# kwea123/CasMVSNet_pl

Measured on NVIDIA H100. Metric: depth-maps/sec at 640x512 V=3 D=48/32/8, higher is better.
Workload: dtype f32 (conv products tf32, fp32 accumulate)

## Files before the change

### casmvsnet_pl_b200/_lib.py

```python
import ctypes
import os
from ctypes import c_char_p, c_double, c_float, c_int, c_size_t, c_uint64, c_void_p, POINTER

_HERE = os.path.dirname(os.path.abspath(__file__))
LIB_PATH = os.path.join(_HERE, "csrc", "libcasmvs.so")

NCHW, NHWC = 0, 1
ROUND_TF32 = 256
KEEP_FP32_OUT = 256
FP32, TF32 = 0, 1
CONV, CONV_TRANSPOSE, CONV_PLANAR = 0, 1, 2
PRECISIONS = {"fp32": FP32, "tf32": TF32}

SIGNATURES = {
    "casmvs_version": (c_int, []),
    "casmvs_last_error": (c_char_p, []),
    "casmvs_device_check": (c_int, [c_int]),
    "casmvs_launch_count": (c_uint64, []),
    "casmvs_fallback_count": (c_uint64, []),
    "casmvs_release_weight_images": (c_int, [c_void_p, c_size_t]),
    "casmvs_weight_cache_generation": (c_uint64, []),
    "casmvs_weight_image_count": (c_int, [c_void_p, c_size_t]),
    "casmvs_settle_weight_images": (c_int, []),
    "casmvs_warp_cost_workspace_bytes": (c_size_t, [c_int] * 6),
    "casmvs_warp_cost_fwd": (c_int, [c_void_p, c_int, c_void_p, c_void_p, c_void_p, c_int,
                                     c_int, c_int, c_int, c_int, c_int, c_int, c_int,
                                     c_void_p, c_size_t, c_void_p]),
    "casmvs_homo_warp_fwd": (c_int, [c_void_p, c_int, c_void_p, c_void_p, c_void_p, c_int,
                                     c_int, c_int, c_int, c_int, c_int, c_void_p]),
    "casmvs_packed_conv3d_weight_floats": (c_size_t, [c_int, c_int]),
    "casmvs_pack_conv3d_weights": (c_int, [c_void_p, c_int, c_int, c_int, c_void_p, c_void_p]),
    "casmvs_invalidate_weight_cache": (c_int, []),
    "casmvs_conv3d_fwd": (c_int, [c_void_p, c_void_p, c_void_p, c_void_p, c_float, c_void_p,
                                  c_void_p, c_int, c_int, c_int, c_int, c_int, c_int,
                                  c_int, c_int, c_int, c_void_p]),
    "casmvs_costreg_param_floats": (c_size_t, [c_int]),
    "casmvs_costreg_layer_info": (c_int, [c_int, c_int, POINTER(c_int), POINTER(c_int),
                                          POINTER(c_int), POINTER(c_int), POINTER(c_size_t),
                                          POINTER(c_size_t), POINTER(c_size_t)]),
    "casmvs_costreg_workspace_bytes": (c_size_t, [c_int] * 5),
    "casmvs_costreg_fwd": (c_int, [c_void_p, c_void_p, c_void_p, c_int, c_int, c_int, c_int,
                                   c_int, c_int, c_void_p, c_size_t, c_void_p]),
    "casmvs_regress_fwd": (c_int, [c_void_p, c_void_p, c_int, c_int, c_void_p, c_void_p,
                                   c_void_p, c_void_p, c_int, c_int, c_int, c_int, c_void_p]),
    "casmvs_depth_hypotheses_fwd": (c_int, [c_void_p, c_int, c_float, c_float, c_void_p,
                                            c_void_p, c_int, c_int, c_int, c_int, c_void_p]),
    "casmvs_uniform_hypotheses_fwd": (c_int, [c_float, c_float, c_void_p, c_void_p, c_void_p,
                                              c_int, c_int, c_int, c_int, c_void_p]),
    "casmvs_depth_first_fwd": (c_int, [c_void_p, c_int, c_float, c_float, c_void_p, c_void_p,
                                       c_int, c_int, c_int, c_int, c_void_p]),
    "casmvs_warp_cost_ladder_fwd": (c_int, [c_void_p, c_void_p, c_void_p, c_void_p, c_float, c_void_p,
                                            c_float, c_void_p] + [c_int] * 8 + [c_void_p]),
    "casmvs_regress_ladder_fwd": (c_int, [c_void_p, c_void_p, c_void_p, c_float, c_void_p, c_float,
                                          c_void_p, c_void_p, c_void_p] + [c_int] * 4 + [c_void_p]),
    "casmvs_fpn_level_fwd": (c_int, [c_void_p] * 8 + [c_int] * 5 + [c_void_p]),
    "casmvs_fpn_merge_fwd": (c_int, [c_void_p] * 5 + [c_int] * 5 + [c_void_p]),
    "casmvs_conv2d_rgb8_fwd": (c_int, [c_void_p, c_void_p, c_void_p, c_float, c_void_p] + [c_int] * 4 + [c_void_p]),
    "casmvs_conv2d_5x5s2_fwd": (c_int, [c_void_p, c_void_p, c_void_p, c_float, c_void_p] + [c_int] * 6 + [c_void_p]),
    "casmvs_conv2d_5x5s2_fp32_fwd": (c_int, [c_void_p, c_void_p, c_void_p, c_float, c_void_p] + [c_int] * 5 + [c_void_p]),
    "casmvs_bias_act_nhwc": (c_int, [c_void_p, c_void_p, c_float, c_size_t, c_int, c_int, c_void_p]),
    "casmvs_bias_lrelu_nhwc": (c_int, [c_void_p, c_void_p, c_float, c_size_t, c_int, c_void_p]),
    "casmvs_normalize_u8_fwd": (c_int, [c_void_p, c_void_p, c_int, c_int, c_int, POINTER(c_float),
                                        POINTER(c_float), c_void_p]),
    "casmvs_warp_cost_bwd": (c_int, [c_void_p] * 5 + [c_int] * 7 + [c_void_p]),
    "casmvs_conv3d_wgrad": (c_int, [c_void_p] * 3 + [c_int] * 10 + [c_void_p]),
    "casmvs_regress_bwd": (c_int, [c_void_p, c_void_p, c_int, c_void_p, c_void_p] + [c_int] * 4 + [c_void_p]),
    "casmvs_geo_fuse_fwd": (c_int, [c_void_p, c_void_p, c_void_p, c_void_p, c_void_p,
                                    POINTER(c_float), POINTER(c_float), c_void_p, c_int, c_int,
                                    c_int, c_float, c_int, c_void_p, c_void_p, c_void_p, c_void_p,
                                    c_void_p, c_void_p, c_void_p, c_void_p]),
    "casmvs_pcd_cell_keys": (c_int, [c_void_p, c_int, c_double, c_double, c_double, c_double,
                                     c_int, c_int, c_int, c_int, c_void_p, c_void_p]),
    "casmvs_pcd_thin_workspace_bytes": (c_size_t, [c_int, c_int]),
    "casmvs_pcd_thin_prepare": (c_int, [c_void_p, c_void_p, c_int, c_int, c_int, c_int, c_int,
                                        c_void_p, c_size_t, c_void_p]),
    "casmvs_pcd_thin_round": (c_int, [c_void_p, c_void_p, c_void_p, c_int, c_int, c_double,
                                      c_void_p, c_void_p, c_void_p, c_size_t, c_void_p]),
    "casmvs_pcd_capped_nn": (c_int, [c_void_p, c_int, c_void_p, c_void_p, c_void_p, c_int, c_void_p,
                                     POINTER(c_double), c_double, POINTER(c_int), POINTER(c_double),
                                     POINTER(c_double), c_double, c_void_p, c_void_p]),
    "casmvs_nchw_to_nhwc":(c_int, [c_void_p, c_void_p, c_int, c_int, c_size_t, c_void_p]),
    "casmvs_nhwc_to_nchw": (c_int, [c_void_p, c_void_p, c_int, c_int, c_size_t, c_void_p]),
}

_lib = None


class CasMVSError(RuntimeError):
    pass


def load():
    global _lib
    if _lib is not None:
        return _lib
    if not os.path.isfile(LIB_PATH):
        raise CasMVSError(
            f"{LIB_PATH} not found: build it with `python -c 'import __graft_entry__ as g; "
            "g.build()'` (or `make -C casmvsnet_pl_b200/csrc`). There is no CPU/PyTorch "
            "fallback for the hot path.")
    lib = ctypes.CDLL(LIB_PATH)
    for name, (res, args) in SIGNATURES.items():
        fn = getattr(lib, name)
        fn.restype = res
        fn.argtypes = args
    _lib = lib
    return lib


def check(rc, what=""):
    if rc != 0:
        msg = load().casmvs_last_error()
        raise CasMVSError(f"{what}: {msg.decode() if msg else 'error'} (status {rc})")


def launch_count():
    return int(load().casmvs_launch_count())


def fallback_count():
    return int(load().casmvs_fallback_count())


def weight_cache_generation():
    return int(load().casmvs_weight_cache_generation())
```

### casmvsnet_pl_b200/csrc/api.cu

```cuda
#include <stdarg.h>
#include <string.h>

#include "common.cuh"

namespace casmvs {

std::atomic<uint64_t> g_launches{0};
std::atomic<uint64_t> g_fallbacks{0};
static thread_local char t_err[512] = "";

void set_error(const char* fmt, ...) {
  va_list ap;
  va_start(ap, fmt);
  vsnprintf(t_err, sizeof(t_err), fmt, ap);
  va_end(ap);
}

int conv3d_direct(const float* x, const float* wpk, const float* scale, const float* shift,
                  float slope, const float* skip, float* y, int B, int Cin, int Cout, int D,
                  int h, int w, int kind, int stride, cudaStream_t st, int round_out);
int conv3d_tma(const float* x, const float* wpk, const float* scale, const float* shift,
               float slope, const float* skip, float* y, int B, int Cin, int Cout, int D, int h,
               int w, int kind, int stride, int precision, cudaStream_t st);
int conv3d_tma2(const float* x, const float* wpk, const float* scale, const float* shift,
                float slope, const float* skip, float* y, int B, int Cin, int Cout, int D, int h,
                int w, int kind, int stride, int precision, cudaStream_t st);

struct LayerSpec { int cin, cout, kind, stride; };

static void costreg_layers(int Cin, LayerSpec (&L)[11]) {
  const LayerSpec t[11] = {
      {Cin, 8, CASMVS_CONV, 1},  {8, 16, CASMVS_CONV, 2},  {16, 16, CASMVS_CONV, 1},
      {16, 32, CASMVS_CONV, 2},  {32, 32, CASMVS_CONV, 1}, {32, 64, CASMVS_CONV, 2},
      {64, 64, CASMVS_CONV, 1},  {64, 32, CASMVS_CONV_TRANSPOSE, 2},
      {32, 16, CASMVS_CONV_TRANSPOSE, 2}, {16, 8, CASMVS_CONV_TRANSPOSE, 2},
      {8, 1, CASMVS_CONV, 1}};
  memcpy(L, t, sizeof(t));
}

}

using namespace casmvs;

extern "C" int casmvs_version(void) { return CASMVS_VERSION; }
extern "C" const char* casmvs_last_error(void) { return t_err; }
extern "C" uint64_t casmvs_launch_count(void) { return g_launches.load(); }

extern "C" uint64_t casmvs_fallback_count(void) { return g_fallbacks.load(); }

extern "C" int casmvs_device_check(int device) {
  int n = 0;
  cudaError_t e = cudaGetDeviceCount(&n);
  if (e != cudaSuccess || n == 0) {
    set_error("device_check: no CUDA device (%s)", cudaGetErrorString(e));
    return -3;
  }
  CASMVS_REQUIRE(device >= 0 && device < n, "device_check: device %d out of range (%d)", device, n);
  int major = 0, minor = 0;
  cudaDeviceGetAttribute(&major, cudaDevAttrComputeCapabilityMajor, device);
  cudaDeviceGetAttribute(&minor, cudaDevAttrComputeCapabilityMinor, device);
  if (major != 9 || minor != 0) {
    set_error("device_check: compute capability %d.%d; libcasmvs is built for sm_90a only "
              "(no fallback path)", major, minor);
    return -3;
  }
  return 0;
}

extern "C" int casmvs_conv3d_fwd(const float* x, const float* w_packed, const float* scale,
                                 const float* shift, float slope, const float* skip, float* y,
                                 int B, int Cin, int Cout, int D, int h, int w, int kind,
                                 int stride, int precision, void* stream) {
  CASMVS_REQUIRE(x && w_packed && y, "conv3d: null pointer");
  CASMVS_REQUIRE(B >= 0 && Cin > 0 && Cout > 0 && D > 0 && h > 0 && w > 0, "conv3d: bad dims");
  CASMVS_REQUIRE(Cin % 4 == 0, "conv3d: Cin must be a multiple of 4 (got %d)", Cin);
  CASMVS_REQUIRE(kind == CASMVS_CONV || kind == CASMVS_CONV_TRANSPOSE ||
                     kind == CASMVS_CONV_PLANAR, "conv3d: bad kind");
  CASMVS_REQUIRE(kind == CASMVS_CONV ? (stride == 1 || stride == 2)
                 : kind == CASMVS_CONV_PLANAR ? stride == 1 : stride == 2,
                 "conv3d: unsupported stride %d", stride);
  const int flags = precision & ~0xff;
  precision &= 0xff;
  CASMVS_REQUIRE((precision == CASMVS_FP32 || precision == CASMVS_TF32) &&
                     (flags & ~CASMVS_KEEP_FP32_OUT) == 0, "conv3d: bad precision %d", precision);
  if (B == 0) return 0;
  cudaStream_t st = as_stream(stream);
  if (precision == CASMVS_TF32) {
    const int pf = precision | flags;
    int rc = conv3d_tma(x, w_packed, scale, shift, slope, skip, y, B, Cin, Cout, D, h, w, kind,
                    stride, pf, st);
    if (rc <= 0) return rc;
    if (kind != CASMVS_CONV_PLANAR) {
      rc = conv3d_tma2(x, w_packed, scale, shift, slope, skip, y, B, Cin, Cout, D, h, w, kind,
                       stride, precision, st);
      if (rc <= 0) return rc;
    }
    g_fallbacks.fetch_add(1, std::memory_order_relaxed);
  }
  const int round_out =
      (precision == CASMVS_TF32 && Cout > 1 && !(flags & CASMVS_KEEP_FP32_OUT)) ? 1 : 0;
  return conv3d_direct(x, w_packed, scale, shift, slope, skip, y, B, Cin, Cout, D, h, w, kind,
                       stride, st, round_out);
}

extern "C" size_t casmvs_costreg_param_floats(int Cin) {
  LayerSpec L[11];
  costreg_layers(Cin, L);
  size_t n = 0;
  for (auto& l : L) n += (size_t)27 * l.cin * l.cout + 2 * (size_t)l.cout;
  return n;
}

extern "C" int casmvs_costreg_layer_info(int Cin, int layer, int* cin, int* cout, int* kind,
                                         int* stride, size_t* w_off, size_t* scale_off,
                                         size_t* shift_off) {
  CASMVS_REQUIRE(layer >= 0 && layer < 11, "costreg_layer_info: layer %d out of range", layer);
  LayerSpec L[11];
  costreg_layers(Cin, L);
  size_t off = 0;
  for (int i = 0; i < layer; ++i) off += (size_t)27 * L[i].cin * L[i].cout + 2 * (size_t)L[i].cout;
  if (cin) *cin = L[layer].cin;
  if (cout) *cout = L[layer].cout;
  if (kind) *kind = L[layer].kind;
  if (stride) *stride = L[layer].stride;
  if (w_off) *w_off = off;
  off += (size_t)27 * L[layer].cin * L[layer].cout;
  if (scale_off) *scale_off = off;
  if (shift_off) *shift_off = off + L[layer].cout;
  return 0;
}

extern "C" size_t casmvs_costreg_workspace_bytes(int B, int Cin, int D, int h, int w) {
  (void)Cin;
  const size_t n = (size_t)B * D * h * w;
  return (8 * n + 2 * n + 2 * n + n / 2 + n / 2 + n / 8 + n / 8 + n / 2 + 2 * n + 8 * n + 64) *
         sizeof(float);
}

extern "C" int casmvs_costreg_fwd(const float* x, const float* params, float* logits, int B,
                                  int Cin, int D, int h, int w, int precision, void* workspace,
                                  size_t workspace_bytes, void* stream) {
  CASMVS_REQUIRE(x && params && logits, "costreg: null pointer");
  CASMVS_REQUIRE(D % 8 == 0 && h % 8 == 0 && w % 8 == 0,
                 "costreg: D,h,w must be divisible by 8 (got %d,%d,%d)", D, h, w);
  const size_t need = casmvs_costreg_workspace_bytes(B, Cin, D, h, w);
  CASMVS_REQUIRE(workspace && workspace_bytes >= need, "costreg: workspace too small (%zu < %zu)",
                 workspace_bytes, need);
  if (B == 0) return 0;
  LayerSpec L[11];
  costreg_layers(Cin, L);
  const float *W[11], *SC[11], *SH[11];
  {
    size_t off = 0;
    for (int i = 0; i < 11; ++i) {
      W[i] = params + off; off += (size_t)27 * L[i].cin * L[i].cout;
      SC[i] = params + off; off += L[i].cout;
      SH[i] = params + off; off += L[i].cout;
    }
  }
  const size_t n = (size_t)B * D * h * w;
  float* ws = (float*)workspace;
  float* c0 = ws;            ws += 8 * n;
  float* c1 = ws;            ws += 2 * n;
  float* c2 = ws;            ws += 2 * n;
  float* c3 = ws;            ws += n / 2;
  float* c4 = ws;            ws += n / 2;
  float* c5 = ws;            ws += n / 8;
  float* c6 = ws;            ws += n / 8;
  float* u7 = ws;            ws += n / 2;
  float* u9 = ws;            ws += 2 * n;
  float* u11 = ws;
  const float slope = 0.01f;
  int rc;
#define LAYER(i, in, skip, out, d_, h_, w_, sl)                                                   \
  rc = casmvs_conv3d_fwd(in, W[i], SC[i], SH[i], sl, skip, out, B, L[i].cin, L[i].cout, d_, h_,  \
                         w_, L[i].kind, L[i].stride, precision, stream);                          \
  if (rc) return rc;
  LAYER(0, x, nullptr, c0, D, h, w, slope)
  LAYER(1, c0, nullptr, c1, D, h, w, slope)
  LAYER(2, c1, nullptr, c2, D / 2, h / 2, w / 2, slope)
  LAYER(3, c2, nullptr, c3, D / 2, h / 2, w / 2, slope)
  LAYER(4, c3, nullptr, c4, D / 4, h / 4, w / 4, slope)
  LAYER(5, c4, nullptr, c5, D / 4, h / 4, w / 4, slope)
  LAYER(6, c5, nullptr, c6, D / 8, h / 8, w / 8, slope)
  LAYER(7, c6, c4, u7, D / 8, h / 8, w / 8, slope)
  LAYER(8, u7, c2, u9, D / 4, h / 4, w / 4, slope)
  LAYER(9, u9, c0, u11, D / 2, h / 2, w / 2, slope)
  LAYER(10, u11, nullptr, logits, D, h, w, 1.0f)
#undef LAYER
  return 0;
}
```

### casmvsnet_pl_b200/csrc/common.cuh

```cuda
#pragma once
#include <cuda_runtime.h>
#include <stdint.h>
#include <stdio.h>
#include <atomic>

#include "casmvs.h"

#if defined(__CUDA_ARCH__) && (__CUDA_ARCH__ != 900)
#error "libcasmvs is written for sm_90a (H100) only"
#endif

namespace casmvs {

void set_error(const char* fmt, ...);
extern std::atomic<uint64_t> g_launches;
extern std::atomic<uint64_t> g_fallbacks;

inline cudaStream_t as_stream(void* s) { return reinterpret_cast<cudaStream_t>(s); }

inline int after_launch(const char* what) {
  g_launches.fetch_add(1, std::memory_order_relaxed);
  cudaError_t e = cudaGetLastError();
  if (e != cudaSuccess) {
    set_error("%s: kernel launch failed: %s", what, cudaGetErrorString(e));
    return -2;
  }
  return 0;
}

#define CASMVS_REQUIRE(cond, ...)        \
  do {                                   \
    if (!(cond)) {                       \
      casmvs::set_error(__VA_ARGS__);    \
      return -1;                         \
    }                                    \
  } while (0)

constexpr int kMaxDevices = 64;
inline int cur_device() {
  int dev = 0;
  cudaGetDevice(&dev);
  return dev >= 0 && dev < kMaxDevices ? dev : 0;
}
inline int num_sms() {
  static std::atomic<int> n[kMaxDevices];
  const int dev = cur_device();
  int v = n[dev].load(std::memory_order_relaxed);
  if (v == 0) {
    cudaDeviceGetAttribute(&v, cudaDevAttrMultiProcessorCount, dev);
    if (v <= 0) v = 132;
    n[dev].store(v, std::memory_order_relaxed);
  }
  return v;
}
template <typename K>
inline int opt_in_smem(K kfn, int bytes, std::atomic<bool> (&done)[kMaxDevices], const char* what) {
  const int dev = cur_device();
  if (done[dev].load(std::memory_order_acquire)) return 0;
  cudaError_t e = cudaFuncSetAttribute(kfn, cudaFuncAttributeMaxDynamicSharedMemorySize, bytes);
  if (e != cudaSuccess) {
    set_error("%s: cannot opt in to %d B of shared memory: %s", what, bytes, cudaGetErrorString(e));
    return -2;
  }
  done[dev].store(true, std::memory_order_release);
  return 0;
}

struct FastDiv {
  uint32_t d, m;
};
inline FastDiv make_fastdiv(uint32_t d) {
  return FastDiv{d, d > 1 ? (uint32_t)((1ull << 32) / d) + 1u : 0u};
}
inline bool fastdiv_ok(uint64_t n_max, uint32_t d) { return n_max * d < (1ull << 32); }
__device__ __forceinline__ uint32_t fastdivmod(uint32_t n, const FastDiv f, uint32_t& r) {
  const uint32_t q = f.d > 1 ? __umulhi(n, f.m) : n;
  r = n - q * f.d;
  return q;
}

__device__ __forceinline__ float4 ldg4(const float* p) {
  return __ldg(reinterpret_cast<const float4*>(p));
}
__device__ __forceinline__ void st4(float* p, float4 v) {
  *reinterpret_cast<float4*>(p) = v;
}
__device__ __forceinline__ void st4_stream(float* p, float4 v) {
  asm volatile("st.global.L1::no_allocate.v4.f32 [%0], {%1,%2,%3,%4};" ::"l"(p), "f"(v.x),
               "f"(v.y), "f"(v.z), "f"(v.w)
               : "memory");
}

}
```

### casmvsnet_pl_b200/csrc/conv3d_tma.cu

```cuda
#include <cudaTypedefs.h>
#include <stdlib.h>

#include "common.cuh"
#include "tc_common.cuh"
#include <mutex>

#include "tma_common.cuh"

namespace casmvs {

namespace tma {

using namespace tc;

struct Params {
  const float* bimg;
  const float* scale;
  const float* shift;
  const float* skip;
  float* y;
  float slope;
  int B, D, H, W, Cout;
  int cout_total;
  int tiles_w, tiles_h, nchunks, dchunk;
  int round_out;
  int planar;
};

template <int CIN, int GW, int SLOTS_>
struct Smem {
  static constexpr int SLOTS = SLOTS_;
  static constexpr int CQ = CIN / 4;
  static constexpr int kBrickData = kHaloH * kHaloW * 16;
  static constexpr int kBrickBytes = (kBrickData + 127) / 128 * 128;
  static constexpr int kSlotBytes = CQ * kBrickBytes;
  static constexpr int kWBytes = 9 * CIN * 3 * GW * 4;
  static constexpr int kRingOff = 0;
  static constexpr int kWOff = SLOTS * kSlotBytes;
  static constexpr int kParamOff = kWOff + kWBytes;
  static constexpr int kBarOff = kParamOff + 2 * GW * 4;
  static constexpr int kTotal = kBarOff + 192 + 1024;
};

template <int GW, int OFF>
__device__ __forceinline__ void store_slice(const float* acc, const Params& p, const float* s_param,
                                            int b, int od, int h0, int w0, int row0, int wl,
                                            int lane, int co_base) {
  for_each_pair<OFF, GW>(acc, wl, lane, [&](int r, int c, float a0, float a1) {
    const int m = row0 + r;
    const int oh = h0 + (m >> 3), ow = w0 + (m & 7);
    if (oh >= p.H || ow >= p.W || c >= p.Cout) return;
    const size_t o = ((((size_t)b * p.D + od) * p.H + oh) * p.W + ow) * p.cout_total + co_base + c;
    float v0 = fmaf(a0, s_param[c], s_param[GW + c]);
    float v1 = fmaf(a1, s_param[c + 1], s_param[GW + c + 1]);
    v0 = v0 >= 0.f ? v0 : v0 * p.slope;
    v1 = v1 >= 0.f ? v1 : v1 * p.slope;
    if (c + 1 < p.Cout && (p.cout_total & 1) == 0) {
      if (p.skip) {
        const float2 s2 = __ldg(reinterpret_cast<const float2*>(p.skip + o));
        v0 += s2.x; v1 += s2.y;
      }
      if (p.round_out) { v0 = to_tf32(v0); v1 = to_tf32(v1); }
      *reinterpret_cast<float2*>(p.y + o) = make_float2(v0, v1);
    } else {
      if (p.skip) v0 += __ldg(p.skip + o);
      p.y[o] = p.round_out ? to_tf32(v0) : v0;
      if (c + 1 < p.Cout) {
        if (p.skip) v1 += __ldg(p.skip + o + 1);
        p.y[o + 1] = p.round_out ? to_tf32(v1) : v1;
      }
    }
  });
}

template <int CIN, int GW, int SLOTS_, bool PLANAR>
__global__ void __launch_bounds__(kConvThreads, 1)
conv3d_tma_kernel(const __grid_constant__ CUtensorMap xmap, const Params p) {
  using S = Smem<CIN, GW, SLOTS_>;
  constexpr int SLOTS = S::SLOTS;
  extern __shared__ unsigned char smem_raw[];
  const uint32_t s_raw = smem_u32(smem_raw);
  const uint32_t s_base = (s_raw + 1023u) & ~1023u;
  unsigned char* smem = smem_raw + (s_base - s_raw);
  const uint32_t s_ring = s_base + S::kRingOff, s_w = s_base + S::kWOff,
                 s_bar = s_base + S::kBarOff;
  float* s_param = reinterpret_cast<float*>(smem + S::kParamOff);
  const uint32_t bar_full = s_bar, bar_empty = s_bar + 64, bar_w = s_bar + 128;

  const int warp = warp_uniform(threadIdx.x >> 5), lane = threadIdx.x & 31;
  const int total_items = p.B * p.nchunks * p.tiles_h * p.tiles_w;

  {
    const int t = threadIdx.x;
    if (t < SLOTS) mbar_init(bar_full + 8 * t, 1);
    else if (t < 2 * SLOTS) mbar_init(bar_empty + 8 * (t - SLOTS), kConsumerThreads);
    else if (t == 2 * SLOTS) mbar_init(bar_w, 1);
    if (t <= 2 * SLOTS) fence_barrier_init();
  }
  const int co_base = blockIdx.y * p.Cout;
  for (int i = threadIdx.x; i < GW; i += kConvThreads) {
    s_param[i] = (i < p.Cout) ? (p.scale ? __ldg(p.scale + co_base + i) : 1.f) : 0.f;
    s_param[GW + i] = (i < p.Cout) ? (p.shift ? __ldg(p.shift + co_base + i) : 0.f) : 0.f;
  }
  fence_proxy_async();
  __syncthreads();
  if (threadIdx.x == 0) load_image_bulk(s_w, p.bimg + (size_t)blockIdx.y * (S::kWBytes / 4), S::kWBytes, bar_w);

  tma::pdl_trigger();
  tma::pdl_wait();
  bool w_ready = false;
  uint32_t gs = 0;
  float acc[(PLANAR ? 1 : 3) * GW / 2];
#pragma unroll
  for (int i = 0; i < (PLANAR ? 1 : 3) * GW / 2; ++i) acc[i] = 0.f;
  float done[GW / 2];
  int pend_od = -1, pend_b = 0, pend_h0 = 0, pend_w0 = 0;
  const int wg = warp >> 2, wl = warp & 3;
  const int row0 = 64 * wg;
  for (int item0 = blockIdx.x; item0 < total_items; item0 += gridDim.x) {
    int item = item0;
    const int tw = item % p.tiles_w; item /= p.tiles_w;
    const int th = item % p.tiles_h; item /= p.tiles_h;
    const int ck = item % p.nchunks;
    const int b = item / p.nchunks;
    const int w0 = tw * kTileW, h0 = th * kTileH;
    const int d0 = ck * p.dchunk, d1 = min(p.D, d0 + p.dchunk);
    const int nd = d1 - d0;
    const int halo = PLANAR ? 0 : 1;
    const int nslices = nd + 2 * halo;

    if (warp == kProdWarp) {
      if (lane == 0) {
        for (int it = 0; it < nslices; ++it) {
          const uint32_t g = gs + it;
          const int slot = g % SLOTS;
          if (g >= (uint32_t)SLOTS) mbar_wait(bar_empty + 8 * slot, ((g / SLOTS) - 1) & 1);
          const uint32_t dst = s_ring + slot * S::kSlotBytes;
          mbar_expect_tx(bar_full + 8 * slot, S::CQ * S::kBrickData);
#pragma unroll
          for (int q = 0; q < S::CQ; ++q)
            tma_load_5d(dst + q * S::kBrickBytes, &xmap, bar_full + 8 * slot, q * 4, w0 - 1,
                        h0 - 1, d0 - halo + it, b);
        }
      }
      __syncwarp();
    } else {
      constexpr uint32_t a_lbo = S::kBrickBytes, a_sbo = kHaloW * 16;
      constexpr uint32_t b_lbo = 3 * GW * 16, b_sbo = 128;
      const uint64_t a_desc0 = make_desc(s_ring + 8 * wg * a_sbo, a_lbo, a_sbo);
      const uint64_t b_desc0 = make_desc(s_w, b_lbo, b_sbo);
      for (int it = 0; it < nslices; ++it) {
        const uint32_t g = gs + it;
        mbar_wait(bar_full + 8 * (g % SLOTS), (g / SLOTS) & 1);
        if (!w_ready) { mbar_wait(bar_w, 0); w_ready = true; }
        const uint64_t a_s = a_desc0 + (((g % SLOTS) * S::kSlotBytes) >> 4);
        wgmma_fence();
#pragma unroll
        for (int khw = 0; khw < 9; ++khw) {
          const int kh = khw / 3, kw = khw % 3;
#pragma unroll
          for (int k8 = 0; k8 < CIN / 8; ++k8) {
            const uint32_t a_off = ((kh * kHaloW + kw) * 16 + 2 * k8 * S::kBrickBytes) >> 4;
            const uint32_t b_off = (khw * (CIN * 3 * GW * 4) + k8 * 2 * 3 * GW * 16) >> 4;
            if constexpr (PLANAR)
              wgmma_tf32<GW>(acc, a_s + a_off, b_desc0 + b_off + ((GW * 16) >> 4));
            else
              wgmma_tf32<3 * GW>(acc, a_s + a_off, b_desc0 + b_off);
          }
        }
        wgmma_commit();
        if (pend_od >= 0)
          store_slice<GW, 0>(done, p, s_param, pend_b, pend_od, pend_h0, pend_w0, row0, wl, lane,
                             co_base);
        wgmma_wait_all();
        mbar_arrive(bar_empty + 8 * (g % SLOTS));
#pragma unroll
        for (int i = 0; i < GW / 2; ++i) done[i] = acc[i];
        if constexpr (PLANAR) {
#pragma unroll
          for (int i = 0; i < GW / 2; ++i) acc[i] = 0.f;
        } else {
#pragma unroll
          for (int i = 0; i < GW; ++i) acc[i] = acc[i + GW / 2];
#pragma unroll
          for (int i = 0; i < GW / 2; ++i) acc[GW + i] = 0.f;
        }
        const int j = PLANAR ? it : it - 2;
        pend_od = (j >= 0 && j < nd) ? d0 + j : -1;
        pend_b = b; pend_h0 = h0; pend_w0 = w0;
      }
    }
    gs += nslices;
  }
  if (pend_od >= 0)
    store_slice<GW, 0>(done, p, s_param, pend_b, pend_od, pend_h0, pend_w0, row0, wl, lane, co_base);
}


static PFN_cuTensorMapEncodeTiled_v12000 encode_fn() {
  static PFN_cuTensorMapEncodeTiled_v12000 fn = nullptr;
  static bool tried = false;
  if (!tried) {
    tried = true;
    void* ptr = nullptr;
    cudaDriverEntryPointQueryResult q;
    if (cudaGetDriverEntryPoint("cuTensorMapEncodeTiled", &ptr, cudaEnableDefault, &q) ==
            cudaSuccess && q == cudaDriverEntryPointSuccess)
      fn = reinterpret_cast<PFN_cuTensorMapEncodeTiled_v12000>(ptr);
  }
  return fn;
}

int encode_tiled(CUtensorMap* out, const void* base, int rank, const uint64_t* dims,
                 const uint64_t* strides_bytes, const uint32_t* box, int swizzle_bytes) {
  auto enc = encode_fn();
  if (!enc) { set_error("tma: cuTensorMapEncodeTiled is not available"); return -2; }
  cuuint64_t gdim[5], gstr[4];
  cuuint32_t bx[5], es[5];
  for (int i = 0; i < rank; ++i) { gdim[i] = dims[i]; bx[i] = box[i]; es[i] = 1; }
  for (int i = 0; i + 1 < rank; ++i) gstr[i] = strides_bytes[i];
  const CUtensorMapSwizzle sw = swizzle_bytes == 128 ? CU_TENSOR_MAP_SWIZZLE_128B
                                : swizzle_bytes == 64 ? CU_TENSOR_MAP_SWIZZLE_64B
                                : swizzle_bytes == 32 ? CU_TENSOR_MAP_SWIZZLE_32B
                                                      : CU_TENSOR_MAP_SWIZZLE_NONE;
  const CUresult r = enc(out, CU_TENSOR_MAP_DATA_TYPE_FLOAT32, (cuuint32_t)rank,
                         const_cast<void*>(base), gdim, gstr, bx, es,
                         CU_TENSOR_MAP_INTERLEAVE_NONE, sw, CU_TENSOR_MAP_L2_PROMOTION_L2_128B,
                         CU_TENSOR_MAP_FLOAT_OOB_FILL_NONE);
  if (r != CUDA_SUCCESS) {
    set_error("tma: cuTensorMapEncodeTiled failed (%d), rank %d", (int)r, rank);
    return -2;
  }
  return 0;
}

struct MapEntry { const void* x; int B, D, H, W, C, CB, bw, bh, sw; CUtensorMap map; };
static MapEntry g_maps[128];
static int g_maps_n = 0, g_maps_next = 0;
static std::mutex g_maps_mu;

const CUtensorMap* input_map(const float* x, int B, int D, int H, int W, int C, int CB, int box_w,
                             int box_h, int stride_w) {
  static thread_local CUtensorMap t_ret;
  std::lock_guard<std::mutex> lock(g_maps_mu);
  for (int i = 0; i < g_maps_n; ++i) {
    const MapEntry& e = g_maps[i];
    if (e.x == x && e.B == B && e.D == D && e.H == H && e.W == W && e.C == C && e.CB == CB &&
        e.bw == box_w && e.bh == box_h && e.sw == stride_w) {
      t_ret = e.map;
      return &t_ret;
    }
  }
  auto enc = encode_fn();
  if (!enc) { set_error("conv3d_tma: cuTensorMapEncodeTiled is not available"); return nullptr; }
  MapEntry& e = g_maps[g_maps_next];
  g_maps_next = (g_maps_next + 1) % 128;
  if (g_maps_n < 128) ++g_maps_n;
  const cuuint64_t gdim[5] = {(cuuint64_t)C, (cuuint64_t)W, (cuuint64_t)H, (cuuint64_t)D,
                              (cuuint64_t)B};
  const cuuint64_t gstr[4] = {(cuuint64_t)C * 4, (cuuint64_t)W * C * 4, (cuuint64_t)H * W * C * 4,
                              (cuuint64_t)D * H * W * C * 4};
  const cuuint32_t box[5] = {(cuuint32_t)CB, (cuuint32_t)box_w, (cuuint32_t)box_h, 1, 1};
  const cuuint32_t estr[5] = {1, (cuuint32_t)stride_w, 1, 1, 1};
  const CUtensorMapSwizzle sw = CB * 4 == 128 ? CU_TENSOR_MAP_SWIZZLE_128B
                                : CB * 4 == 64 ? CU_TENSOR_MAP_SWIZZLE_64B
                                : CB * 4 == 32 ? CU_TENSOR_MAP_SWIZZLE_32B
                                               : CU_TENSOR_MAP_SWIZZLE_NONE;
  const CUresult r = enc(&e.map, CU_TENSOR_MAP_DATA_TYPE_FLOAT32, 5, const_cast<float*>(x), gdim,
                         gstr, box, estr, CU_TENSOR_MAP_INTERLEAVE_NONE, sw,
                         CU_TENSOR_MAP_L2_PROMOTION_L2_128B, CU_TENSOR_MAP_FLOAT_OOB_FILL_NONE);
  if (r != CUDA_SUCCESS) {
    e.x = nullptr;
    set_error("conv3d_tma: cuTensorMapEncodeTiled failed (%d) for C=%d W=%d H=%d D=%d B=%d",
              (int)r, C, W, H, D, B);
    return nullptr;
  }
  e.x = x; e.B = B; e.D = D; e.H = H; e.W = W; e.C = C; e.CB = CB; e.bw = box_w; e.bh = box_h; e.sw = stride_w;
  t_ret = e.map;
  return &t_ret;
}


template <int CIN, int GW, int SLOTS, bool PLANAR>
static int launch(const float* x, const float* wpk, Params p, cudaStream_t st) {
  using S = Smem<CIN, GW, SLOTS>;
  static_assert(S::kTotal <= 227 * 1024, "shared memory budget");
  auto kfn = conv3d_tma_kernel<CIN, GW, SLOTS, PLANAR>;
  static std::atomic<bool> attr_set[kMaxDevices];
  if (int rc = opt_in_smem(kfn, S::kTotal, attr_set, "conv3d_tma")) return rc;
  const CUtensorMap* map = input_map(x, p.B, p.D, p.H, p.W, CIN, 4, kHaloW, kHaloH);
  if (!map) return -2;
  static int dchunk_env = -1;
  if (dchunk_env < 0) {
    const char* d = getenv("CASMVS_TMA_DCHUNK");
    dchunk_env = d ? atoi(d) : 0;
  }
  const int per_sm = resident_per_sm(kfn, kConvThreads, S::kTotal);
  const int nco = p.cout_total / p.Cout;
  const int cap = 32;
  const long cols = (long)p.B * p.tiles_w * p.tiles_h;
  int dchunk = pick_dchunk(p.D, cap, cols, (long)num_sms() * per_sm / nco, 1, p.planar ? 0 : 2);
  if (dchunk_env > 0 && dchunk_env <= cap) dchunk = dchunk_env < p.D ? dchunk_env : p.D;
  p.dchunk = dchunk;
  p.nchunks = (p.D + dchunk - 1) / dchunk;
  const ImageRef ir = image_cache_get(wpk, 1000 + CIN * 100 + GW, (size_t)S::kWBytes * nco, st);
  if (!ir.img) return -2;
  if (!ir.hit) {
    if (int rc = build_stride1_image(wpk, ir.img, CIN, GW, p.Cout, p.cout_total, st)) return rc;
    image_cache_built(ir.img, st);
  }
  p.bimg = ir.img;
  const long items = (long)p.B * p.nchunks * p.tiles_h * p.tiles_w;
  int resident = num_sms() * per_sm / nco;
  if (resident < 1) resident = 1;
  const long gx = items < resident ? items : resident;
  launch_pdl(ir.settled, kfn, dim3((unsigned)gx, (unsigned)nco), kConvThreads, S::kTotal, st, *map, p);
  return after_launch("conv3d_tma");
}

}

int conv3d_tma(const float* x, const float* wpk, const float* scale, const float* shift,
               float slope, const float* skip, float* y, int B, int Cin, int Cout, int D, int h,
               int w, int kind, int stride, int precision_flags, cudaStream_t st) {
  const int precision = precision_flags & 0xff;
  static int enabled = -1, round_out = 1;
  if (enabled < 0) {
    const char* e = getenv("CASMVS_TMA");
    enabled = e ? atoi(e) : 1;
    if (const char* s = getenv("CASMVS_TC_ROUND")) round_out = atoi(s);
  }
  if (!enabled || precision != CASMVS_TF32) return 1;
  if ((kind != CASMVS_CONV && kind != CASMVS_CONV_PLANAR) || stride != 1) return 1;
  const bool deep = Cin == 64 && Cout == 64;
  if (!deep && (!(Cin == 8 || Cin == 16 || Cin == 32) || Cout > 32)) return 1;
  if ((reinterpret_cast<uintptr_t>(x) & 15) != 0) return 1;
  tma::Params p;
  p.scale = scale; p.shift = shift; p.skip = skip; p.y = y;
  p.slope = slope; p.B = B; p.D = D; p.H = h; p.W = w;
  p.Cout = deep ? 16 : Cout; p.cout_total = Cout;
  p.tiles_w = (w + tc::kTileW - 1) / tc::kTileW;
  p.tiles_h = (h + tc::kTileH - 1) / tc::kTileH;
  const int npad = p.Cout <= 8 ? 8 : p.Cout <= 16 ? 16 : 32;
  p.planar = kind == CASMVS_CONV_PLANAR ? 1 : 0;
  p.round_out = (round_out && Cout > 1 && !(precision_flags & CASMVS_KEEP_FP32_OUT)) ? 1 : 0;
#define TMA_CASE(CI, NP, SL)                                                    \
  if (Cin == CI && npad == NP)                                                  \
    return p.planar ? tma::launch<CI, NP, SL, true>(x, wpk, p, st)              \
                    : tma::launch<CI, NP, SL, false>(x, wpk, p, st);
  TMA_CASE(8, 8, 4) TMA_CASE(8, 32, 4) TMA_CASE(16, 8, 4) TMA_CASE(16, 16, 4)
  TMA_CASE(16, 32, 4) TMA_CASE(32, 8, 4) TMA_CASE(32, 16, 4) TMA_CASE(32, 32, 4)
  TMA_CASE(64, 16, 2)
#undef TMA_CASE
  return 1;
}

}
```

### casmvsnet_pl_b200/csrc/conv3d_tma2.cu

```cuda
#include <stdlib.h>

#include "common.cuh"
#include "tc_common.cuh"
#include "tma_common.cuh"

namespace casmvs {
namespace tma2 {

using namespace casmvs::tc;
using casmvs::tma::mbar_expect_tx;
using casmvs::tma::tma_load_5d;

enum { MODE_S2 = 0, MODE_T = 1, MODE_P5 = 2 };

struct Params {
  const float* bimg;
  const float* scale;
  const float* shift;
  const float* skip;
  float* y;
  float slope;
  int B, Di, Hi, Wi, Do, Ho, Wo, Cout;
  int tiles_w, tiles_h, nchunks, dchunk;
  int round_out;
};

template <int MODE, int CIN, int COUT>
struct Cfg {
  static constexpr int CQ = CIN / 4;
  static constexpr int BR = MODE == MODE_S2 ? 33 : MODE == MODE_T ? 17 : 35;
  static constexpr int BW = MODE == MODE_P5 ? 10 : 9;
  static constexpr int PAR = MODE == MODE_T ? 1 : 2;
  static constexpr int NPL = PAR * CQ;
  static constexpr int kPlaneData = BR * BW * 16;
  static constexpr int kPlaneBytes = (kPlaneData + 127) / 128 * 128;
  static constexpr int kSlotBytes = NPL * kPlaneBytes;
  static constexpr int GW = MODE == MODE_T ? 8 * COUT : (COUT <= 16 ? 16 : 32);
  static constexpr int BROWS = MODE == MODE_S2 ? 3 * GW : MODE == MODE_T ? 12 * COUT : GW;
  static constexpr int NTAP = MODE == MODE_S2 ? 9 : MODE == MODE_T ? 4 : 25;
  static constexpr int kWBytes = NTAP * CIN * BROWS * 4;
  static constexpr int kFixed = kWBytes + 2 * 32 * 4 + 192 + 1024;
  static constexpr int SLOTS = (kFixed + 4 * kSlotBytes <= 227 * 1024) ? 4
                               : (kFixed + 3 * kSlotBytes <= 227 * 1024) ? 3 : 2;
  static constexpr int kRingOff = 0;
  static constexpr int kWOff = SLOTS * kSlotBytes;
  static constexpr int kParamOff = kWOff + kWBytes;
  static constexpr int kBarOff = kParamOff + 2 * 32 * 4;
  static constexpr int kTotal = kBarOff + 192 + 1024;
};

template <int MODE, int CIN, int COUT>
__global__ void __launch_bounds__(kConvThreads, 1)
conv3d_tma2_kernel(const __grid_constant__ CUtensorMap xmap, const Params p) {
  using C = Cfg<MODE, CIN, COUT>;
  constexpr int BW = C::BW, GW = C::GW, BROWS = C::BROWS;
  constexpr int SLOTS = C::SLOTS;
  extern __shared__ unsigned char smem_raw[];
  const uint32_t s_raw = smem_u32(smem_raw);
  const uint32_t s_base = (s_raw + 1023u) & ~1023u;
  unsigned char* smem = smem_raw + (s_base - s_raw);
  const uint32_t s_ring = s_base + C::kRingOff, s_w = s_base + C::kWOff,
                 s_bar = s_base + C::kBarOff;
  float* s_param = reinterpret_cast<float*>(smem + C::kParamOff);
  const uint32_t bar_full = s_bar, bar_empty = s_bar + 64, bar_w = s_bar + 128;
  const int warp = warp_uniform(threadIdx.x >> 5), lane = threadIdx.x & 31;
  const int total_items = p.B * p.nchunks * p.tiles_h * p.tiles_w;
  const int Dm = MODE == MODE_T ? p.Di : p.Do;

  {
    const int t = threadIdx.x;
    if (t < SLOTS) mbar_init(bar_full + 8 * t, 1);
    else if (t < 2 * SLOTS) mbar_init(bar_empty + 8 * (t - SLOTS), kConsumerThreads);
    else if (t == 2 * SLOTS) mbar_init(bar_w, 1);
    if (t <= 2 * SLOTS) fence_barrier_init();
  }
  const int co_base = blockIdx.y * COUT;
  for (int i = threadIdx.x; i < 32; i += kConvThreads) {
    s_param[i] = (i < COUT) ? (p.scale ? __ldg(p.scale + co_base + i) : 1.f) : 0.f;
    s_param[32 + i] = (i < COUT) ? (p.shift ? __ldg(p.shift + co_base + i) : 0.f) : 0.f;
  }
  fence_proxy_async();
  __syncthreads();
  if (threadIdx.x == 0) tma::load_image_bulk(s_w, p.bimg + (size_t)blockIdx.y * (C::kWBytes / 4), C::kWBytes, bar_w);

  tma::pdl_trigger();
  tma::pdl_wait();
  bool w_ready = false;
  uint32_t gs = 0;
  for (int item0 = blockIdx.x; item0 < total_items; item0 += gridDim.x) {
    int item = item0;
    const int tw = item % p.tiles_w; item /= p.tiles_w;
    const int th = item % p.tiles_h; item /= p.tiles_h;
    const int ck = item % p.nchunks;
    const int b = item / p.nchunks;
    const int w0 = tw * kTileW, h0 = th * kTileH;
    const int g0 = ck * p.dchunk, g1 = min(Dm, g0 + p.dchunk);
    const int ng = g1 - g0;
    const int nslices = MODE == MODE_S2 ? 2 * ng + 1 : MODE == MODE_T ? ng + 1 : ng;
    const int s_first = MODE == MODE_S2 ? 2 * g0 - 1 : g0;

    if (warp == kProdWarp) {
      if (lane == 0) {
        for (int it = 0; it < nslices; ++it) {
          const uint32_t g = gs + it;
          const int slot = g % SLOTS;
          if (g >= (uint32_t)SLOTS) mbar_wait(bar_empty + 8 * slot, ((g / SLOTS) - 1) & 1);
          const uint32_t dst = s_ring + slot * C::kSlotBytes;
          mbar_expect_tx(bar_full + 8 * slot, C::NPL * C::kPlaneData);
#pragma unroll
          for (int pl = 0; pl < C::NPL; ++pl) {
            const int q = pl / C::PAR, par = pl % C::PAR;
            const int wc = MODE == MODE_S2 ? 2 * w0 - 1 + par
                           : MODE == MODE_T ? w0 : 2 * w0 - 2 + par;
            const int hc = MODE == MODE_S2 ? 2 * h0 - 1 : MODE == MODE_T ? h0 : 2 * h0 - 2;
            tma_load_5d(dst + pl * C::kPlaneBytes, &xmap, bar_full + 8 * slot, 4 * q, wc,
                        hc, s_first + it, b);
          }
        }
      }
      __syncwarp();
    } else {
      const int wg = warp >> 2, wl = warp & 3;
      const int row0 = 64 * wg;
      constexpr uint32_t a_lbo = C::PAR * C::kPlaneBytes;
      constexpr uint32_t a_sbo = (MODE == MODE_T ? 1 : 2) * BW * 16;
      constexpr uint32_t b_lbo = BROWS * 16, b_sbo = 128;
      const uint64_t a_desc0 = make_desc(s_ring + 8 * wg * a_sbo, a_lbo, a_sbo);
      const uint64_t b_desc0 = make_desc(s_w, b_lbo, b_sbo);
      constexpr int NACC = MODE == MODE_S2 ? 2 * GW : MODE == MODE_T ? 12 * COUT : GW;
      float acc[NACC / 2];
      float prev0[MODE == MODE_T ? 2 * COUT : 1];
#pragma unroll
      for (int i = 0; i < NACC / 2; ++i) acc[i] = 0.f;

      auto issue = [&](auto n_tag, uint64_t a_s, int row0b) {
        constexpr int N = decltype(n_tag)::value;
        wgmma_fence();
#pragma unroll
        for (int tap = 0; tap < C::NTAP; ++tap) {
          int a_tap, pl0;
          if (MODE == MODE_S2) {
            const int kh = tap / 3, kw = tap % 3;
            a_tap = kh * BW + (kw == 2 ? 1 : 0);
            pl0 = kw == 1 ? 1 : 0;
          } else if (MODE == MODE_P5) {
            const int kh = tap / 5, kw = tap % 5;
            a_tap = kh * BW + (kw >> 1);
            pl0 = kw & 1;
          } else {
            const int sh = tap >> 1, sw = tap & 1;
            a_tap = sh * BW + sw;
            pl0 = 0;
          }
#pragma unroll
          for (int k8 = 0; k8 < CIN / 8; ++k8) {
            const uint32_t a_off = ((2 * k8 * C::PAR + pl0) * C::kPlaneBytes + a_tap * 16) >> 4;
            const uint32_t b_off = (tap * (CIN * BROWS * 4) + k8 * 2 * BROWS * 16 + row0b * 16) >> 4;
            wgmma_tf32<N>(acc, a_s + a_off, b_desc0 + b_off);
          }
        }
        wgmma_commit();
        wgmma_wait_all();
      };

      auto store2 = [&](int od, int oh, int ow, int c, float a0, float a1, bool has_skip) {
        const size_t o = ((((size_t)b * p.Do + od) * p.Ho + oh) * p.Wo + ow) * p.Cout + co_base + c;
        float v0 = fmaf(a0, s_param[c], s_param[32 + c]);
        float v1 = fmaf(a1, s_param[c + 1], s_param[32 + c + 1]);
        v0 = v0 >= 0.f ? v0 : v0 * p.slope;
        v1 = v1 >= 0.f ? v1 : v1 * p.slope;
        if (has_skip) {
          const float2 s2 = __ldg(reinterpret_cast<const float2*>(p.skip + o));
          v0 += s2.x; v1 += s2.y;
        }
        if (p.round_out) { v0 = to_tf32(v0); v1 = to_tf32(v1); }
        *reinterpret_cast<float2*>(p.y + o) = make_float2(v0, v1);
      };
      auto store_plain = [&](const float* src, int od) {
        for_each_pair<0, GW>(src, wl, lane, [&](int r, int c, float a0, float a1) {
          const int m = row0 + r;
          const int mh = h0 + (m >> 3), mw = w0 + (m & 7);
          if (c < COUT && mh < p.Ho && mw < p.Wo) store2(od, mh, mw, c, a0, a1, false);
        });
      };
      auto store_t = [&](const float* pd1, int jd) {
        auto one = [&](int pd, int r, int col, float a0, float a1) {
          const int m = row0 + r;
          const int mh = h0 + (m >> 3), mw = w0 + (m & 7);
          if (mh >= p.Hi || mw >= p.Wi) return;
          const int cls = col / COUT, c = col % COUT;
          const int ph = cls >> 1, pw = cls & 1;
          store2(2 * jd + pd, 2 * mh + ph, 2 * mw + pw, c, a0, a1, p.skip != nullptr);
        };
        for_each_pair<0, 4 * COUT>(prev0, wl, lane,
                                   [&](int r, int col, float a0, float a1) { one(0, r, col, a0, a1); });
        for_each_pair<0, 4 * COUT>(pd1, wl, lane,
                                   [&](int r, int col, float a0, float a1) { one(1, r, col, a0, a1); });
      };

      for (int it = 0; it < nslices; ++it) {
        const uint32_t g = gs + it;
        mbar_wait(bar_full + 8 * (g % SLOTS), (g / SLOTS) & 1);
        if (!w_ready) { mbar_wait(bar_w, 0); w_ready = true; }
        const uint64_t a_s = a_desc0 + (((g % SLOTS) * C::kSlotBytes) >> 4);
        if constexpr (MODE == MODE_S2) {
          if ((it & 1) == 0) issue(std::integral_constant<int, 2 * GW>{}, a_s, GW);
          else issue(std::integral_constant<int, GW>{}, a_s, 0);
        } else if constexpr (MODE == MODE_P5) {
#pragma unroll
          for (int i = 0; i < GW / 2; ++i) acc[i] = 0.f;
          issue(std::integral_constant<int, GW>{}, a_s, 0);
        } else {
          issue(std::integral_constant<int, 12 * COUT>{}, a_s, 0);
        }
        mbar_arrive(bar_empty + 8 * (g % SLOTS));
        if constexpr (MODE == MODE_S2) {
          if ((it & 1) == 0) {
            const int a = it >> 1;
            float done[GW / 2];
#pragma unroll
            for (int i = 0; i < GW / 2; ++i) {
              done[i] = acc[i];
              acc[i] = acc[GW / 2 + i];
              acc[GW / 2 + i] = 0.f;
            }
            if (a >= 1) store_plain(done, g0 + a - 1);
          }
        } else if constexpr (MODE == MODE_P5) {
          float done[GW / 2];
#pragma unroll
          for (int i = 0; i < GW / 2; ++i) done[i] = acc[i];
          store_plain(done, g0 + it);
        } else {
          float pd1[2 * COUT];
#pragma unroll
          for (int i = 0; i < 2 * COUT; ++i) pd1[i] = acc[i];
          if (it >= 1) store_t(pd1, g0 + it - 1);
#pragma unroll
          for (int i = 0; i < 2 * COUT; ++i) {
            prev0[i] = acc[2 * COUT + i];
            acc[i] = acc[4 * COUT + i];
            acc[2 * COUT + i] = 0.f;
            acc[4 * COUT + i] = 0.f;
          }
        }
      }
    }
    gs += nslices;
  }
}

template <int MODE, int CIN, int COUT>
__global__ void build_image_tma2_kernel(const float* __restrict__ wpk, float* __restrict__ img,
                                        int cout_total) {
  using C = Cfg<MODE, CIN, COUT>;
  constexpr int CQ = C::CQ, GW = C::GW, BROWS = C::BROWS;
  constexpr int per = C::NTAP * CIN * BROWS;
  for (int t = blockIdx.x * blockDim.x + threadIdx.x; t < per * (cout_total / COUT);
       t += gridDim.x * blockDim.x) {
    const int ck = t / per, i = t - ck * per;
    const int jq = i & 3;
    const int row = (i >> 2) % BROWS;
    const int r = (i >> 2) / BROWS;
    const int cq = r % CQ, tap = r / CQ;
    const int ci = cq * 4 + jq;
    int kd = -1, kh = -1, kw = -1, co = -1;
    if (MODE == MODE_S2) {
      const int g = row / GW;
      co = row % GW;
      kd = g == 0 ? 1 : g == 1 ? 2 : 0;
      kh = tap / 3; kw = tap % 3;
      if (co >= COUT) kd = -1;
    } else {
      const int sh = tap >> 1, sw = tap & 1;
      const int blk = row / (4 * COUT);
      const int cls = (row / COUT) & 3;
      co = row % COUT;
      const int ph = cls >> 1, pw = cls & 1;
      kd = blk;
      kh = sh == 0 ? (ph == 0 ? 1 : 2) : (ph == 1 ? 0 : -1);
      kw = sw == 0 ? (pw == 0 ? 1 : 2) : (pw == 1 ? 0 : -1);
      if (kh < 0 || kw < 0) kd = -1;
    }
    float v = 0.f;
    if (kd >= 0)
      v = to_tf32(__ldg(wpk + ((size_t)((kd * 3 + kh) * 3 + kw) * CIN + ci) * cout_total +
                        ck * COUT + co));
    img[t] = v;
  }
}

template <int CIN, int COUT>
__global__ void build_image_p5_kernel(const float* __restrict__ wt, float* __restrict__ img) {
  using C = Cfg<MODE_P5, CIN, COUT>;
  constexpr int CQ = C::CQ, GW = C::GW;
  constexpr int total = 25 * CIN * GW;
  for (int t = blockIdx.x * blockDim.x + threadIdx.x; t < total; t += gridDim.x * blockDim.x) {
    const int jq = t & 3;
    const int co = (t >> 2) % GW;
    const int r = (t >> 2) / GW;
    const int cq = r % CQ, tap = r / CQ;
    const int ci = cq * 4 + jq;
    img[t] = co < COUT ? to_tf32(__ldg(wt + ((size_t)co * CIN + ci) * 25 + tap)) : 0.f;
  }
}

template <int MODE, int CIN, int COUT>
static int launch2(const float* x, const float* wpk, Params p, cudaStream_t st) {
  using C = Cfg<MODE, CIN, COUT>;
  static_assert(C::kTotal <= 227 * 1024, "shared memory budget");
  auto kfn = conv3d_tma2_kernel<MODE, CIN, COUT>;
  static std::atomic<bool> attr_set[kMaxDevices];
  if (int rc = opt_in_smem(kfn, C::kTotal, attr_set, "conv3d_tma2")) return rc;
  const CUtensorMap* map =
      MODE == MODE_S2   ? tma::input_map(x, p.B, p.Di, p.Hi, p.Wi, CIN, 4, 17, C::BR, 2)
      : MODE == MODE_P5 ? tma::input_map(x, p.B, p.Di, p.Hi, p.Wi, CIN, 4, 19, C::BR, 2)
                        : tma::input_map(x, p.B, p.Di, p.Hi, p.Wi, CIN, 4, C::BW, C::BR, 1);
  if (!map) return -2;
  const int per_sm = tma::resident_per_sm(kfn, kConvThreads, C::kTotal);
  const int Dm = MODE == MODE_T ? p.Di : p.Do;
  const int Hm = MODE == MODE_T ? p.Hi : p.Ho, Wm = MODE == MODE_T ? p.Wi : p.Wo;
  p.tiles_w = (Wm + kTileW - 1) / kTileW;
  p.tiles_h = (Hm + kTileH - 1) / kTileH;
  const int nco = p.Cout / COUT;
  const int cap = 32;
  const long cols = (long)p.B * p.tiles_w * p.tiles_h;
  const int dchunk = tma::pick_dchunk(Dm, cap, cols, (long)num_sms() * per_sm / nco,
                                      MODE == MODE_S2 ? 2 : 1,
                                      MODE == MODE_S2 ? 1 : MODE == MODE_T ? 1 : 0);
  p.dchunk = dchunk;
  p.nchunks = (Dm + dchunk - 1) / dchunk;
  const long items = cols * p.nchunks;
  const ImageRef ir = image_cache_get(wpk, 2000 + MODE * 10000 + CIN * 100 + COUT,
                                      (size_t)C::kWBytes * nco, st);
  float* img = ir.img;
  if (!img) return -2;
  if (!ir.hit) {
    if constexpr (MODE == MODE_P5)
      build_image_p5_kernel<CIN, COUT><<<32, 256, 0, st>>>(wpk, img);
    else
      build_image_tma2_kernel<MODE, CIN, COUT><<<64, 256, 0, st>>>(wpk, img, p.Cout);
    if (int rc = after_launch("conv3d_tma2/build_image")) return rc;
    image_cache_built(img, st);
  }
  p.bimg = img;
  long resident = (long)num_sms() * per_sm / nco;
  if (resident < 1) resident = 1;
  const long gx = items < resident ? items : resident;
  tma::launch_pdl(ir.settled, kfn, dim3((unsigned)gx, (unsigned)nco), kConvThreads, C::kTotal, st, *map, p);
  return after_launch("conv3d_tma2");
}

}

int conv3d_tma2(const float* x, const float* wpk, const float* scale, const float* shift,
                float slope, const float* skip, float* y, int B, int Cin, int Cout, int D, int h,
                int w, int kind, int stride, int precision, cudaStream_t st) {
  static int enabled = -1;
  if (enabled < 0) {
    const char* e = getenv("CASMVS_TMA2");
    enabled = e ? atoi(e) : 3;
  }
  if (!enabled || precision != CASMVS_TF32) return 1;
  if ((reinterpret_cast<uintptr_t>(x) & 15) != 0) return 1;
  tma2::Params p;
  p.scale = scale; p.shift = shift; p.skip = skip; p.y = y;
  p.slope = slope; p.B = B; p.Di = D; p.Hi = h; p.Wi = w; p.Cout = Cout; p.round_out = 1;
  if (kind == CASMVS_CONV && stride == 2 && (enabled & 1)) {
    if (skip) return 1;
    p.Do = (D - 1) / 2 + 1; p.Ho = (h - 1) / 2 + 1; p.Wo = (w - 1) / 2 + 1;
    if (Cin == 8 && Cout == 16) return tma2::launch2<tma2::MODE_S2, 8, 16>(x, wpk, p, st);
    if (Cin == 16 && Cout == 32) return tma2::launch2<tma2::MODE_S2, 16, 32>(x, wpk, p, st);
    if (Cin == 32 && Cout == 64) return tma2::launch2<tma2::MODE_S2, 32, 16>(x, wpk, p, st);
    return 1;
  }
  if (kind == CASMVS_CONV_TRANSPOSE && (enabled & 2)) {
    p.Do = 2 * D; p.Ho = 2 * h; p.Wo = 2 * w;
    if (Cin == 16 && Cout == 8) return tma2::launch2<tma2::MODE_T, 16, 8>(x, wpk, p, st);
    if (Cin == 32 && Cout == 16) return tma2::launch2<tma2::MODE_T, 32, 16>(x, wpk, p, st);
    if (Cin == 64 && Cout == 32) return tma2::launch2<tma2::MODE_T, 64, 8>(x, wpk, p, st);
    return 1;
  }
  return 1;
}

}

using namespace casmvs;

extern "C" int casmvs_conv2d_5x5s2_fwd(const float* x, const float* w, const float* shift,
                                       float slope, float* y, int N, int Cin, int Cout, int H,
                                       int W, int round_tf32, void* stream) {
  CASMVS_REQUIRE(x && w && y, "conv2d_5x5s2: null pointer");
  CASMVS_REQUIRE(N >= 0 && H >= 2 && W >= 2, "conv2d_5x5s2: bad dims");
  CASMVS_REQUIRE((reinterpret_cast<uintptr_t>(x) & 15) == 0, "conv2d_5x5s2: x must be 16 B aligned");
  if (N == 0) return 0;
  tma2::Params p;
  p.scale = nullptr; p.shift = shift; p.skip = nullptr; p.y = y; p.slope = slope;
  p.B = 1; p.Di = N; p.Hi = H; p.Wi = W; p.Do = N; p.Ho = (H - 1) / 2 + 1; p.Wo = (W - 1) / 2 + 1;
  p.Cout = Cout; p.round_out = round_tf32 ? 1 : 0;
  cudaStream_t st = as_stream(stream);
  if (Cin == 8 && Cout == 16) return tma2::launch2<tma2::MODE_P5, 8, 16>(x, w, p, st);
  if (Cin == 16 && Cout == 32) return tma2::launch2<tma2::MODE_P5, 16, 32>(x, w, p, st);
  set_error("conv2d_5x5s2: only the FeatureNet shapes 8->16 and 16->32 are built (got %d->%d)",
            Cin, Cout);
  return -1;
}
```

### casmvsnet_pl_b200/csrc/k1_common.cuh

```cuda
#pragma once
#include "common.cuh"

namespace casmvs {

constexpr int kCPT = 8;

typedef unsigned long long u64;
__device__ __forceinline__ u64 pk2(float lo, float hi) {
  u64 r; asm("mov.b64 %0, {%1,%2};" : "=l"(r) : "f"(lo), "f"(hi)); return r;
}
__device__ __forceinline__ void unpk2(u64 v, float& lo, float& hi) {
  asm("mov.b64 {%0,%1}, %2;" : "=f"(lo), "=f"(hi) : "l"(v));
}
__device__ __forceinline__ u64 fma2(u64 a, u64 b, u64 c) {
  float a0, a1, b0, b1, c0, c1;
  unpk2(a, a0, a1); unpk2(b, b0, b1); unpk2(c, c0, c1);
  return pk2(__fmaf_rn(a0, b0, c0), __fmaf_rn(a1, b1, c1));
}
__device__ __forceinline__ u64 mul2(u64 a, u64 b) {
  float a0, a1, b0, b1;
  unpk2(a, a0, a1); unpk2(b, b0, b1);
  return pk2(__fmul_rn(a0, b0), __fmul_rn(a1, b1));
}
__device__ __forceinline__ u64 add2(u64 a, u64 b) {
  float a0, a1, b0, b1;
  unpk2(a, a0, a1); unpk2(b, b0, b1);
  return pk2(__fadd_rn(a0, b0), __fadd_rn(a1, b1));
}
struct Tex8 { u64 v[4]; };
__device__ __forceinline__ Tex8 ldg256(const float* p) {
  Tex8 t;
  asm volatile("ld.global.nc.v2.b64 {%0,%1}, [%2];" : "=l"(t.v[0]), "=l"(t.v[1]) : "l"(p));
  asm volatile("ld.global.nc.v2.b64 {%0,%1}, [%2];" : "=l"(t.v[2]), "=l"(t.v[3]) : "l"(p + 4));
  return t;
}
__device__ __forceinline__ void stg256(float* p, const u64 (&v)[4]) {
  asm volatile("st.global.v2.b64 [%0], {%1,%2};" ::"l"(p), "l"(v[0]), "l"(v[1]) : "memory");
  asm volatile("st.global.v2.b64 [%0], {%1,%2};" ::"l"(p + 4), "l"(v[2]), "l"(v[3]) : "memory");
}

__device__ __forceinline__ float round_tf32_f(float x) {
  uint32_t r; asm("cvt.rna.tf32.f32 %0, %1;" : "=r"(r) : "f"(x)); return __uint_as_float(r);
}
__device__ __forceinline__ float rcp_approx(float x) {
  float r; asm("rcp.approx.ftz.f32 %0, %1;" : "=f"(r) : "f"(x)); return r;
}


struct Window {
  Tex8 t00, t01, t10, t11;
};

template <int CT>
__device__ __forceinline__ void sample_view(const float* __restrict__ vbase, float qx, float qy,
                                            float qz, int h, int w, int C, int row_floats,
                                            Window& win, float& w00, float& w01, float& w10,
                                            float& w11) {
  const float rz = rcp_approx(qz);
  const float u = qx * rz, v = qy * rz;
  const float x0f = floorf(u), y0f = floorf(v);
  const int x0 = __float2int_rd(u), y0 = __float2int_rd(v);
  const bool valid = (qz > 1e-7f) && (unsigned)(x0 + 1) <= (unsigned)w &&
                     (unsigned)(y0 + 1) <= (unsigned)h;
  const float fx = u - x0f, fy = v - y0f;
  float wxa = 1.f - fx, wxb = fx, wya = 1.f - fy, wyb = fy;
  if (x0 < 0) { wxa = wxb; wxb = 0.f; }
  if (x0 > w - 2) { wxb = wxa; wxa = 0.f; }
  if (y0 < 0) { wya = wyb; wyb = 0.f; }
  if (y0 > h - 2) { wyb = wya; wya = 0.f; }
  if (!valid) { wxa = 0.f; wxb = 0.f; }
  const int xs = min(max(x0, 0), w - 2), ys = min(max(y0, 0), h - 2);
  w00 = wxa * wya; w01 = wxb * wya; w10 = wxa * wyb; w11 = wxb * wyb;
  const int cc = CT > 0 ? CT : C;
  const unsigned off = (unsigned)(ys * row_floats + xs * cc);
  const float* p = vbase + off;
  win.t00 = ldg256(p);
  win.t01 = ldg256(p + cc);
  win.t10 = ldg256(p + row_floats);
  win.t11 = ldg256(p + row_floats + cc);
}


struct Hyp {
  const float* dv;
  const float* first_map;
  const float* first_b;
  const float* step_b;
  float first, step;
};
struct HypPix {
  const float* p;
  size_t hw;
  float first, step;
  __device__ __forceinline__ HypPix(const Hyp& h, int b, int D, size_t hw_, int pix) : hw(hw_) {
    p = h.dv ? h.dv + (size_t)b * D * hw_ + pix : nullptr;
    first = h.first_map ? __ldg(h.first_map + (size_t)b * hw_ + pix) : h.first_b ? __ldg(h.first_b + b) : h.first;
    step = h.step_b ? __ldg(h.step_b + b) : h.step;
  }
  __device__ __forceinline__ float at(int d) const {
    return p ? __ldg(p + (size_t)d * hw) : __fadd_rn(first, __fmul_rn(step, (float)d));
  }
};

}
```

### casmvsnet_pl_b200/csrc/tma_common.cuh

```cuda
#pragma once
#include <cuda.h>
#include <stdlib.h>

#include "tc_common.cuh"

namespace casmvs {
namespace tma {

__device__ __forceinline__ void mbar_expect_tx(uint32_t bar, uint32_t bytes) {
  asm volatile("mbarrier.arrive.expect_tx.shared::cta.b64 _, [%0], %1;" ::"r"(bar), "r"(bytes)
               : "memory");
}
__device__ __forceinline__ void tma_load_5d(uint32_t dst, const CUtensorMap* map, uint32_t bar,
                                            int c0, int c1, int c2, int c3, int c4) {
  asm volatile(
      "cp.async.bulk.tensor.5d.shared::cluster.global.mbarrier::complete_tx::bytes "
      "[%0], [%1, {%3, %4, %5, %6, %7}], [%2];"
      ::"r"(dst), "l"(reinterpret_cast<uint64_t>(map)), "r"(bar), "r"(c0), "r"(c1), "r"(c2),
      "r"(c3), "r"(c4)
      : "memory");
}

__device__ __forceinline__ void load_image_bulk(uint32_t dst_smem, const float* src, int bytes,
                                                uint32_t bar) {
  mbar_expect_tx(bar, (uint32_t)bytes);
  for (int off = 0; off < bytes; off += 32768) {
    const uint32_t n = (uint32_t)(bytes - off < 32768 ? bytes - off : 32768);
    asm volatile(
        "cp.async.bulk.shared::cluster.global.mbarrier::complete_tx::bytes [%0], [%1], %2, [%3];"
        ::"r"(dst_smem + off), "l"(reinterpret_cast<const char*>(src) + off), "r"(n), "r"(bar)
        : "memory");
  }
}

__device__ __forceinline__ void pdl_wait() { asm volatile("griddepcontrol.wait;" ::: "memory"); }
__device__ __forceinline__ void pdl_trigger() {
  asm volatile("griddepcontrol.launch_dependents;" ::: "memory");
}
template <typename Kernel, typename... Args>
inline cudaError_t launch_pdl(bool allow, Kernel kfn, dim3 grid, int threads, size_t smem,
                              cudaStream_t st, Args... args) {
  static int pdl = -1;
  if (pdl < 0) {
    const char* e = getenv("CASMVS_PDL");
    pdl = e ? atoi(e) : 1;
  }
  cudaLaunchConfig_t cfg = {};
  cfg.gridDim = grid;
  cfg.blockDim = dim3((unsigned)threads);
  cfg.dynamicSmemBytes = smem;
  cfg.stream = st;
  cudaLaunchAttribute attr[1];
  attr[0].id = cudaLaunchAttributeProgrammaticStreamSerialization;
  attr[0].val.programmaticStreamSerializationAllowed = 1;
  cfg.attrs = attr;
  cfg.numAttrs = (pdl && allow) ? 1 : 0;
  return cudaLaunchKernelEx(&cfg, kfn, args...);
}

const CUtensorMap* input_map(const float* x, int B, int D, int H, int W, int C, int CB, int box_w,
                             int box_h, int stride_w = 1);

int encode_tiled(CUtensorMap* out, const void* base, int rank, const uint64_t* dims,
                 const uint64_t* strides_bytes, const uint32_t* box, int swizzle_bytes);

__device__ __forceinline__ void tma_load_4d(uint32_t dst, const CUtensorMap* map, uint32_t bar,
                                            int c0, int c1, int c2, int c3) {
  asm volatile(
      "cp.async.bulk.tensor.4d.shared::cluster.global.mbarrier::complete_tx::bytes "
      "[%0], [%1, {%3, %4, %5, %6}], [%2];"
      ::"r"(dst), "l"(reinterpret_cast<uint64_t>(map)), "r"(bar), "r"(c0), "r"(c1), "r"(c2),
      "r"(c3)
      : "memory");
}

inline int pow2_floor(int v) { int r = 1; while (r * 2 <= v) r *= 2; return r; }

template <typename K>
inline int resident_per_sm(K kfn, int threads, int smem) {
  int n = 0;
  if (cudaOccupancyMaxActiveBlocksPerMultiprocessor(&n, kfn, threads, smem) != cudaSuccess) n = 1;
  return n < 1 ? 1 : n;
}

inline int pick_dchunk(int D, int cap, long cols, long resident, int mul, int add, int fixed = -1) {
  if (fixed < 0) {
    static int env_fixed = -1;
    if (env_fixed < 0) {
      const char* e = getenv("CASMVS_DCHUNK_FIXED");
      env_fixed = e ? atoi(e) : 0;
    }
    fixed = env_fixed;
  }
  if (cap > D) cap = D;
  if (cap < 1) cap = 1;
  if (resident < 1) resident = 1;
  int best = cap;
  long best_cost = -1;
  for (int dc = cap; dc >= 1; --dc) {
    const long items = cols * ((D + dc - 1) / dc);
    const long rounds = (items + resident - 1) / resident;
    const long cost = rounds * (mul * dc + add + fixed);
    if (best_cost < 0 || cost < best_cost) { best_cost = cost; best = dc; }
  }
  return best;
}

}
}
```

### casmvsnet_pl_b200/csrc/warp_cost.cu

```cuda
#include <stdlib.h>

#include "k1_common.cuh"

namespace casmvs {

constexpr int kMaxSrc = 15;
constexpr int kK1Threads = 128;

struct Taps {
  int o00, o01, o10, o11;
  float w00, w01, w10, w11;
  bool any;
};

__device__ __forceinline__ Taps make_taps(float qx, float qy, float qz, int h, int w, int C) {
  Taps t;
  t.any = false;
  t.o00 = t.o01 = t.o10 = t.o11 = 0;
  t.w00 = t.w01 = t.w10 = t.w11 = 0.f;
  if (!(qz > 1e-7f)) return t;
  float rz = __frcp_rn(qz);
  float u = qx * rz, v = qy * rz;
  if (!(u > -1.f && u < (float)w && v > -1.f && v < (float)h)) return t;
  float x0f = floorf(u), y0f = floorf(v);
// ... 274 lines not shown
  const int d_end = min(D, d_begin + dchunk);
  const float* dptr = dv + (size_t)b * D * hw + pixc + (size_t)d_begin * hw;
  float depth_next = d_begin < d_end ? __ldg(dptr) : 1.f;
  float* optr = cost + ((size_t)(b * D + d_begin) * hw + pixc) * C + c0;

  for (int d = d_begin; d < d_end; ++d) {
    const float depth = depth_next;
    dptr += hw;
    if (d + 1 < d_end) depth_next = __ldg(dptr);
    const float inv_d = rcp_approx(depth);
    u64 S[NP], Q[NP];
#pragma unroll
    for (int k = 0; k < NP; ++k) { S[k] = ref.v[k]; Q[k] = mul2(ref.v[k], ref.v[k]); }
#pragma unroll
    for (int v = 0; v < NSRC; ++v) {
      const float qx = fmaf(tx[v], inv_d, ax[v]);
      const float qy = fmaf(ty[v], inv_d, ay[v]);
      const float qz = fmaf(tz[v], inv_d, az[v]);
      const float rz = rcp_approx(qz);
      const float u = qx * rz, vv = qy * rz;
      const float x0f = floorf(u), y0f = floorf(vv);
      const int x0 = __float2int_rd(u), y0 = __float2int_rd(vv);
      const bool valid = (qz > 1e-7f) && (unsigned)(x0 + 1) <= (unsigned)w &&
                         (unsigned)(y0 + 1) <= (unsigned)h;
      const float fx = u - x0f, fy = vv - y0f;
      float wxa = 1.f - fx, wxb = fx, wya = 1.f - fy, wyb = fy;
      if (x0 < 0) { wxa = wxb; wxb = 0.f; }
      if (x0 > w - 2) { wxb = wxa; wxa = 0.f; }
      if (y0 < 0) { wya = wyb; wyb = 0.f; }
      if (y0 > h - 2) { wyb = wya; wya = 0.f; }
      if (!valid) { wxa = 0.f; wxb = 0.f; }
      const int xs = min(max(x0, 0), w - 2), ys = min(max(y0, 0), h - 2);
      if (!SKIP || xs != cx[v] || ys != cy[v]) {
        const float* p = fb + (size_t)(v + 1) * view_stride + (unsigned)(ys * row_floats + xs * C);
        t00[v] = ldg_tex<CPT>(p);
        t01[v] = ldg_tex<CPT>(p + C);
        t10[v] = ldg_tex<CPT>(p + row_floats);
        t11[v] = ldg_tex<CPT>(p + row_floats + C);
        cx[v] = xs; cy[v] = ys;
      }
      const float w00 = wxa * wya, w01 = wxb * wya, w10 = wxa * wyb, w11 = wxb * wyb;
      const u64 p00 = pk2(w00, w00), p01 = pk2(w01, w01), p10 = pk2(w10, w10), p11 = pk2(w11, w11);
#pragma unroll
      for (int k = 0; k < NP; ++k) {
        u64 r = mul2(t00[v].v[k], p00);
        r = fma2(t01[v].v[k], p01, r);
        r = fma2(t10[v].v[k], p10, r);
        r = fma2(t11[v].v[k], p11, r);
        S[k] = add2(S[k], r);
        Q[k] = fma2(r, r, Q[k]);
      }
    }
    u64 o[NP];
#pragma unroll
    for (int k = 0; k < NP; ++k) {
      const u64 m = mul2(S[k], inv_v2), mn = mul2(S[k], ninv_v2);
      o[k] = fma2(mn, m, mul2(Q[k], inv_v2));
    }
    if (round_tf32) {
#pragma unroll
      for (int k = 0; k < NP; ++k) {
        float lo, hi;
        unpk2(o[k], lo, hi);
        o[k] = pk2(round_tf32_f(lo), round_tf32_f(hi));
      }
    }
    if (active) stg_tex<CPT>(optr, o);
    optr += (size_t)hw * C;
  }
}

template <int NSRC, int CT>
static bool launch_var(cudaStream_t st, const float* f, const float* p, const float* dv,
                       float* cost, int B, int D, int h, int w, int dchunk, int rnd) {
  const long threads = (long)h * w * (CT / 8);
  dim3 grd((unsigned)((threads + kK1Threads - 1) / kK1Threads), (unsigned)B,
           (unsigned)((D + dchunk - 1) / dchunk));
  warp_var_kernel<NSRC, CT, 8, false, 6><<<grd, kK1Threads, 0, st>>>(f, p, dv, cost, D, h, w, dchunk, rnd);
  return true;
}

template <bool OUT_NHWC>
__global__ void __launch_bounds__(kK1Threads)
homo_warp_kernel(const float* __restrict__ src,
                 const float* __restrict__ proj,
                 const float* __restrict__ dv, float* __restrict__ out, int C, int D, int h,
                 int w) {
  const int b = blockIdx.y;
  const float* P = proj + (size_t)b * 12;
  const int tpp = C / kCPT;
  const int gtid = blockIdx.x * blockDim.x + threadIdx.x;
  const int pix = gtid / tpp;
  const int c0 = (gtid - pix * tpp) * kCPT;
  const int hw = h * w;
  if (pix >= hw) return;
  const int y = pix / w, x = pix - y * w;
  const float xf = (float)x, yf = (float)y;
  const float ax = fmaf(P[0], xf, fmaf(P[1], yf, P[2]));
  const float ay = fmaf(P[4], xf, fmaf(P[5], yf, P[6]));
  const float az = fmaf(P[8], xf, fmaf(P[9], yf, P[10]));
  const float* sb = src + (size_t)b * hw * C + c0;
  for (int d = 0; d < D; ++d) {
    const float inv_d = __frcp_rn(__ldg(dv + ((size_t)b * D + d) * hw + pix));
    Taps t = make_taps(fmaf(P[3], inv_d, ax), fmaf(P[7], inv_d, ay), fmaf(P[11], inv_d, az),
                       h, w, C);
    float r[kCPT];
#pragma unroll
    for (int k = 0; k < kCPT; ++k) r[k] = 0.f;
    if (t.any) blend8(sb, t, r);
    if (OUT_NHWC) {
      float* op = out + ((size_t)(b * D + d) * hw + pix) * C + c0;
      st4(op, make_float4(r[0], r[1], r[2], r[3]));
      st4(op + 4, make_float4(r[4], r[5], r[6], r[7]));
    } else {
#pragma unroll
      for (int k = 0; k < kCPT; ++k) out[((size_t)(b * C + c0 + k) * D + d) * hw + pix] = r[k];
    }
  }
}

__global__ void transpose_rs_kernel(const float* __restrict__ in, float* __restrict__ out,
                                    size_t R, size_t S, unsigned tiles_s) {
  __shared__ float tile[32][33];
  const size_t n = blockIdx.y;
  const float* ip = in + n * R * S;
  float* op = out + n * R * S;
  const size_t s0 = (size_t)(blockIdx.x % tiles_s) * 32;
  const size_t r0 = (size_t)(blockIdx.x / tiles_s) * 32;
  for (int j = threadIdx.y; j < 32; j += blockDim.y) {
    size_t r = r0 + j, s = s0 + threadIdx.x;
    tile[j][threadIdx.x] = (r < R && s < S) ? ip[r * S + s] : 0.f;
  }
  __syncthreads();
  for (int j = threadIdx.y; j < 32; j += blockDim.y) {
    size_t s = s0 + j, r = r0 + threadIdx.x;
    if (r < R && s < S) op[s * R + r] = tile[threadIdx.x][j];
  }
}

static int launch_transpose(const float* in, float* out, int N, size_t R, size_t S,
                            cudaStream_t st, const char* what) {
  if (N == 0 || R == 0 || S == 0) return 0;
  dim3 blk(32, 8);
  size_t tiles_s = (S + 31) / 32, tiles_r = (R + 31) / 32;
  CASMVS_REQUIRE(tiles_s * tiles_r < (1ull << 31) && N <= 65535, "%s: dims too large", what);
  dim3 grd((unsigned)(tiles_s * tiles_r), (unsigned)N);
  transpose_rs_kernel<<<grd, blk, 0, st>>>(in, out, R, S, (unsigned)tiles_s);
  return after_launch(what);
}

int g_k1_dchunk = 0;

int warp_var_smem(const float* feats, const float* proj, const Hyp& dv, float* cost, int B,
                  int V, int C, int D, int h, int w, int num_groups, int rnd, cudaStream_t st);

template <int NSRC, int CT>
static void launch_k1(bool gwc, bool nhwc, dim3 grd, cudaStream_t st, const float* f,
                      const float* p, const float* dv, float* cost, int V, int C, int D, int h,
                      int w, int G, int dchunk, int rnd) {
  if (gwc) {
    if (nhwc) warp_cost_kernel<NSRC, CT, true, true><<<grd, kK1Threads, 0, st>>>(f, p, dv, cost, V, C, D, h, w, G, dchunk, rnd);
    else warp_cost_kernel<NSRC, CT, true, false><<<grd, kK1Threads, 0, st>>>(f, p, dv, cost, V, C, D, h, w, G, dchunk, rnd);
  } else {
    if (nhwc) warp_cost_kernel<NSRC, CT, false, true><<<grd, kK1Threads, 0, st>>>(f, p, dv, cost, V, C, D, h, w, G, dchunk, rnd);
    else warp_cost_kernel<NSRC, CT, false, false><<<grd, kK1Threads, 0, st>>>(f, p, dv, cost, V, C, D, h, w, G, dchunk, rnd);
  }
}

template <int NSRC>
static void launch_k1_c(bool gwc, bool nhwc, dim3 grd, cudaStream_t st, const float* f,
                        const float* p, const float* dv, float* cost, int V, int C, int D, int h,
                        int w, int G, int dchunk, int rnd) {
  switch (C) {
    case 8: launch_k1<NSRC, 8>(gwc, nhwc, grd, st, f, p, dv, cost, V, C, D, h, w, G, dchunk, rnd); break;
    case 16: launch_k1<NSRC, 16>(gwc, nhwc, grd, st, f, p, dv, cost, V, C, D, h, w, G, dchunk, rnd); break;
    case 32: launch_k1<NSRC, 32>(gwc, nhwc, grd, st, f, p, dv, cost, V, C, D, h, w, G, dchunk, rnd); break;
    default: launch_k1<NSRC, 0>(gwc, nhwc, grd, st, f, p, dv, cost, V, C, D, h, w, G, dchunk, rnd); break;
  }
}

}

using namespace casmvs;

extern "C" size_t casmvs_warp_cost_workspace_bytes(int feat_layout, int B, int V, int C, int h,
                                                   int w) {
  if (feat_layout == CASMVS_NHWC) return 0;
  return (size_t)B * V * C * h * w * sizeof(float);
}

extern "C" int casmvs_warp_cost_fwd(const float* feats, int feat_layout, const float* proj,
                                    const float* depth_values, float* cost, int cost_layout,
                                    int B, int V, int C, int D, int h, int w, int num_groups,
                                    void* workspace, size_t workspace_bytes, void* stream) {
  CASMVS_REQUIRE(feats && proj && depth_values && cost, "warp_cost: null pointer");
  CASMVS_REQUIRE(B >= 0 && V >= 2 && C > 0 && D > 0 && h >= 2 && w >= 2, "warp_cost: bad dims (h,w >= 2)");
  CASMVS_REQUIRE(V - 1 <= kMaxSrc, "warp_cost: at most %d source views", kMaxSrc);
  CASMVS_REQUIRE(C % kCPT == 0, "warp_cost: C must be a multiple of %d (got %d)", kCPT, C);
  CASMVS_REQUIRE(C / kCPT <= 32 && (32 % (C / kCPT)) == 0, "warp_cost: C/8 must divide 32");
  CASMVS_REQUIRE(num_groups >= 1 && C % num_groups == 0, "warp_cost: C %% num_groups != 0");
  const bool gwc = num_groups > 1;
  if (gwc) {
    int cpg = C / num_groups;
    CASMVS_REQUIRE((cpg & (cpg - 1)) == 0, "warp_cost: C/num_groups must be a power of two");
  }
  CASMVS_REQUIRE((size_t)h * w * C < (1u << 31), "warp_cost: view too large for 32-bit offsets");
  CASMVS_REQUIRE(B <= 65535, "warp_cost: B too large");
  if (B == 0) return 0;
  cudaStream_t st = as_stream(stream);
  const float* f = feats;
  if (feat_layout == CASMVS_NCHW) {
    size_t need = casmvs_warp_cost_workspace_bytes(feat_layout, B, V, C, h, w);
    CASMVS_REQUIRE(workspace && workspace_bytes >= need,
                   "warp_cost: workspace too small (%zu < %zu)", workspace_bytes, need);
    int rc = launch_transpose(feats, (float*)workspace, B * V, (size_t)C, (size_t)h * w, st,
                              "warp_cost/nchw_to_nhwc");
    if (rc) return rc;
    f = (const float*)workspace;
  } else {
    CASMVS_REQUIRE(feat_layout == CASMVS_NHWC, "warp_cost: bad feat_layout");
  }
  const int rnd = (cost_layout & CASMVS_ROUND_TF32) ? 1 : 0;
  cost_layout &= ~CASMVS_ROUND_TF32;
  CASMVS_REQUIRE(cost_layout == CASMVS_NCHW || cost_layout == CASMVS_NHWC,
                 "warp_cost: bad cost_layout");
  const bool nhwc = cost_layout == CASMVS_NHWC;
  const long threads = (long)h * w * (C / kCPT);
  const unsigned xblocks = (unsigned)((threads + kK1Threads - 1) / kK1Threads);
  static bool env_read = false;
  if (!env_read) {
    env_read = true;
    if (const char* e = getenv("CASMVS_K1_DCHUNK")) g_k1_dchunk = atoi(e);
  }
  int dchunk = D;
  if (g_k1_dchunk > 0) dchunk = g_k1_dchunk;
  else {
    const long want_ctas = (long)num_sms() * 16;
    while (dchunk > 8 && (long)xblocks * B * ((D + dchunk - 1) / dchunk) < want_ctas)
      dchunk = (dchunk + 1) / 2;
  }
  if (nhwc) {
    const Hyp hyp{depth_values, nullptr, nullptr, nullptr, 0.f, 0.f};
    const int rc = warp_var_smem(f, proj, hyp, cost, B, V, C, D, h, w, num_groups, rnd, st);
    if (rc <= 0) return rc;
  }
  if (!gwc && nhwc && (V == 3 || V == 2) && (C == 8 || C == 16 || C == 32)) {
    bool ok = false;
    if (V == 3) {
      if (C == 8) ok = launch_var<2, 8>(st, f, proj, depth_values, cost, B, D, h, w, dchunk, rnd);
      else if (C == 16) ok = launch_var<2, 16>(st, f, proj, depth_values, cost, B, D, h, w, dchunk, rnd);
      else ok = launch_var<2, 32>(st, f, proj, depth_values, cost, B, D, h, w, dchunk, rnd);
    } else {
      if (C == 8) ok = launch_var<1, 8>(st, f, proj, depth_values, cost, B, D, h, w, dchunk, rnd);
      else if (C == 16) ok = launch_var<1, 16>(st, f, proj, depth_values, cost, B, D, h, w, dchunk, rnd);
      else ok = launch_var<1, 32>(st, f, proj, depth_values, cost, B, D, h, w, dchunk, rnd);
    }
    if (ok) return after_launch("warp_cost");
  }
  dim3 grd(xblocks, (unsigned)B, (unsigned)((D + dchunk - 1) / dchunk));
  switch (V - 1) {
    case 1: launch_k1_c<1>(gwc, nhwc, grd, st, f, proj, depth_values, cost, V, C, D, h, w, num_groups, dchunk, rnd); break;
    case 2: launch_k1_c<2>(gwc, nhwc, grd, st, f, proj, depth_values, cost, V, C, D, h, w, num_groups, dchunk, rnd); break;
    case 4: launch_k1_c<4>(gwc, nhwc, grd, st, f, proj, depth_values, cost, V, C, D, h, w, num_groups, dchunk, rnd); break;
    case 6: launch_k1_c<6>(gwc, nhwc, grd, st, f, proj, depth_values, cost, V, C, D, h, w, num_groups, dchunk, rnd); break;
    default: launch_k1<0, 0>(gwc, nhwc, grd, st, f, proj, depth_values, cost, V, C, D, h, w, num_groups, dchunk, rnd); break;
  }
  return after_launch("warp_cost");
}

extern "C" int casmvs_homo_warp_fwd(const float* src_feat, int feat_layout, const float* proj,
                                    const float* depth_values, float* warped, int out_layout,
                                    int B, int C, int D, int h, int w, void* stream) {
  CASMVS_REQUIRE(src_feat && proj && depth_values && warped, "homo_warp: null pointer");
  CASMVS_REQUIRE(feat_layout == CASMVS_NHWC,
                 "homo_warp: features must be channels-last (use casmvs_nchw_to_nhwc)");
  CASMVS_REQUIRE(C % kCPT == 0 && B >= 0 && B <= 65535 && D > 0 && h > 0 && w > 0,
                 "homo_warp: bad dims");
  CASMVS_REQUIRE((size_t)h * w * C < (1u << 31), "homo_warp: view too large");
  if (B == 0) return 0;
  const long threads = (long)h * w * (C / kCPT);
  dim3 grd((unsigned)((threads + kK1Threads - 1) / kK1Threads), (unsigned)B);
  cudaStream_t st = as_stream(stream);
  if (out_layout == CASMVS_NHWC)
    homo_warp_kernel<true><<<grd, kK1Threads, 0, st>>>(src_feat, proj, depth_values, warped, C, D, h, w);
  else
    homo_warp_kernel<false><<<grd, kK1Threads, 0, st>>>(src_feat, proj, depth_values, warped, C, D, h, w);
  return after_launch("homo_warp");
}

extern "C" int casmvs_nchw_to_nhwc(const float* in, float* out, int N, int C, size_t S,
                                   void* stream) {
  CASMVS_REQUIRE(in && out, "nchw_to_nhwc: null pointer");
  return launch_transpose(in, out, N, (size_t)C, S, as_stream(stream), "nchw_to_nhwc");
}

extern "C" int casmvs_nhwc_to_nchw(const float* in, float* out, int N, int C, size_t S,
                                   void* stream) {
  CASMVS_REQUIRE(in && out, "nhwc_to_nchw: null pointer");
  return launch_transpose(in, out, N, S, (size_t)C, as_stream(stream), "nhwc_to_nchw");
}

extern "C" int casmvs_warp_cost_ladder_fwd(const float* feats, const float* proj,
                                           const float* first_map, const float* first_b,
                                           float first, const float* step_b, float step, float* cost,
                                           int round_tf32, int B, int V, int C, int D, int h, int w,
                                           int num_groups, void* stream) {
  CASMVS_REQUIRE(feats && proj && cost, "warp_cost_ladder: null pointer");
  CASMVS_REQUIRE(B >= 0 && B <= 65535 && V >= 2 && C > 0 && D > 0 && h >= 2 && w >= 2,
                 "warp_cost_ladder: bad dims (h,w >= 2)");
  CASMVS_REQUIRE((size_t)h * w * C < (1u << 31), "warp_cost_ladder: view too large");
  if (B == 0) return 0;
  const Hyp hyp{nullptr, first_map, first_b, step_b, first, step};
  const int rc = warp_var_smem(feats, proj, hyp, cost, B, V, C, D, h, w, num_groups,
                               round_tf32 ? 1 : 0, as_stream(stream));
  if (rc == 1) {
    set_error("warp_cost_ladder: shape not covered by the staged kernel (V-1 in {1,2}, C in "
              "{8,16,32}, groups 1 or 8, channels-last features): materialise the hypotheses and "
              "call casmvs_warp_cost_fwd (got V=%d C=%d G=%d)", V, C, num_groups);
    return -1;
  }
  return rc;
}
```

### casmvsnet_pl_b200/csrc/warp_cost_smem.cu

```cuda
#include <limits.h>
#include <stdlib.h>

#include <mutex>

#include "k1_common.cuh"
#include "tma_common.cuh"

namespace casmvs {
namespace k1s {

using tc::fence_barrier_init;
using tc::mbar_init;
using tc::mbar_wait;
using tc::smem_u32;

constexpr int kMaxSrcSmem = 6;
constexpr float kMagic = 12582912.f;
constexpr int kMagicBits = 0x4B400000;

__device__ __forceinline__ float fadd_rd(float a, float b) { return __fadd_rd(a, b); }

template <int TEXB>
__device__ __forceinline__ uint32_t swz(uint32_t off) {
  constexpr uint32_t m = (TEXB == 128 ? 7u : TEXB == 64 ? 3u : 1u) << 4;
  return off ^ ((off >> 3) & m);
}
__device__ __forceinline__ void lds_tex(uint32_t addr, Tex8& t) {
  asm volatile("ld.shared.v2.b64 {%0,%1}, [%2];" : "=l"(t.v[0]), "=l"(t.v[1]) : "r"(addr));
  asm volatile("ld.shared.v2.b64 {%0,%1}, [%2];" : "=l"(t.v[2]), "=l"(t.v[3]) : "r"(addr ^ 16u));
}

struct Small {
  float proj[kMaxSrcSmem * 12];
  int mm[kMaxSrcSmem * 4];
  int box[kMaxSrcSmem * 2];
  unsigned long long bar;
};

template <int CP> struct TexP { u64 v[CP / 2]; };
template <int CP>
__device__ __forceinline__ void lds_texp(uint32_t addr, TexP<CP>& t) {
#pragma unroll
  for (int k = 0; k < CP / 4; ++k)
    asm volatile("ld.shared.v2.b64 {%0,%1}, [%2];" : "=l"(t.v[2 * k]), "=l"(t.v[2 * k + 1])
                 : "r"(addr ^ (16u * k)));
}
template <int CP>
__device__ __forceinline__ TexP<CP> ldg_texp(const float* p) {
  TexP<CP> t;
#pragma unroll
  for (int k = 0; k < CP / 8; ++k) {
    const Tex8 a = ldg256(p + 8 * k);
#pragma unroll
    for (int j = 0; j < 4; ++j) t.v[4 * k + j] = a.v[j];
  }
  return t;
}

template <int NSRC, int C, int TW, int TH, int MINB, bool GWC = false, int CP = 8>
__global__ void __launch_bounds__(TW* TH*(C / CP), MINB)
warp_var_smem_kernel(const __grid_constant__ CUtensorMap fmap, const float* __restrict__ feats,
                     const float* __restrict__ proj, const Hyp hyp,
                     float* __restrict__ cost, int D, int h, int w, int dchunk, int BW, int BH,
                     int box_stride, int tiles_x, int round_tf32) {
  constexpr int V = NSRC + 1, TPP = C / CP, TEXB = C * 4, NT = TW * TH * TPP, NP = CP / 2;
  static_assert(!GWC || CP == 8, "group-wise correlation is built for 8 channels per thread");
  constexpr int CPG = C / 8, NG = kCPT / CPG, COUT = GWC ? 8 : C;
  extern __shared__ uint8_t smem_raw[];
  const uint32_t base = (smem_u32(smem_raw) + 1023u) & ~1023u;
  Small* sm = reinterpret_cast<Small*>(smem_raw + (base - smem_u32(smem_raw)) + NSRC * box_stride);
  const uint32_t bar = smem_u32(&sm->bar);

  const int tid = threadIdx.x;
  const int b = blockIdx.y;
  const int tile_y = blockIdx.x / tiles_x, tile_x = blockIdx.x - tile_y * tiles_x;
  const int lp = tid / TPP, sub = tid - lp * TPP;
  const int py = lp / TW, px = lp - py * TW;
  const int xr = tile_x * TW + px, yr = tile_y * TH + py;
  const bool active = xr < w && yr < h;
  const int x = min(xr, w - 1), y = min(yr, h - 1);
  const int c0 = sub * CP;
  const int hw = h * w, pix = y * w + x;

  for (int i = tid; i < NSRC * 12; i += NT) sm->proj[i] = proj[(size_t)b * NSRC * 12 + i];
  if (tid == 0) {
    mbar_init(bar, 1);
    fence_barrier_init();
  }
  __syncthreads();

  const float xf = (float)x, yf = (float)y;
  float ax[NSRC], ay[NSRC], az[NSRC], tx[NSRC], ty[NSRC], tz[NSRC];
#pragma unroll
  for (int v = 0; v < NSRC; ++v) {
    const float* P = sm->proj + v * 12;
    ax[v] = fmaf(P[0], xf, fmaf(P[1], yf, P[2]));
    ay[v] = fmaf(P[4], xf, fmaf(P[5], yf, P[6]));
    az[v] = fmaf(P[8], xf, fmaf(P[9], yf, P[10]));
    tx[v] = P[3]; ty[v] = P[7]; tz[v] = P[11];
  }
  const size_t view_stride = (size_t)hw * C;
  const float* fb = feats + (size_t)b * V * view_stride + c0;
  const TexP<CP> ref = ldg_texp<CP>(fb + (size_t)pix * C);
  const float inv_v = 1.f / (float)V;
  const u64 inv_v2 = pk2(inv_v, inv_v), ninv_v2 = pk2(-inv_v, -inv_v);

  const int d_begin = blockIdx.z * dchunk;
  const int d_end = min(D, d_begin + dchunk);
  const HypPix hp(hyp, b, D, (size_t)hw, pix);
  float* optr = cost + ((size_t)(b * D + d_begin) * hw + pix) * COUT + (GWC ? sub * NG : c0);
  const int row_b = BW * TEXB;

  uint32_t phase = 0;

  for (int d0 = d_begin; d0 < d_end;) {
    int n = d_end - d0;
    int bx[NSRC], by[NSRC];
    for (;;) {
      __syncthreads();
      if (tid < NSRC * 4) sm->mm[tid] = (tid & 2) ? INT_MIN : INT_MAX;
      __syncthreads();
      const float ia = rcp_approx(hp.at(d0));
      const float ib = rcp_approx(hp.at(d0 + n - 1));
#pragma unroll
      for (int v = 0; v < NSRC; ++v) {
        int mnx = INT_MAX, mny = INT_MAX, mxx = INT_MIN, mxy = INT_MIN;
#pragma unroll
        for (int e = 0; e < 2; ++e) {
          const float id = e ? ib : ia;
          const float qz = fmaf(tz[v], id, az[v]);
          const float rz = rcp_approx(qz);
          const float u = fmaf(tx[v], id, ax[v]) * rz, vv = fmaf(ty[v], id, ay[v]) * rz;
          if (active && qz > 1e-7f && u > -2.f && u < (float)(w + 1) && vv > -2.f &&
              vv < (float)(h + 1)) {
            const int xi = __float2int_rd(u), yi = __float2int_rd(vv);
            mnx = min(mnx, xi); mxx = max(mxx, xi);
            mny = min(mny, yi); mxy = max(mxy, yi);
          }
        }
        mnx = __reduce_min_sync(0xffffffffu, mnx); mny = __reduce_min_sync(0xffffffffu, mny);
        mxx = __reduce_max_sync(0xffffffffu, mxx); mxy = __reduce_max_sync(0xffffffffu, mxy);
        if ((tid & 31) == 0) {
          atomicMin(&sm->mm[v * 4 + 0], mnx); atomicMin(&sm->mm[v * 4 + 1], mny);
          atomicMax(&sm->mm[v * 4 + 2], mxx); atomicMax(&sm->mm[v * 4 + 3], mxy);
        }
      }
      __syncthreads();
      bool fits = true;
#pragma unroll
      for (int v = 0; v < NSRC; ++v) {
        const int mnx = sm->mm[v * 4 + 0], mny = sm->mm[v * 4 + 1];
        const int mxx = sm->mm[v * 4 + 2], mxy = sm->mm[v * 4 + 3];
        if (mnx > mxx) { bx[v] = 0; by[v] = 0; continue; }
        const int sx = mxx + 2 - mnx, sy = mxy + 2 - mny;
        if (sx > BW || sy > BH) fits = false;
        bx[v] = mnx - max(0, (BW - sx) >> 1);
        by[v] = mny - max(0, (BH - sy) >> 1);
      }
      if (fits || n == 1) break;
      n = (n + 1) >> 1;
    }
    if (tid == 0) {
      tma::mbar_expect_tx(bar, (uint32_t)(NSRC * BW * BH * TEXB));
#pragma unroll
      for (int v = 0; v < NSRC; ++v)
        tma::tma_load_4d(base + v * box_stride, &fmap, bar, 0, bx[v], by[v], b * V + v + 1);
    }
    int kx[NSRC], ky[NSRC];
#pragma unroll
    for (int v = 0; v < NSRC; ++v) {
      kx[v] = kMagicBits + bx[v]; ky[v] = kMagicBits + by[v];
    }
    float depth_next = hp.at(d0);
    mbar_wait(bar, phase);
    phase ^= 1;

    for (int d = d0; d < d0 + n; ++d) {
      const float inv_d = rcp_approx(depth_next);
      if (d + 1 < d0 + n) depth_next = hp.at(d + 1);
      u64 S[NP], Q[NP];
#pragma unroll
      for (int k = 0; k < NP; ++k) {
        S[k] = GWC ? 0ull : ref.v[k];
        Q[k] = mul2(ref.v[k], ref.v[k]);
      }
#pragma unroll
      for (int v = 0; v < NSRC; ++v) {
        const float qx = fmaf(tx[v], inv_d, ax[v]);
        const float qy = fmaf(ty[v], inv_d, ay[v]);
        const float qz = fmaf(tz[v], inv_d, az[v]);
        const float rz = rcp_approx(qz);
        const float u = qx * rz, vv = qy * rz;
        const float fu = fadd_rd(u, kMagic), fv = fadd_rd(vv, kMagic);
        const int xi = __float_as_int(fu) - kx[v], yi = __float_as_int(fv) - ky[v];
        const bool inbox = (unsigned)xi < (unsigned)(BW - 1) && (unsigned)yi < (unsigned)(BH - 1) &&
                           qz > 1e-7f;
        u64 r[NP];
        if (__builtin_expect(inbox, 1)) {
          const float fx = u - (fu - kMagic), fy = vv - (fv - kMagic);
          const float wxa = 1.f - fx, wya = 1.f - fy;
          const int l00 = v * box_stride + yi * row_b + xi * TEXB + c0 * 4;
          TexP<CP> t00, t01, t10, t11;
          lds_texp<CP>(base + swz<TEXB>(l00), t00);
          lds_texp<CP>(base + swz<TEXB>(l00 + TEXB), t01);
          lds_texp<CP>(base + swz<TEXB>(l00 + row_b), t10);
          lds_texp<CP>(base + swz<TEXB>(l00 + row_b + TEXB), t11);
          const float w00 = wxa * wya, w01 = fx * wya, w10 = wxa * fy, w11 = fx * fy;
          const u64 p00 = pk2(w00, w00), p01 = pk2(w01, w01), p10 = pk2(w10, w10),
                    p11 = pk2(w11, w11);
#pragma unroll
          for (int k = 0; k < NP; ++k) {
            u64 a = mul2(t00.v[k], p00);
            a = fma2(t01.v[k], p01, a);
            a = fma2(t10.v[k], p10, a);
            r[k] = fma2(t11.v[k], p11, a);
          }
        } else if (qz <= 1e-7f || u <= -1.f || u >= (float)w || vv <= -1.f || vv >= (float)h) {
          continue;
        } else {
#pragma unroll
          for (int hh = 0; hh < CP / 8; ++hh) {
            Window win;
            float w00, w01, w10, w11;
            sample_view<C>(fb + (size_t)(v + 1) * view_stride + 8 * hh, qx, qy, qz, h, w, C, w * C,
                           win, w00, w01, w10, w11);
            const u64 p00 = pk2(w00, w00), p01 = pk2(w01, w01), p10 = pk2(w10, w10),
                      p11 = pk2(w11, w11);
#pragma unroll
            for (int k = 0; k < 4; ++k) {
              u64 a = mul2(win.t00.v[k], p00);
              a = fma2(win.t01.v[k], p01, a);
              a = fma2(win.t10.v[k], p10, a);
              r[4 * hh + k] = fma2(win.t11.v[k], p11, a);
            }
          }
        }
#pragma unroll
        for (int k = 0; k < NP; ++k) {
          S[k] = add2(S[k], r[k]);
          if (!GWC) Q[k] = fma2(r[k], r[k], Q[k]);
        }
      }
      if constexpr (GWC) {
        float pr[kCPT], o[NG];
#pragma unroll
        for (int k = 0; k < NP; ++k) unpk2(mul2(S[k], ref.v[k]), pr[2 * k], pr[2 * k + 1]);
#pragma unroll
        for (int k = 0; k < NG; ++k) {
          float acc = CPG == 1 ? pr[k] : CPG == 2 ? pr[2 * k] + pr[2 * k + 1]
                      : (pr[4 * k] + pr[4 * k + 1]) + (pr[4 * k + 2] + pr[4 * k + 3]);
          float val = __fdiv_rn(acc * (1.f / (float)CPG), (float)NSRC);
          o[k] = round_tf32 ? round_tf32_f(val) : val;
        }
        if (active) {
          if constexpr (NG == 8) {
            u64 ov[4] = {pk2(o[0], o[1]), pk2(o[2], o[3]), pk2(o[4], o[5]), pk2(o[6], o[7])};
            stg256(optr, ov);
          } else if constexpr (NG == 4) {
            st4(optr, make_float4(o[0], o[1], o[2], o[3]));
          } else {
            *reinterpret_cast<float2*>(optr) = make_float2(o[0], o[1]);
          }
        }
        optr += (size_t)hw * COUT;
        continue;
      }
      u64 o[NP];
#pragma unroll
      for (int k = 0; k < NP; ++k) {
        const u64 m = mul2(S[k], inv_v2), mn = mul2(S[k], ninv_v2);
        o[k] = fma2(mn, m, mul2(Q[k], inv_v2));
      }
      if (round_tf32) {
#pragma unroll
        for (int k = 0; k < NP; ++k) {
          float lo, hi;
          unpk2(o[k], lo, hi);
          o[k] = pk2(round_tf32_f(lo), round_tf32_f(hi));
        }
      }
      if (active) {
#pragma unroll
        for (int hh = 0; hh < CP / 8; ++hh) {
          const u64 oo[4] = {o[4 * hh], o[4 * hh + 1], o[4 * hh + 2], o[4 * hh + 3]};
          stg256(optr + 8 * hh, oo);
        }
      }
      optr += (size_t)hw * C;
    }
    d0 += n;
  }
}

template <int C, int TW, int TH, int PG, int MINB>
__global__ void __launch_bounds__(TW* TH*(C / kCPT), MINB)
warp_var_smem_pg_kernel(const __grid_constant__ CUtensorMap fmap, const float* __restrict__ feats,
                        const float* __restrict__ proj, const Hyp hyp, float* __restrict__ cost,
                        int D, int h, int w, int dchunk, int BW, int BH, int box_stride, int tiles_x,
                        int round_tf32) {
  constexpr int NSRC = 2, V = 3, TPP = C / kCPT, TEXB = C * 4, NT = TW * TH * TPP;
  extern __shared__ uint8_t smem_raw[];
  const uint32_t base = (smem_u32(smem_raw) + 1023u) & ~1023u;
  Small* sm = reinterpret_cast<Small*>(smem_raw + (base - smem_u32(smem_raw)) + NSRC * box_stride);
  const uint32_t bar = smem_u32(&sm->bar);
  const int tid = threadIdx.x;
  const int b = blockIdx.y;
  const int tile_y = blockIdx.x / tiles_x, tile_x = blockIdx.x - tile_y * tiles_x;
  const int lp = tid / TPP, sub = tid - lp * TPP;
  const int py = lp / TW, px = lp - py * TW;
  const int xr = tile_x * TW + px, yr = tile_y * TH + py;
  const bool active = xr < w && yr < h;
  const int x = min(xr, w - 1), y = min(yr, h - 1);
  const int c0 = sub * kCPT;
  const int hw = h * w, pix = y * w + x;

  for (int i = tid; i < NSRC * 12; i += NT) sm->proj[i] = proj[(size_t)b * NSRC * 12 + i];
  if (tid == 0) {
    mbar_init(bar, 1);
    fence_barrier_init();
  }
  __syncthreads();
  const float xf = (float)x, yf = (float)y;
  float ax[NSRC], ay[NSRC], az[NSRC], tx[NSRC], ty[NSRC], tz[NSRC];
#pragma unroll
  for (int v = 0; v < NSRC; ++v) {
    const float* P = sm->proj + v * 12;
    ax[v] = fmaf(P[0], xf, fmaf(P[1], yf, P[2]));
    ay[v] = fmaf(P[4], xf, fmaf(P[5], yf, P[6]));
    az[v] = fmaf(P[8], xf, fmaf(P[9], yf, P[10]));
    tx[v] = P[3]; ty[v] = P[7]; tz[v] = P[11];
  }
  const size_t view_stride = (size_t)hw * C;
  const float* fb = feats + (size_t)b * V * view_stride + c0;
  const Tex8 ref = ldg256(fb + (size_t)pix * C);
  const float inv_v = 1.f / (float)V;
  const u64 inv_v2 = pk2(inv_v, inv_v), ninv_v2 = pk2(-inv_v, -inv_v);
  const int d_begin = blockIdx.z * dchunk;
  const int d_end = min(D, d_begin + dchunk);
  const HypPix hp(hyp, b, D, (size_t)hw, pix);
  float* optr = cost + ((size_t)(b * D + d_begin) * hw + pix) * C + c0;
  const int row_b = BW * TEXB;
  const bool rowal = (row_b & 1023) == 0;
  u64 refsq[4];
#pragma unroll
  for (int k = 0; k < 4; ++k) refsq[k] = mul2(ref.v[k], ref.v[k]);
  uint32_t phase = 0;

  for (int d0 = d_begin; d0 < d_end;) {
    int n = d_end - d0;
    int bx[NSRC], by[NSRC];
    for (;;) {
      __syncthreads();
      if (tid < NSRC * 4) sm->mm[tid] = (tid & 2) ? INT_MIN : INT_MAX;
      __syncthreads();
      const float ia = rcp_approx(hp.at(d0));
      const float ib = rcp_approx(hp.at(d0 + n - 1));
#pragma unroll
      for (int v = 0; v < NSRC; ++v) {
        int mnx = INT_MAX, mny = INT_MAX, mxx = INT_MIN, mxy = INT_MIN;
#pragma unroll
        for (int e = 0; e < 2; ++e) {
          const float id = e ? ib : ia;
          const float qz = fmaf(tz[v], id, az[v]);
          const float rz = rcp_approx(qz);
          const float u = fmaf(tx[v], id, ax[v]) * rz, vv = fmaf(ty[v], id, ay[v]) * rz;
          if (active && qz > 1e-7f && u > -2.f && u < (float)(w + 1) && vv > -2.f &&
              vv < (float)(h + 1)) {
            const int xi = __float2int_rd(u), yi = __float2int_rd(vv);
            mnx = min(mnx, xi); mxx = max(mxx, xi);
            mny = min(mny, yi); mxy = max(mxy, yi);
          }
        }
        mnx = __reduce_min_sync(0xffffffffu, mnx); mny = __reduce_min_sync(0xffffffffu, mny);
        mxx = __reduce_max_sync(0xffffffffu, mxx); mxy = __reduce_max_sync(0xffffffffu, mxy);
        if ((tid & 31) == 0) {
          atomicMin(&sm->mm[v * 4 + 0], mnx); atomicMin(&sm->mm[v * 4 + 1], mny);
          atomicMax(&sm->mm[v * 4 + 2], mxx); atomicMax(&sm->mm[v * 4 + 3], mxy);
        }
      }
      __syncthreads();
      bool fits = true;
#pragma unroll
      for (int v = 0; v < NSRC; ++v) {
        const int mnx = sm->mm[v * 4 + 0], mny = sm->mm[v * 4 + 1];
        const int mxx = sm->mm[v * 4 + 2], mxy = sm->mm[v * 4 + 3];
        if (mnx > mxx) { bx[v] = 0; by[v] = 0; continue; }
        const int sx = mxx + 2 - mnx, sy = mxy + 2 - mny;
        if (sx > BW || sy > BH) fits = false;
        bx[v] = mnx - max(0, (BW - sx) >> 1);
        by[v] = mny - max(0, (BH - sy) >> 1);
      }
      if (fits || n == 1) break;
      n = (n + 1) >> 1;
    }
    if (tid == 0) {
      tma::mbar_expect_tx(bar, (uint32_t)(NSRC * BW * BH * TEXB));
#pragma unroll
      for (int v = 0; v < NSRC; ++v)
        tma::tma_load_4d(base + v * box_stride, &fmap, bar, 0, bx[v], by[v], b * V + v + 1);
    }
    int kx[NSRC], ky[NSRC];
#pragma unroll
    for (int v = 0; v < NSRC; ++v) { kx[v] = kMagicBits + bx[v]; ky[v] = kMagicBits + by[v]; }
    float dnext[PG];
#pragma unroll
    for (int p = 0; p < PG; ++p) dnext[p] = hp.at(min(d0 + p, d0 + n - 1));
    mbar_wait(bar, phase);
    phase ^= 1;

    for (int d = d0; d < d0 + n; d += PG) {
      float inv_d[PG];
#pragma unroll
      for (int p = 0; p < PG; ++p) {
        inv_d[p] = rcp_approx(dnext[p]);
        dnext[p] = hp.at(min(d + PG + p, d0 + n - 1));
      }
      u64 r1[PG][4];
#pragma unroll
      for (int v = 0; v < NSRC; ++v) {
        Tex8 t00, t01, t10, t11;
        int cur = -1;
#pragma unroll
        for (int p = 0; p < PG; ++p) {
          const float qx = fmaf(tx[v], inv_d[p], ax[v]);
          const float qy = fmaf(ty[v], inv_d[p], ay[v]);
          const float qz = fmaf(tz[v], inv_d[p], az[v]);
          const float rz = rcp_approx(qz);
          const float u = qx * rz, vv = qy * rz;
          const float fu = fadd_rd(u, kMagic), fv = fadd_rd(vv, kMagic);
          const int xi = __float_as_int(fu) - kx[v], yi = __float_as_int(fv) - ky[v];
          const bool inbox = (unsigned)xi < (unsigned)(BW - 1) && (unsigned)yi < (unsigned)(BH - 1) &&
                             qz > 1e-7f;
          u64 r[4] = {0ull, 0ull, 0ull, 0ull};
          if (__builtin_expect(inbox, 1)) {
            const float fx = u - (fu - kMagic), fy = vv - (fv - kMagic);
            const float wxa = 1.f - fx, wya = 1.f - fy;
            const int l00 = v * box_stride + yi * row_b + xi * TEXB + c0 * 4;
            if (l00 != cur) {
              const uint32_t a0 = base + swz<TEXB>(l00), a1 = base + swz<TEXB>(l00 + TEXB);
              lds_tex(a0, t00);
              lds_tex(a1, t01);
              lds_tex(rowal ? a0 + row_b : base + swz<TEXB>(l00 + row_b), t10);
              lds_tex(rowal ? a1 + row_b : base + swz<TEXB>(l00 + row_b + TEXB), t11);
              cur = l00;
            }
            const float w00 = wxa * wya, w01 = fx * wya, w10 = wxa * fy, w11 = fx * fy;
            const u64 p00 = pk2(w00, w00), p01 = pk2(w01, w01), p10 = pk2(w10, w10),
                      p11 = pk2(w11, w11);
#pragma unroll
            for (int k = 0; k < 4; ++k) {
              u64 a = mul2(t00.v[k], p00);
              a = fma2(t01.v[k], p01, a);
              a = fma2(t10.v[k], p10, a);
              r[k] = fma2(t11.v[k], p11, a);
            }
          } else if (!(qz <= 1e-7f || u <= -1.f || u >= (float)w || vv <= -1.f || vv >= (float)h)) {
            Window win;
            float w00, w01, w10, w11;
            sample_view<C>(fb + (size_t)(v + 1) * view_stride, qx, qy, qz, h, w, C, w * C, win, w00,
                           w01, w10, w11);
            const u64 p00 = pk2(w00, w00), p01 = pk2(w01, w01), p10 = pk2(w10, w10),
                      p11 = pk2(w11, w11);
#pragma unroll
            for (int k = 0; k < 4; ++k) {
              u64 a = mul2(win.t00.v[k], p00);
              a = fma2(win.t01.v[k], p01, a);
              a = fma2(win.t10.v[k], p10, a);
              r[k] = fma2(win.t11.v[k], p11, a);
            }
          }
          if (v == 0) {
#pragma unroll
            for (int k = 0; k < 4; ++k) r1[p][k] = r[k];
          } else if (d + p < d0 + n) {
            u64 o[4];
#pragma unroll
            for (int k = 0; k < 4; ++k) {
              const u64 S = add2(add2(ref.v[k], r1[p][k]), r[k]);
              const u64 Q = fma2(r[k], r[k], fma2(r1[p][k], r1[p][k], refsq[k]));
              const u64 m = mul2(S, inv_v2), mn = mul2(S, ninv_v2);
              o[k] = fma2(mn, m, mul2(Q, inv_v2));
            }
            if (round_tf32) {
#pragma unroll
              for (int k = 0; k < 4; ++k) {
                float lo, hi;
                unpk2(o[k], lo, hi);
                o[k] = pk2(round_tf32_f(lo), round_tf32_f(hi));
              }
            }
            if (active) stg256(optr + (size_t)p * hw * C, o);
          }
        }
      }
      optr += (size_t)PG * hw * C;
    }
    optr -= (size_t)(((n + PG - 1) / PG) * PG - n) * hw * C;
    d0 += n;
  }
}

struct MapEntry { const void* p; int BV, h, w, C, BW, BH; CUtensorMap map; };
static MapEntry g_maps[32];
static int g_maps_n = 0, g_maps_next = 0;
static std::mutex g_maps_mu;

static bool feature_map(CUtensorMap* out, const float* feats, int BV, int h, int w, int C, int BW,
                        int BH) {
  std::lock_guard<std::mutex> lock(g_maps_mu);
  for (int i = 0; i < g_maps_n; ++i) {
    const MapEntry& e = g_maps[i];
    if (e.p == feats && e.BV == BV && e.h == h && e.w == w && e.C == C && e.BW == BW && e.BH == BH) {
      *out = e.map;
      return true;
    }
  }
  const uint64_t dims[4] = {(uint64_t)C, (uint64_t)w, (uint64_t)h, (uint64_t)BV};
  const uint64_t str[3] = {(uint64_t)C * 4, (uint64_t)w * C * 4, (uint64_t)h * w * C * 4};
  const uint32_t box[4] = {(uint32_t)C, (uint32_t)BW, (uint32_t)BH, 1};
  MapEntry e{feats, BV, h, w, C, BW, BH, {}};
  if (tma::encode_tiled(&e.map, feats, 4, dims, str, box, C * 4)) return false;
  g_maps[g_maps_next] = e;
  g_maps_next = (g_maps_next + 1) % 32;
  if (g_maps_n < 32) ++g_maps_n;
  *out = e.map;
  return true;
}

static int env_int(const char* name, int dflt) {
  const char* e = getenv(name);
  return e ? atoi(e) : dflt;
}

template <int NSRC, int C, int TW, int TH, int MINB, bool GWC = false, int CP = 8>
static int launch(const float* feats, const float* proj, const Hyp& dv, float* cost, int B, int D,
                  int h, int w, int rnd, cudaStream_t st) {
  constexpr int NT = TW * TH * (C / CP);
  static const int mx = env_int("CASMVS_K1_MARGIN_X", NSRC <= 2 ? 16 : 8);
  static const int my = env_int("CASMVS_K1_MARGIN_Y", NSRC <= 2 ? 4 : 3);
  static const int dc_env = env_int("CASMVS_K1S_DCHUNK", 0);
  const int BW = TW + mx, BH = TH + my;
  const int box_stride = (BW * BH * C * 4 + 1023) & ~1023;
  const size_t smem = (size_t)NSRC * box_stride + sizeof(Small) + 1024;
  auto kfn = warp_var_smem_kernel<NSRC, C, TW, TH, MINB, GWC, CP>;
  static std::atomic<bool> attr_set[kMaxDevices];
  if (int rc = opt_in_smem(kfn, 200 * 1024, attr_set, "warp_cost")) return rc;
  if (smem > 200 * 1024) return 1;
  CUtensorMap map;
  if (!feature_map(&map, feats, B * (NSRC + 1), h, w, C, BW, BH)) return -2;
  const int tiles_x = (w + TW - 1) / TW, tiles_y = (h + TH - 1) / TH;
  int dchunk = dc_env > 0 ? dc_env : (D <= 16 ? D : 16);
  while (dc_env <= 0 && dchunk > 4 &&
         (long)tiles_x * tiles_y * B * ((D + dchunk - 1) / dchunk) < (long)num_sms() * 8)
    dchunk = (dchunk + 1) / 2;
  dim3 grd((unsigned)(tiles_x * tiles_y), (unsigned)B, (unsigned)((D + dchunk - 1) / dchunk));
  kfn<<<grd, NT, smem, st>>>(map, feats, proj, dv, cost, D, h, w, dchunk, BW, BH, box_stride,
                             tiles_x, rnd);
  return after_launch("warp_cost(smem)");
}

template <int C, int TW, int TH, int PG, int MINB>
static int launch_pg(const float* feats, const float* proj, const Hyp& dv, float* cost, int B, int D,
                     int h, int w, int rnd, cudaStream_t st) {
  constexpr int NSRC = 2, NT = TW * TH * (C / kCPT);
  static const int mx = env_int("CASMVS_K1_MARGIN_X", 16);
  static const int my = env_int("CASMVS_K1_MARGIN_Y", 4);
  static const int dc_env = env_int("CASMVS_K1S_DCHUNK", 0);
  const int wq = 1024 / (C * 4);
  const int BW = (TW + mx + wq - 1) / wq * wq, BH = TH + my;
  const int box_stride = (BW * BH * C * 4 + 1023) & ~1023;
  const size_t smem = (size_t)NSRC * box_stride + sizeof(Small) + 1024;
  auto kfn = warp_var_smem_pg_kernel<C, TW, TH, PG, MINB>;
  static std::atomic<bool> attr_set[kMaxDevices];
  if (int rc = opt_in_smem(kfn, 200 * 1024, attr_set, "warp_cost")) return rc;
  if (smem > 200 * 1024) return 1;
  CUtensorMap map;
  if (!feature_map(&map, feats, B * (NSRC + 1), h, w, C, BW, BH)) return -2;
  const int tiles_x = (w + TW - 1) / TW, tiles_y = (h + TH - 1) / TH;
  int dchunk = dc_env > 0 ? dc_env : (D <= 16 ? D : 16);
  while (dc_env <= 0 && dchunk > 4 &&
         (long)tiles_x * tiles_y * B * ((D + dchunk - 1) / dchunk) < (long)num_sms() * 8)
    dchunk = (dchunk + 1) / 2;
  dim3 grd((unsigned)(tiles_x * tiles_y), (unsigned)B, (unsigned)((D + dchunk - 1) / dchunk));
  kfn<<<grd, NT, smem, st>>>(map, feats, proj, dv, cost, D, h, w, dchunk, BW, BH, box_stride,
                             tiles_x, rnd);
  return after_launch("warp_cost(smem,pg)");
}

}

int warp_var_smem(const float* feats, const float* proj, const Hyp& dv, float* cost, int B,
                  int V, int C, int D, int h, int w, int num_groups, int rnd, cudaStream_t st) {
  static const int enabled = k1s::env_int("CASMVS_K1_SMEM", 1);
  if (!enabled) return 1;
  if ((reinterpret_cast<uintptr_t>(feats) & 15) != 0 || B > 65535) return 1;
  using namespace k1s;
  static const int many = env_int("CASMVS_K1S_MANYVIEWS", 0);
  if (V - 1 > 2 && !many) return 1;
  if (num_groups != 1) {
    if (num_groups != 8) return 1;
#define K1G(NS, CC, TW_, TH_, MB) \
  if (V - 1 == NS && C == CC) return launch<NS, CC, TW_, TH_, MB, true>(feats, proj, dv, cost, B, D, h, w, rnd, st);
    K1G(1, 8, 32, 4, 5) K1G(1, 16, 32, 2, 5) K1G(1, 32, 16, 2, 5)
    K1G(2, 8, 32, 4, 5) K1G(2, 16, 32, 2, 5) K1G(2, 32, 16, 2, 5)
    K1G(4, 8, 32, 4, 4) K1G(4, 16, 32, 4, 2) K1G(4, 32, 16, 4, 2)
#undef K1G
    return 1;
  }
  static const int variant = env_int("CASMVS_K1S_VARIANT", 16);
#define K1S(VAR, NS, CC, TW_, TH_, MB) \
  if (variant == VAR && V - 1 == NS && C == CC) return launch<NS, CC, TW_, TH_, MB>(feats, proj, dv, cost, B, D, h, w, rnd, st);
#define K1P(VAR, CC, TW_, TH_, PG_, MB) \
  if (variant == VAR && V - 1 == 2 && C == CC) return launch_pg<CC, TW_, TH_, PG_, MB>(feats, proj, dv, cost, B, D, h, w, rnd, st);
  K1P(16, 8, 32, 4, 2, 4) K1P(16, 16, 32, 2, 2, 4) K1P(16, 32, 16, 2, 2, 4)
  K1P(11, 8, 32, 4, 4, 4) K1P(11, 16, 32, 2, 4, 4) K1P(11, 32, 16, 2, 4, 4)
  K1S(4, 2, 8, 32, 4, 5) K1S(4, 2, 16, 32, 2, 5) K1S(4, 2, 32, 16, 2, 5)
#undef K1P
  if (V - 1 == 2) return 1;
  K1S(variant, 1, 8, 32, 4, 5) K1S(variant, 1, 16, 32, 2, 5) K1S(variant, 1, 32, 16, 2, 5)
  K1S(variant, 4, 8, 32, 4, 4) K1S(variant, 4, 16, 32, 4, 2) K1S(variant, 4, 32, 16, 4, 2)
  K1S(variant, 6, 8, 32, 4, 4) K1S(variant, 6, 16, 32, 4, 2) K1S(variant, 6, 32, 16, 4, 2)
#undef K1S
  return 1;
}

}
```

### casmvsnet_pl_b200/models/mvsnet.py

```python
import torch
import torch.nn as nn
import torch.nn.functional as F

from .. import ops
from ..norm_act import activation_slope, folded_scale_shift
from .modules import *
from .modules import ConvBnReLU, ConvBnReLU3D, InPlaceABN


class FeatureNet(nn.Module):

    def __init__(self, norm_act=InPlaceABN):
        super().__init__()
        self.conv0 = nn.Sequential(ConvBnReLU(3, 8, 3, 1, 1, norm_act=norm_act),
                                   ConvBnReLU(8, 8, 3, 1, 1, norm_act=norm_act))
        self.conv1 = nn.Sequential(ConvBnReLU(8, 16, 5, 2, 2, norm_act=norm_act),
                                   ConvBnReLU(16, 16, 3, 1, 1, norm_act=norm_act),
                                   ConvBnReLU(16, 16, 3, 1, 1, norm_act=norm_act))
        self.conv2 = nn.Sequential(ConvBnReLU(16, 32, 5, 2, 2, norm_act=norm_act),
                                   ConvBnReLU(32, 32, 3, 1, 1, norm_act=norm_act),
                                   ConvBnReLU(32, 32, 3, 1, 1, norm_act=norm_act))
        self.toplayer = nn.Conv2d(32, 32, 1)
        self.lat1 = nn.Conv2d(16, 32, 1)
        self.lat0 = nn.Conv2d(8, 32, 1)
# ... 109 lines not shown
    def _forward_folded(self, x):
        cache = self._folded()
        if not x.is_cuda:
            x = x.contiguous(memory_format=torch.channels_last)

            def run(t, lo, hi):
                for w, b, stride, pad, slope in cache[lo:hi]:
                    t = F.leaky_relu_(F.conv2d(t, w, b, stride, pad), slope)
                return t
            c0 = run(x, 0, 2)
            c1 = run(c0, 2, 5)
            c2 = run(c1, 5, 8)
            return self._head(c0, c1, c2)
        packed = self._packed_fp32()

        def planar(t, i):
            w, b, _, _, slope = cache[i]
            return ops.conv2d_planar(t, packed[i], w.shape[1], w.shape[0], b, slope, ops.FP32)

        def strided(t, i):
            _, b, _, _, slope = cache[i]
            return ops.conv2d_5x5s2_fp32(t, packed[i], b, slope)

        w0, b0, _, _, slope0 = cache[0]
        c0 = planar(ops.conv2d_rgb8(x, w0, b0, slope0), 1)
        c1 = planar(planar(strided(c0, 2), 3), 4)
        c2 = planar(planar(strided(c1, 5), 6), 7)
        return self._head(c0, c1, c2)

    def _packed_fp32(self):
        key = self._fold_key
        if getattr(self, "_pack32_key", None) != key:
            cache = self._fold_cache
            packed = {i: ops.pack_conv3d_weight(cache[i][0].contiguous(), ops.CONV_PLANAR)
                      for i in (1, 3, 4, 6, 7)}
            for i in (2, 5):
                packed[i] = cache[i][0].detach().contiguous(memory_format=torch.contiguous_format).clone()
            self._pack32_cache, self._pack32_key = packed, key
        return self._pack32_cache

    def _forward_modules(self, x):
        x = x.contiguous(memory_format=torch.channels_last)
        c0 = self.conv0(x)
        c1 = self.conv1(c0)
        c2 = self.conv2(c1)
        return self._head(c0, c1, c2)

    def _head(self, c0, c1, c2):
        if c0.is_cuda and not (self.training or torch.is_grad_enabled()):
            f2 = ops.fpn_merge(None, c2, self.toplayer.weight, self.toplayer.bias)
        else:
            f2 = self.toplayer(c2)
        if c0.is_cuda and not (self.training or torch.is_grad_enabled()):
            f1, l1 = ops.fpn_level(f2, c1, self.lat1.weight, self.lat1.bias,
                                   self.smooth1.weight, self.smooth1.bias, want_feat=True)
            _, l0 = ops.fpn_level(f1, c0, self.lat0.weight, self.lat0.bias,
                                  self.smooth0.weight, self.smooth0.bias, want_feat=False)
            return {"level_0": l0, "level_1": l1,
                    "level_2": f2.contiguous(memory_format=torch.channels_last)}
        f1 = self._up2(f2) + self.lat1(c1)
        f0 = self._up2(f1) + self.lat0(c0)
        f1 = self.smooth1(f1)
        f0 = self.smooth0(f0)
        return {"level_0": f0.contiguous(memory_format=torch.channels_last),
                "level_1": f1.contiguous(memory_format=torch.channels_last),
                "level_2": f2.contiguous(memory_format=torch.channels_last)}


class CostRegNet(nn.Module):

    _ORDER = ("conv0", "conv1", "conv2", "conv3", "conv4", "conv5", "conv6",
              "conv7", "conv9", "conv11", "prob")

    def __init__(self, in_channels, norm_act=InPlaceABN):
        super().__init__()
        self.in_channels = in_channels
        self.conv0 = ConvBnReLU3D(in_channels, 8, norm_act=norm_act)
        self.conv1 = ConvBnReLU3D(8, 16, stride=2, norm_act=norm_act)
        self.conv2 = ConvBnReLU3D(16, 16, norm_act=norm_act)
        self.conv3 = ConvBnReLU3D(16, 32, stride=2, norm_act=norm_act)
        self.conv4 = ConvBnReLU3D(32, 32, norm_act=norm_act)
        self.conv5 = ConvBnReLU3D(32, 64, stride=2, norm_act=norm_act)
        self.conv6 = ConvBnReLU3D(64, 64, norm_act=norm_act)

        def up(cin, cout):
            return nn.Sequential(nn.ConvTranspose3d(cin, cout, 3, padding=1, output_padding=1,
                                                    stride=2, bias=False), norm_act(cout))
        self.conv7 = up(64, 32)
        self.conv9 = up(32, 16)
        self.conv11 = up(16, 8)
        self.prob = nn.Conv3d(8, 1, 3, stride=1, padding=1)
        self.precision = "fp32"
        self._blob = None
        self._blob_key = None

    def _layer_tensors(self, name):
        m = getattr(self, name)
        if name == "prob":
            return m.weight, None, m.bias
        if isinstance(m, ConvBnReLU3D):
            return m.conv.weight, m.bn, None
        return m[0].weight, m[1], None

    def _norm_modules(self):
        for name in self._ORDER[:-1]:
            yield self._layer_tensors(name)[1]

    def packed_params(self):
        key = tuple((t.data_ptr(), t._version) for t in
                    list(self.parameters()) + list(self.buffers()))
        if key == self._blob_key:
            return self._blob
        dev = self.prob.weight.device
        if self._blob is not None:
            ops.release_weight_images(self._blob)
        n = ops._lib.load().casmvs_costreg_param_floats(self.in_channels)
        blob = torch.empty(n, device=dev, dtype=torch.float32)
        ops.release_weight_images(blob)
        for i, name in enumerate(self._ORDER):
            info = ops.costreg_layer_info(self.in_channels, i)
            w, bn, bias = self._layer_tensors(name)
            wp = ops.pack_conv3d_weight(w, info["kind"])
            blob[info["w_off"]:info["w_off"] + wp.numel()] = wp
            co = info["cout"]
            if bn is not None:
                a, b = folded_scale_shift(bn)
            else:
                a = torch.ones(co, device=dev)
                b = bias.detach().float()
            blob[info["scale_off"]:info["scale_off"] + co] = a
            blob[info["shift_off"]:info["shift_off"] + co] = b
        self._blob, self._blob_key = blob, key
        return blob

    def _forward_autograd(self, x):
        from .. import autograd as AG
        prec = ops.PRECISIONS[self.precision]

        def cbr(m, t, stride=1):
            return m.bn(AG.conv3d(t, m.conv.weight, ops.CONV, stride, prec))

        def up(m, t):
            return m[1](AG.conv3d(t, m[0].weight, ops.CONV_TRANSPOSE, 2, prec))

        conv0 = cbr(self.conv0, x)
        conv2 = cbr(self.conv2, cbr(self.conv1, conv0, 2))
        conv4 = cbr(self.conv4, cbr(self.conv3, conv2, 2))
        x = cbr(self.conv6, cbr(self.conv5, conv4, 2))
        x = conv4 + up(self.conv7, x)
        x = conv2 + up(self.conv9, x)
        x = conv0 + up(self.conv11, x)
        return AG.conv3d(x, self.prob.weight, ops.CONV, 1, prec) + self.prob.bias.view(1, -1, 1, 1, 1)

    def forward(self, x):
        if torch.is_grad_enabled() and (x.requires_grad or
                                        any(p.requires_grad for p in self.parameters())):
            return self._forward_autograd(x)
        for bn in self._norm_modules():
            if bn.training:
                raise ops._lib.CasMVSError("CostRegNet inference path needs .eval() (training "
                                           "runs through the autograd path: enable grad)")
            if abs(activation_slope(bn) - 0.01) > 1e-12:
                raise ops._lib.CasMVSError("casmvs_costreg_fwd assumes LeakyReLU(0.01) norm_act")
        logits = ops.costreg(x, self.packed_params(), self.in_channels,
                             ops.PRECISIONS[self.precision])
        return logits.unsqueeze(1)


class CascadeMVSNet(nn.Module):
    def __init__(self, n_depths=[8, 32, 48], interval_ratios=[1, 2, 4], num_groups=1,
                 norm_act=InPlaceABN, precision="fp32"):
        super().__init__()
        self.levels = 3
        self.n_depths = n_depths
        self.interval_ratios = interval_ratios
        self.G = num_groups
        self.feature = FeatureNet(norm_act)
        import os
        self.overlap_pyramid = os.environ.get("CASMVS_OVERLAP", "1") != "0"
        self.return_index = False
        self._last_index = None
        self.fuse_hypotheses = os.environ.get("CASMVS_LADDER", "1") != "0"
        for l in range(self.levels):
            cin = self.G if self.G > 1 else 8 * 2 ** l
            setattr(self, f"cost_reg_{l}", CostRegNet(cin, norm_act))
        self.set_precision(precision)

    def set_precision(self, precision):
        if precision not in ops.PRECISIONS:
            raise ValueError(f"precision must be one of {list(ops.PRECISIONS)}")
        self.precision = precision
        for m in self.modules():
            if isinstance(m, (CostRegNet, ConvBnReLU3D)):
                m.precision = precision
        self.feature.allow_tf32 = precision == "tf32"
        return self

    def predict_depth(self, feats, proj_mats, depth_values, cost_reg):
        if torch.is_grad_enabled() and (feats.requires_grad or
                                        any(p.requires_grad for p in cost_reg.parameters())):
            from .. import autograd as AG
            cost = AG.warp_cost(feats, proj_mats, depth_values, self.G)
            logits = cost_reg(cost).squeeze(1)
            return AG.regress(logits, depth_values)
        cost = ops.warp_cost(feats, proj_mats, depth_values, self.G, ops.NHWC,
                             round_tf32=(getattr(cost_reg, "precision", "fp32") == "tf32"))
        logits = cost_reg(cost).squeeze(1)
        del cost
        depth, confidence, index, _ = ops.regress(logits, depth_values,
                                                  want_index=self.return_index)
        self._last_index = index
        return depth, confidence

    def _forward_autograd(self, imgs, proj_mats, init_depth_min, depth_interval):
        B, V, _, H, W = imgs.shape
        torch.backends.cudnn.allow_tf32 = self.precision == "tf32"
        feats = self.feature(imgs.reshape(B * V, 3, H, W))
        proj_by_level = proj_mats.permute(2, 0, 1, 3, 4).contiguous()
        results = {}
        depth_l = None
        for l in reversed(range(self.levels)):
            feats_l = feats[f"level_{l}"]
            feats_l = feats_l.view(B, V, *feats_l.shape[1:])
            depth_interval_l = depth_interval * self.interval_ratios[l]
            D = self.n_depths[l]
            h, w = feats_l.shape[-2:]
            with torch.no_grad():
                if l == self.levels - 1:
                    depth_values = ops.uniform_hypotheses(init_depth_min, depth_interval_l, D, B,
                                                          h, w, imgs.device)
                else:
                    depth_values = ops.depth_hypotheses(depth_l.detach(), D, depth_interval_l,
                                                        upsample=True)
            depth_l, confidence_l = self.predict_depth(feats_l, proj_by_level[l], depth_values,
                                                       getattr(self, f"cost_reg_{l}"))
            results[f"depth_{l}"] = depth_l
            results[f"confidence_{l}"] = confidence_l
        return results

    def packed_buffers(self):
        bufs = []
        for l in range(self.levels):
            b = getattr(self, f"cost_reg_{l}")._blob
            if b is not None:
                bufs.append(b)
        f = self.feature
        bufs += list(getattr(f, "_pack_cache", {}).values()) + list(getattr(f, "_smooth_pack", ()))
        return [b for b in bufs if torch.is_tensor(b) and b.is_cuda]

    def run_stage(self, l, feats_l, proj_mats_l, depth_prev, init_depth_min, depth_interval):
        B, V, C, h, w = feats_l.shape
        D = self.n_depths[l]
        depth_interval_l = depth_interval * self.interval_ratios[l]
        cost_reg = getattr(self, f"cost_reg_{l}")
        if self.fuse_hypotheses and ops.ladder_supported(V, C, self.G) and \
                ops.is_channels_last_feats(feats_l):
            first = init_depth_min if depth_prev is None else ops.depth_first(depth_prev, D, depth_interval_l)
            lad = ops.Ladder(first, depth_interval_l, D, B, h, w, feats_l.device)
            cost = ops.warp_cost_ladder(feats_l, proj_mats_l, lad, self.G,
                                        round_tf32=(cost_reg.precision == "tf32"))
            logits = cost_reg(cost).squeeze(1)
            del cost
            depth, confidence, self._last_index = ops.regress_ladder(logits, lad,
                                                                     want_index=self.return_index)
            return depth, confidence
        if depth_prev is None:
            depth_values = ops.uniform_hypotheses(init_depth_min, depth_interval_l, D, B, h, w,
                                                  feats_l.device)
        else:
            depth_values = ops.depth_hypotheses(depth_prev, D, depth_interval_l, upsample=True)
        return self.predict_depth(feats_l, proj_mats_l, depth_values, cost_reg)

    def forward(self, imgs, proj_mats, init_depth_min, depth_interval):
        B, V, _, H, W = imgs.shape
        if not imgs.is_cuda:
            raise ops._lib.CasMVSError(
                "CascadeMVSNet (H100 engine) needs CUDA inputs; there is no CPU fallback")
        differentiable = torch.is_grad_enabled() and (
            imgs.requires_grad or any(p.requires_grad for p in self.parameters()))
        if torch.is_tensor(init_depth_min):
            init_depth_min = init_depth_min.to(imgs.device, torch.float32)
        if torch.is_tensor(depth_interval):
            depth_interval = depth_interval.to(imgs.device, torch.float32)
        if differentiable:
            return self._forward_autograd(imgs, proj_mats, init_depth_min, depth_interval)
        results = {}
        with torch.no_grad():
            feats = self.feature(imgs.reshape(B * V, 3, H, W), overlap=self.overlap_pyramid)
            ready = feats.get("_ready", {})
            proj_by_level = proj_mats.permute(2, 0, 1, 3, 4).contiguous()
            depth_l = None
            for l in reversed(range(self.levels)):
                if l in ready:
                    torch.cuda.current_stream(imgs.device).wait_event(ready[l])
                feats_l = feats[f"level_{l}"]
                feats_l = feats_l.view(B, V, *feats_l.shape[1:])
                proj_mats_l = proj_by_level[l]
                depth_l, confidence_l = self.run_stage(l, feats_l, proj_mats_l, depth_l,
                                                       init_depth_min, depth_interval)
                results[f"depth_{l}"] = depth_l
                results[f"confidence_{l}"] = confidence_l
                if self.return_index:
                    results[f"depth_index_{l}"] = self._last_index
        return results
```

### casmvsnet_pl_b200/ops.py

```python
from __future__ import annotations

import ctypes
import functools
import math

import torch

from . import _lib
from ._lib import (CONV, CONV_PLANAR, CONV_TRANSPOSE, FP32, KEEP_FP32_OUT, NCHW, NHWC, PRECISIONS, TF32,
                   check)

_checked_devices = set()


def _stream():
    return ctypes.c_void_p(torch.cuda.current_stream().cuda_stream)


def _on_tensor_device(fn):
    @functools.wraps(fn)
    def wrapper(*args, **kw):
        dev = kw.get("device")
        if dev is None:
            dev = next((a.device for a in args if torch.is_tensor(a) and a.is_cuda), None)
        else:
            dev = torch.device(dev)
        if dev is None or dev.type != "cuda" or dev.index is None or \
                dev.index == torch.cuda.current_device():
            return fn(*args, **kw)
        with torch.cuda.device(dev):
            return fn(*args, **kw)
    return wrapper


def _ptr(t):
    return ctypes.c_void_p(t.data_ptr()) if t is not None else None


def _require_cuda(*tensors):
    for t in tensors:
        if t is None:
            continue
        if not t.is_cuda:
            raise _lib.CasMVSError(
                "casmvsnet_pl_b200 ops need CUDA tensors on a H100 (no CPU fallback); "
                f"got a tensor on {t.device}")
        if t.dtype != torch.float32:
            raise _lib.CasMVSError(f"fp32 only (reference opt.py:69-70), got {t.dtype}")
    first = next((t for t in tensors if t is not None), None)
    if first is None:
        return
    for t in tensors:
        if t is not None and t.device != first.device:
            raise _lib.CasMVSError(f"tensors on different devices: {first.device} and {t.device}")
    dev = first.device.index
    if dev is None:
        dev = torch.cuda.current_device()
    if dev not in _checked_devices:
        check(_lib.load().casmvs_device_check(dev), "device_check")
        _checked_devices.add(dev)


def _no_grad_only(*tensors):
    if torch.is_grad_enabled() and any(t is not None and t.requires_grad for t in tensors):
        raise _lib.CasMVSError(
            "the H100 engine is forward-only this round (SURVEY.md §8f-1): call it under "
            "torch.no_grad() or with tensors that do not require grad")


def is_channels_last_feats(feats):
    C, h, w = feats.shape[-3:]
    st = feats.stride()
    if not (st[-3] == 1 and st[-1] == C and st[-2] == w * C):
        return False
    expect = h * w * C
    for size, s in zip(reversed(feats.shape[:-3]), reversed(st[:-3])):
        if size != 1 and s != expect:
            return False
        expect *= size
    return True


def as_volume_view(buf_ndhwc):
    return buf_ndhwc.permute(0, 4, 1, 2, 3)


def volume_storage(x):
    v = x.permute(0, 2, 3, 4, 1)
    return v if v.is_contiguous() else v.contiguous()


@_on_tensor_device
def warp_cost(feats, proj_mats, depth_values, num_groups=1, out_layout=NHWC, round_tf32=False):
    _require_cuda(feats, proj_mats, depth_values)
    _no_grad_only(feats)
    B, V, C, h, w = feats.shape
    D = depth_values.shape[1]
    lib = _lib.load()
    if is_channels_last_feats(feats):
        flayout, fbuf = NHWC, feats
    else:
        flayout, fbuf = NCHW, feats.contiguous()
    proj = proj_mats.contiguous()
    dv = depth_values.contiguous()
    assert proj.shape == (B, V - 1, 3, 4) and dv.shape == (B, D, h, w)
    cout = C if num_groups == 1 else num_groups
    ws_bytes = lib.casmvs_warp_cost_workspace_bytes(flayout, B, V, C, h, w)
    ws = torch.empty(ws_bytes // 4, device=feats.device, dtype=torch.float32) if ws_bytes else None
    if out_layout == NHWC:
        out = torch.empty(B, D, h, w, cout, device=feats.device, dtype=torch.float32)
    else:
        out = torch.empty(B, cout, D, h, w, device=feats.device, dtype=torch.float32)
    check(lib.casmvs_warp_cost_fwd(_ptr(fbuf), flayout, _ptr(proj), _ptr(dv), _ptr(out),
                                   out_layout | (_lib.ROUND_TF32 if round_tf32 else 0),
                                   B, V, C, D, h, w, num_groups, _ptr(ws),
                                   ws_bytes, _stream()), "warp_cost")
    return as_volume_view(out) if out_layout == NHWC else out


@_on_tensor_device
def homo_warp(src_feat, proj_mat, depth_values):
    _require_cuda(src_feat, proj_mat, depth_values)
    _no_grad_only(src_feat)
    B, C, h, w = src_feat.shape
    D = depth_values.shape[1]
    lib = _lib.load()
    if is_channels_last_feats(src_feat):
        fbuf = src_feat
    else:
        fbuf = torch.empty(B, h, w, C, device=src_feat.device, dtype=torch.float32)
        check(lib.casmvs_nchw_to_nhwc(_ptr(src_feat.contiguous()), _ptr(fbuf), B, C, h * w,
                                      _stream()), "nchw_to_nhwc")
    out = torch.empty(B, C, D, h, w, device=src_feat.device, dtype=torch.float32)
    check(lib.casmvs_homo_warp_fwd(_ptr(fbuf), NHWC, _ptr(proj_mat.contiguous()),
                                   _ptr(depth_values.contiguous()), _ptr(out), NCHW,
                                   B, C, D, h, w, _stream()), "homo_warp")
    return out


def invalidate_weight_cache():
    check(_lib.load().casmvs_invalidate_weight_cache(), "invalidate_weight_cache")


def release_weight_images(packed):
    check(_lib.load().casmvs_release_weight_images(_ptr(packed), packed.numel() * packed.element_size()),
          "release_weight_images")


@_on_tensor_device
def pack_conv3d_weight(weight, kind):
    _require_cuda(weight)
    if kind == CONV_PLANAR:
        assert weight.dim() == 4 and tuple(weight.shape[2:]) == (3, 3)
    if kind in (CONV, CONV_PLANAR):
        cout, cin = weight.shape[:2]
    else:
        cin, cout = weight.shape[:2]
    out = torch.empty(27 * cin * cout, device=weight.device, dtype=torch.float32)
    release_weight_images(out)
    check(_lib.load().casmvs_pack_conv3d_weights(_ptr(weight.detach().contiguous()), kind, cin,
                                                 cout, _ptr(out), _stream()), "pack_conv3d")
    return out


@_on_tensor_device
def conv3d(x, w_packed, cin, cout, scale=None, shift=None, slope=1.0, skip=None,
           kind=CONV, stride=1, precision=FP32):
    _require_cuda(x, w_packed, scale, shift, skip)
    _no_grad_only(x)
    xs = volume_storage(x)
    B, D, h, w, _ = xs.shape
    if kind == CONV_PLANAR:
        assert stride == 1
        Do, ho, wo = D, h, w
    elif kind == CONV:
        Do, ho, wo = (D - 1) // stride + 1, (h - 1) // stride + 1, (w - 1) // stride + 1
    else:
        Do, ho, wo = 2 * D, 2 * h, 2 * w
    y = torch.empty(B, Do, ho, wo, cout, device=x.device, dtype=torch.float32)
    sk = volume_storage(skip) if skip is not None else None
    check(_lib.load().casmvs_conv3d_fwd(_ptr(xs), _ptr(w_packed), _ptr(scale), _ptr(shift),
                                        float(slope), _ptr(sk), _ptr(y), B, cin, cout, D, h, w,
                                        kind, stride, precision, _stream()), "conv3d")
    return as_volume_view(y)


def costreg_layer_info(cin, layer):
    lib = _lib.load()
    ci, co, kind, stride = (ctypes.c_int() for _ in range(4))
    wo, so, ho = (ctypes.c_size_t() for _ in range(3))
    check(lib.casmvs_costreg_layer_info(cin, layer, ci, co, kind, stride, wo, so, ho),
          "costreg_layer_info")
    return dict(cin=ci.value, cout=co.value, kind=kind.value, stride=stride.value,
                w_off=wo.value, scale_off=so.value, shift_off=ho.value)


@_on_tensor_device
def costreg(x, params, cin, precision=FP32):
    _require_cuda(x, params)
    _no_grad_only(x)
    xs = volume_storage(x)
    B, D, h, w, c = xs.shape
    assert c == cin
    lib = _lib.load()
    ws_bytes = lib.casmvs_costreg_workspace_bytes(B, cin, D, h, w)
    ws = torch.empty(ws_bytes // 4, device=x.device, dtype=torch.float32)
    logits = torch.empty(B, D, h, w, device=x.device, dtype=torch.float32)
    check(lib.casmvs_costreg_fwd(_ptr(xs), _ptr(params), _ptr(logits), B, cin, D, h, w,
                                 precision, _ptr(ws), ws_bytes, _stream()), "costreg")
    return logits


@_on_tensor_device
def regress(logits, depth_values, input_is_prob=False, want_index=False, want_prob=False):
    _require_cuda(logits, depth_values)
    _no_grad_only(logits)
    lg = logits.contiguous()
    B, D, h, w = lg.shape
    dv_vec = depth_values.dim() == 1
    dv = depth_values.contiguous()
    depth = torch.empty(B, h, w, device=lg.device, dtype=torch.float32)
    conf = torch.empty_like(depth)
    index = torch.empty(B, h, w, device=lg.device, dtype=torch.int64) if want_index else None
    prob = torch.empty_like(lg) if want_prob else None
    check(_lib.load().casmvs_regress_fwd(_ptr(lg), _ptr(dv), int(dv_vec), int(input_is_prob),
                                         _ptr(depth), _ptr(conf), _ptr(index), _ptr(prob),
                                         B, D, h, w, _stream()), "regress")
    return depth, conf, index, prob


def _interval_args(depth_interval, B, device):
    if isinstance(depth_interval, (float, int)):
        return float(depth_interval), None
    t = depth_interval.reshape(-1).to(device=device, dtype=torch.float32).contiguous()
    if t.numel() == 1 and B > 1:
        t = t.expand(B).contiguous()
    assert t.numel() == B
    return 0.0, t


@_on_tensor_device
def depth_hypotheses(current_depth, n_depths, depth_interval, upsample=False):
    _require_cuda(current_depth)
    cur = current_depth.contiguous()
    if upsample:
        B, hi, wi = cur.shape
        h, w = 2 * hi, 2 * wi
    else:
        B, _, h, w = cur.shape
    step, step_dev = _interval_args(depth_interval, B, cur.device)
    half = float(n_depths / 2 * step)
    out = torch.empty(B, n_depths, h, w, device=cur.device, dtype=torch.float32)
    check(_lib.load().casmvs_depth_hypotheses_fwd(_ptr(cur), int(upsample), half, step,
                                                  _ptr(step_dev), _ptr(out), B, n_depths, h, w,
                                                  _stream()), "depth_hypotheses")
    return out


def uniform_hypotheses(init_depth_min, depth_interval, n_depths, B, h, w, device):
    with torch.cuda.device(device):
        return _uniform_hypotheses(init_depth_min, depth_interval, n_depths, B, h, w, device)


def _uniform_hypotheses(init_depth_min, depth_interval, n_depths, B, h, w, device):
    dmin, dmin_dev = _interval_args(init_depth_min, B, device)
    step, step_dev = _interval_args(depth_interval, B, device)
    out = torch.empty(B, n_depths, h, w, device=device, dtype=torch.float32)
    check(_lib.load().casmvs_uniform_hypotheses_fwd(dmin, step, _ptr(dmin_dev), _ptr(step_dev),
                                                    _ptr(out), B, n_depths, h, w, _stream()),
          "uniform_hypotheses")
    return out


class Ladder:

    def __init__(self, first, step, D, B, h, w, device):
        self.first, self.step, self.D, self.B, self.h, self.w, self.device = first, step, D, B, h, w, device

    def _args(self):
        fm = fb = sb = None
        f = s = 0.0
        if torch.is_tensor(self.first):
            if self.first.dim() == 3:
                fm = self.first.contiguous()
            else:
                fb = self.first.reshape(-1).contiguous()
        else:
            f = float(self.first)
        if torch.is_tensor(self.step):
            sb = self.step.reshape(-1).contiguous()
        else:
            s = float(self.step)
        return fm, fb, f, sb, s

    def materialize(self):
        d = torch.arange(self.D, device=self.device, dtype=torch.float32).view(1, -1, 1, 1)
        first = self.first if torch.is_tensor(self.first) else torch.tensor(float(self.first), device=self.device)
        step = self.step if torch.is_tensor(self.step) else torch.tensor(float(self.step), device=self.device)
        first = first.view(self.B, 1, self.h, self.w) if first.dim() == 3 else first.reshape(-1, 1, 1, 1)
        return (first + step.reshape(-1, 1, 1, 1) * d).expand(self.B, self.D, self.h, self.w).contiguous()


def ladder_supported(V, C, num_groups):
    import os
    if os.environ.get("CASMVS_K1_SMEM", "1") == "0":
        return False
    return (V - 1) in (1, 2) and C in (8, 16, 32) and num_groups in (1, 8)


@_on_tensor_device
def warp_cost_ladder(feats, proj_mats, ladder, num_groups=1, round_tf32=False):
    _require_cuda(feats, proj_mats)
    _no_grad_only(feats)
    B, V, C, h, w = feats.shape
    assert is_channels_last_feats(feats) and (ladder.B, ladder.h, ladder.w) == (B, h, w)
    cout = C if num_groups == 1 else num_groups
    out = torch.empty(B, ladder.D, h, w, cout, device=feats.device, dtype=torch.float32)
    fm, fb, f, sb, s = ladder._args()
    check(_lib.load().casmvs_warp_cost_ladder_fwd(_ptr(feats), _ptr(proj_mats.contiguous()), _ptr(fm),
                                                  _ptr(fb), f, _ptr(sb), s, _ptr(out),
                                                  1 if round_tf32 else 0, B, V, C, ladder.D, h, w,
                                                  num_groups, _stream()), "warp_cost_ladder")
    return as_volume_view(out)


@_on_tensor_device
def regress_ladder(logits, ladder, want_index=False):
    _require_cuda(logits)
    _no_grad_only(logits)
    lg = logits.contiguous()
    B, D, h, w = lg.shape
    depth = torch.empty(B, h, w, device=lg.device, dtype=torch.float32)
    conf = torch.empty_like(depth)
    index = torch.empty(B, h, w, device=lg.device, dtype=torch.int64) if want_index else None
    fm, fb, f, sb, s = ladder._args()
    check(_lib.load().casmvs_regress_ladder_fwd(_ptr(lg), _ptr(fm), _ptr(fb), f, _ptr(sb), s,
                                                _ptr(depth), _ptr(conf), _ptr(index), B, D, h, w,
                                                _stream()), "regress_ladder")
    return depth, conf, index


@_on_tensor_device
def depth_first(current_depth, n_depths, depth_interval):
    _require_cuda(current_depth)
    cur = current_depth.contiguous()
    B, hi, wi = cur.shape
    h, w = 2 * hi, 2 * wi
    step, step_dev = _interval_args(depth_interval, B, cur.device)
    half = float(n_depths / 2 * step)
    out = torch.empty(B, h, w, device=cur.device, dtype=torch.float32)
    check(_lib.load().casmvs_depth_first_fwd(_ptr(cur), 1, half, step, _ptr(step_dev), _ptr(out), B,
                                             n_depths, h, w, _stream()), "depth_first")
    return out


@_on_tensor_device
def fpn_level(prev, c, lat_w, lat_b, smooth_w, smooth_b, want_feat):
    _require_cuda(prev, c, lat_w, lat_b, smooth_w, smooth_b)
    pv = prev.contiguous(memory_format=torch.channels_last)
    cv = c.contiguous(memory_format=torch.channels_last)
    N, clat, h, w = cv.shape
    cout = smooth_w.shape[0]
    assert pv.shape == (N, 32, h // 2, w // 2) and smooth_w.shape[1:] == (32, 3, 3)
    out = torch.empty((N, cout, h, w), device=c.device, dtype=torch.float32,
                      memory_format=torch.channels_last)
    feat = torch.empty((N, 32, h, w), device=c.device, dtype=torch.float32,
                       memory_format=torch.channels_last) if want_feat else None
    check(_lib.load().casmvs_fpn_level_fwd(
        _ptr(pv), _ptr(cv), _ptr(lat_w.detach().contiguous()), _ptr(lat_b.detach().contiguous()),
        _ptr(smooth_w.detach().contiguous()), _ptr(smooth_b.detach().contiguous()), _ptr(feat),
        _ptr(out), N, h, w, clat, cout, _stream()), "fpn_level")
    return feat, out


@_on_tensor_device
def conv2d_planar(x, w_packed, cin, cout, shift=None, slope=1.0, precision=TF32,
                  keep_fp32=False, scale=None):
    _require_cuda(x, w_packed, scale, shift)
    _no_grad_only(x)
    xs = x.contiguous(memory_format=torch.channels_last)
    N, C, H, W = xs.shape
    assert C == cin
    y = torch.empty((N, cout, H, W), device=x.device, dtype=torch.float32,
                    memory_format=torch.channels_last)
    check(_lib.load().casmvs_conv3d_fwd(_ptr(xs), _ptr(w_packed), _ptr(scale), _ptr(shift),
                                        float(slope), None, _ptr(y), 1, cin, cout, N, H, W,
                                        CONV_PLANAR, 1,
                                        precision | (KEEP_FP32_OUT if keep_fp32 else 0),
                                        _stream()), "conv2d_planar")
    return y


@_on_tensor_device
def fpn_merge(prev, c, lat_w, lat_b, round_tf32=False):
    _require_cuda(prev, c, lat_w, lat_b)
    cv = c.contiguous(memory_format=torch.channels_last)
    N, clat, h, w = cv.shape
    pv = None
    if prev is not None:
        pv = prev.contiguous(memory_format=torch.channels_last)
        assert pv.shape == (N, 32, h // 2, w // 2)
    assert lat_w.shape[0] == 32 and lat_w.shape[1] == clat
    feat = torch.empty((N, 32, h, w), device=c.device, dtype=torch.float32,
                       memory_format=torch.channels_last)
    check(_lib.load().casmvs_fpn_merge_fwd(_ptr(pv), _ptr(cv), _ptr(lat_w.detach().contiguous()),
                                           _ptr(lat_b.detach().contiguous()), _ptr(feat), N, h, w,
                                           clat, 1 if round_tf32 else 0, _stream()), "fpn_merge")
    return feat


@_on_tensor_device
def conv2d_rgb8(x, w, bias, slope, round_tf32=False):
    _require_cuda(x, w, bias)
    xs = x.contiguous()
    N, C, H, W = xs.shape
    assert C == 3 and tuple(w.shape) == (8, 3, 3, 3)
    y = torch.empty((N, 8, H, W), device=x.device, dtype=torch.float32,
                    memory_format=torch.channels_last)
    check(_lib.load().casmvs_conv2d_rgb8_fwd(_ptr(xs), _ptr(w.contiguous()), _ptr(bias),
                                             float(slope), _ptr(y), N, H, W,
                                             1 if round_tf32 else 0, _stream()), "conv2d_rgb8")
    return y


@_on_tensor_device
def pack_conv2d_5x5s2_weight(weight):
    _require_cuda(weight)
    assert weight.dim() == 4 and tuple(weight.shape[2:]) == (5, 5)
    out = torch.empty(weight.shape, device=weight.device, dtype=torch.float32)
    release_weight_images(out)
    out.copy_(weight.detach())
    return out


@_on_tensor_device
def conv2d_5x5s2(x, w, shift, slope, round_tf32=False):
    _require_cuda(x, w, shift)
    _no_grad_only(x)
    xs = x.contiguous(memory_format=torch.channels_last)
    N, cin, H, W = xs.shape
    cout = w.shape[0]
    assert tuple(w.shape) == (cout, cin, 5, 5) and w.is_contiguous()
    Ho, Wo = (H - 1) // 2 + 1, (W - 1) // 2 + 1
    y = torch.empty((N, cout, Ho, Wo), device=x.device, dtype=torch.float32,
                    memory_format=torch.channels_last)
    check(_lib.load().casmvs_conv2d_5x5s2_fwd(_ptr(xs), _ptr(w), _ptr(shift), float(slope),
                                              _ptr(y), N, cin, cout, H, W,
                                              1 if round_tf32 else 0, _stream()), "conv2d_5x5s2")
    return y


@_on_tensor_device
def conv2d_5x5s2_fp32(x, w, shift, slope):
    _require_cuda(x, w, shift)
    _no_grad_only(x)
    xs = x.contiguous(memory_format=torch.channels_last)
    N, cin, H, W = xs.shape
    cout = w.shape[0]
    assert tuple(w.shape) == (cout, cin, 5, 5) and w.is_contiguous()
    y = torch.empty((N, cout, (H - 1) // 2 + 1, (W - 1) // 2 + 1), device=x.device,
                    dtype=torch.float32, memory_format=torch.channels_last)
    check(_lib.load().casmvs_conv2d_5x5s2_fp32_fwd(_ptr(xs), _ptr(w), _ptr(shift), float(slope),
                                                   _ptr(y), N, cin, cout, H, W, _stream()),
          "conv2d_5x5s2_fp32")
    return y


@_on_tensor_device
def bias_lrelu_(x, bias, slope, round_tf32=False):
    _require_cuda(x, bias)
    assert x.is_contiguous(memory_format=torch.channels_last) and x.shape[1] % 4 == 0
    check(_lib.load().casmvs_bias_act_nhwc(_ptr(x), _ptr(bias), float(slope), x.numel(),
                                           x.shape[1], 1 if round_tf32 else 0, _stream()),
          "bias_lrelu")
    return x

# ... 87 lines not shown
```

### include/casmvs.h

```cpp
#ifndef CASMVS_H_
#define CASMVS_H_

#include <stddef.h>
#include <stdint.h>

#ifdef __cplusplus
extern "C" {
#endif

#define CASMVS_VERSION 100

enum casmvs_layout { CASMVS_NCHW = 0, CASMVS_NHWC = 1 };
#define CASMVS_ROUND_TF32 256

enum casmvs_precision {
  CASMVS_FP32 = 0,
  CASMVS_TF32 = 1
};

#define CASMVS_KEEP_FP32_OUT 256

enum casmvs_conv_kind {
  CASMVS_CONV = 0,
  CASMVS_CONV_TRANSPOSE = 1,
  CASMVS_CONV_PLANAR = 2
};

int casmvs_version(void);
const char* casmvs_last_error(void);
int casmvs_device_check(int device);
uint64_t casmvs_launch_count(void);
uint64_t casmvs_fallback_count(void);

size_t casmvs_warp_cost_workspace_bytes(int feat_layout, int B, int V, int C, int h, int w);
int casmvs_warp_cost_fwd(const float* feats, int feat_layout, const float* proj,
                         const float* depth_values, float* cost, int cost_layout,
                         int B, int V, int C, int D, int h, int w, int num_groups,
                         void* workspace, size_t workspace_bytes, void* stream);

int casmvs_homo_warp_fwd(const float* src_feat, int feat_layout, const float* proj,
                         const float* depth_values, float* warped, int out_layout,
                         int B, int C, int D, int h, int w, void* stream);

size_t casmvs_packed_conv3d_weight_floats(int Cin, int Cout);
int casmvs_pack_conv3d_weights(const float* w_torch, int kind, int Cin, int Cout,
                               float* w_packed, void* stream);
int casmvs_release_weight_images(const void* w_packed, size_t bytes);
int casmvs_invalidate_weight_cache(void);
uint64_t casmvs_weight_cache_generation(void);
int casmvs_weight_image_count(const void* w_packed, size_t bytes);
int casmvs_settle_weight_images(void);
int casmvs_conv3d_fwd(const float* x, const float* w_packed, const float* scale,
                      const float* shift, float slope, const float* skip, float* y,
                      int B, int Cin, int Cout, int D, int h, int w,
                      int kind, int stride, int precision, void* stream);

size_t casmvs_costreg_param_floats(int Cin);
int casmvs_costreg_layer_info(int Cin, int layer, int* cin, int* cout, int* kind, int* stride,
                              size_t* w_off, size_t* scale_off, size_t* shift_off);
size_t casmvs_costreg_workspace_bytes(int B, int Cin, int D, int h, int w);
int casmvs_costreg_fwd(const float* x, const float* params, float* logits,
                       int B, int Cin, int D, int h, int w, int precision,
                       void* workspace, size_t workspace_bytes, void* stream);

int casmvs_regress_fwd(const float* logits, const float* depth_values, int dv_is_vector,
                       int input_is_prob, float* depth, float* confidence,
                       int64_t* index, float* prob, int B, int D, int h, int w,
                       void* stream);

int casmvs_depth_hypotheses_fwd(const float* cur, int upsample, float half_range,
                                float step, const float* step_dev, float* out,
                                int B, int D, int h, int w, void* stream);
int casmvs_uniform_hypotheses_fwd(float depth_min, float step, const float* depth_min_dev,
                                  const float* step_dev, float* out,
                                  int B, int D, int h, int w, void* stream);

int casmvs_depth_first_fwd(const float* cur, int upsample, float half_range, float step,
                           const float* step_dev, float* out, int B, int D, int h, int w,
                           void* stream);
int casmvs_warp_cost_ladder_fwd(const float* feats, const float* proj, const float* first_map,
                                const float* first_b, float first, const float* step_b, float step,
                                float* cost, int round_tf32, int B, int V, int C, int D, int h, int w,
                                int num_groups, void* stream);
int casmvs_regress_ladder_fwd(const float* logits, const float* first_map, const float* first_b,
                              float first, const float* step_b, float step, float* depth,
                              float* confidence, int64_t* index, int B, int D, int h, int w,
                              void* stream);

int casmvs_fpn_level_fwd(const float* prev, const float* c, const float* lat_w,
                         const float* lat_b, const float* smooth_w, const float* smooth_b,
                         float* feat_out, float* out, int N, int h, int w, int CLAT, int COUT,
                         void* stream);

int casmvs_fpn_merge_fwd(const float* prev, const float* c, const float* lat_w,
                         const float* lat_b, float* feat, int N, int h, int w, int CLAT,
                         int round_tf32, void* stream);

int casmvs_conv2d_rgb8_fwd(const float* x, const float* w, const float* bias, float slope,
                           float* y, int N, int H, int W, int round_tf32, void* stream);

int casmvs_conv2d_5x5s2_fwd(const float* x, const float* w, const float* shift, float slope,
                            float* y, int N, int Cin, int Cout, int H, int W, int round_tf32,
                            void* stream);

int casmvs_conv2d_5x5s2_fp32_fwd(const float* x, const float* w, const float* shift, float slope,
                                 float* y, int N, int Cin, int Cout, int H, int W, void* stream);

int casmvs_bias_lrelu_nhwc(float* x, const float* bias, float slope, size_t numel, int C,
                           void* stream);
int casmvs_bias_act_nhwc(float* x, const float* bias, float slope, size_t numel, int C,
                         int round_tf32, void* stream);

int casmvs_warp_cost_bwd(const float* feats, const float* proj, const float* depth_values,
                         const float* grad_cost, float* grad_feats, int B, int V, int C, int D,
                         int h, int w, int num_groups, void* stream);
int casmvs_conv3d_wgrad(const float* x, const float* grad_y, float* grad_w, int B, int Ca, int Cb,
                        int Di, int hi, int wi, int Do, int ho, int wo, int stride, void* stream);
int casmvs_regress_bwd(const float* logits, const float* depth_values, int dv_is_vector,
                       const float* grad_depth, float* grad_logits, int B, int D, int h, int w,
                       void* stream);

int casmvs_normalize_u8_fwd(const uint8_t* images, float* out, int N, int H, int W,
                            const float* mean3, const float* std3, void* stream);

int casmvs_geo_fuse_fwd(const float* depth_ref, const float* image_ref, const float* proba_ref,
                        const float* const* depth_src, const float* const* image_src,
                        const float* proj_ref2src, const float* proj_src2ref,
                        const float* ref2world, int S, int H, int W, float conf_thresh,
                        int min_consistent, float* depth_refined, float* image_refined,
                        int* geo_count, unsigned char* mask_final, float* points,
                        float* reproj_dbg, unsigned char* mask_dbg, void* stream);

int casmvs_pcd_cell_keys(const float* points, int n, double ox, double oy, double oz, double cell,
                         int gx, int gy, int gz, int sub, int64_t* keys, void* stream);
size_t casmvs_pcd_thin_workspace_bytes(int n, int ncells);
int casmvs_pcd_thin_prepare(const int64_t* cell_keys, const int* cell_start, int n, int ncells,
                            int gx, int gy, int gz, void* workspace, size_t workspace_bytes,
                            void* stream);
int casmvs_pcd_thin_round(const float* points, const int* rank, const int* cell_start, int n,
                          int ncells, double dst, unsigned char* state, int* undecided,
                          const void* workspace, size_t workspace_bytes, void* stream);
int casmvs_pcd_capped_nn(const float* queries, int nq, const float* targets,
                         const int64_t* cell_keys, const int* cell_start, int ncells,
                         const int* super_begin, const double* origin3, double h,
                         const int* super_dims3, const double* box_lo3, const double* box_hi3,
                         double cap, double* dist, void* stream);

int casmvs_nchw_to_nhwc(const float* in, float* out, int N, int C, size_t S, void* stream);
int casmvs_nhwc_to_nchw(const float* in, float* out, int N, int C, size_t S, void* stream);

#ifdef __cplusplus
}
#endif
#endif
```

Baseline: 526.9.

## Use channel-blocked (C/4,D,H,W,4) layout through cost volume and cost-regularization convs

Adds a blocked activation layout in which channels are grouped in fours outermost, (B,C/4,D,h,w,4). The warp-cost kernel writes the cost volume in this layout, and every tensor-core conv3d layer of CostRegNet reads and writes it through new TMA tensor-map descriptors and blocked store offsets. The aim is to make TMA brick loads contiguous and cheaper for the small channel slices the wgmma kernels fetch. It adds layout plumbing across warp, conv and TMA map caching, and returns an error if any layer lacks a tensor-core kernel for the blocked layout.

```diff
diff --git a/casmvsnet_pl_b200/_lib.py b/casmvsnet_pl_b200/_lib.py
--- a/casmvsnet_pl_b200/_lib.py
+++ b/casmvsnet_pl_b200/_lib.py
@@ -8,6 +8,7 @@
 NCHW, NHWC = 0, 1
 ROUND_TF32 = 256
 KEEP_FP32_OUT = 256
+BLOCKED = 512
 FP32, TF32 = 0, 1
 CONV, CONV_TRANSPOSE, CONV_PLANAR = 0, 1, 2
 PRECISIONS = {"fp32": FP32, "tf32": TF32}
@@ -39,6 +40,7 @@
                                           POINTER(c_int), POINTER(c_int), POINTER(c_size_t),
                                           POINTER(c_size_t), POINTER(c_size_t)]),
     "casmvs_costreg_workspace_bytes": (c_size_t, [c_int] * 5),
+    "casmvs_costreg_blocked_supported": (c_int, [c_int, c_int]),
     "casmvs_costreg_fwd": (c_int, [c_void_p, c_void_p, c_void_p, c_int, c_int, c_int, c_int,
                                    c_int, c_int, c_void_p, c_size_t, c_void_p]),
     "casmvs_regress_fwd": (c_int, [c_void_p, c_void_p, c_int, c_int, c_void_p, c_void_p,
diff --git a/casmvsnet_pl_b200/csrc/api.cu b/casmvsnet_pl_b200/csrc/api.cu
--- a/casmvsnet_pl_b200/csrc/api.cu
+++ b/casmvsnet_pl_b200/csrc/api.cu
@@ -21,10 +21,12 @@
                   int h, int w, int kind, int stride, cudaStream_t st, int round_out);
 int conv3d_tma(const float* x, const float* wpk, const float* scale, const float* shift,
                float slope, const float* skip, float* y, int B, int Cin, int Cout, int D, int h,
-               int w, int kind, int stride, int precision, cudaStream_t st);
+               int w, int kind, int stride, int precision, int layout, cudaStream_t st);
 int conv3d_tma2(const float* x, const float* wpk, const float* scale, const float* shift,
                 float slope, const float* skip, float* y, int B, int Cin, int Cout, int D, int h,
-                int w, int kind, int stride, int precision, cudaStream_t st);
+                int w, int kind, int stride, int precision, int layout, cudaStream_t st);
+bool conv3d_tma_enabled();
+int conv3d_tma2_modes();
 
 struct LayerSpec { int cin, cout, kind, stride; };
 
@@ -67,10 +69,10 @@
   return 0;
 }
 
-extern "C" int casmvs_conv3d_fwd(const float* x, const float* w_packed, const float* scale,
-                                 const float* shift, float slope, const float* skip, float* y,
-                                 int B, int Cin, int Cout, int D, int h, int w, int kind,
-                                 int stride, int precision, void* stream) {
+static int conv_layer(const float* x, const float* w_packed, const float* scale,
+                      const float* shift, float slope, const float* skip, float* y, int B,
+                      int Cin, int Cout, int D, int h, int w, int kind, int stride, int precision,
+                      int layout, void* stream) {
   CASMVS_REQUIRE(x && w_packed && y, "conv3d: null pointer");
   CASMVS_REQUIRE(B >= 0 && Cin > 0 && Cout > 0 && D > 0 && h > 0 && w > 0, "conv3d: bad dims");
   CASMVS_REQUIRE(Cin % 4 == 0, "conv3d: Cin must be a multiple of 4 (got %d)", Cin);
@@ -88,19 +90,29 @@
   if (precision == CASMVS_TF32) {
     const int pf = precision | flags;
     int rc = conv3d_tma(x, w_packed, scale, shift, slope, skip, y, B, Cin, Cout, D, h, w, kind,
-                    stride, pf, st);
+                        stride, pf, layout, st);
     if (rc <= 0) return rc;
     if (kind != CASMVS_CONV_PLANAR) {
       rc = conv3d_tma2(x, w_packed, scale, shift, slope, skip, y, B, Cin, Cout, D, h, w, kind,
-                       stride, precision, st);
+                       stride, precision, layout, st);
       if (rc <= 0) return rc;
     }
+    CASMVS_REQUIRE(layout == 0, "conv3d: no tensor-core kernel for the blocked layer %d -> %d "
+                   "(kind %d, stride %d)", Cin, Cout, kind, stride);
     g_fallbacks.fetch_add(1, std::memory_order_relaxed);
   }
   const int round_out =
       (precision == CASMVS_TF32 && Cout > 1 && !(flags & CASMVS_KEEP_FP32_OUT)) ? 1 : 0;
   return conv3d_direct(x, w_packed, scale, shift, slope, skip, y, B, Cin, Cout, D, h, w, kind,
                        stride, st, round_out);
+}
+
+extern "C" int casmvs_conv3d_fwd(const float* x, const float* w_packed, const float* scale,
+                                 const float* shift, float slope, const float* skip, float* y,
+                                 int B, int Cin, int Cout, int D, int h, int w, int kind,
+                                 int stride, int precision, void* stream) {
+  return conv_layer(x, w_packed, scale, shift, slope, skip, y, B, Cin, Cout, D, h, w, kind, stride,
+                    precision, 0, stream);
 }
 
 extern "C" size_t casmvs_costreg_param_floats(int Cin) {
@@ -137,10 +149,23 @@
          sizeof(float);
 }
 
+extern "C" int casmvs_costreg_blocked_supported(int Cin, int precision) {
+  return precision == CASMVS_TF32 && conv3d_tma_enabled() && (conv3d_tma2_modes() & 3) == 3 &&
+         (Cin == 8 || Cin == 16 || Cin == 32);
+}
+
 extern "C" int casmvs_costreg_fwd(const float* x, const float* params, float* logits, int B,
                                   int Cin, int D, int h, int w, int precision, void* workspace,
                                   size_t workspace_bytes, void* stream) {
   CASMVS_REQUIRE(x && params && logits, "costreg: null pointer");
+  const bool blocked_in = (precision & CASMVS_BLOCKED) != 0;
+  precision &= ~CASMVS_BLOCKED;
+  const bool blocked = casmvs_costreg_blocked_supported(Cin, precision) &&
+                       ((reinterpret_cast<uintptr_t>(x) | reinterpret_cast<uintptr_t>(workspace)) &
+                        15) == 0;
+  CASMVS_REQUIRE(!blocked_in || blocked,
+                 "costreg: a blocked input needs the TF32 precision, Cin in {8,16,32}, the "
+                 "tensor-core kernels enabled and 16-byte aligned x and workspace (got Cin=%d)", Cin);
   CASMVS_REQUIRE(D % 8 == 0 && h % 8 == 0 && w % 8 == 0,
                  "costreg: D,h,w must be divisible by 8 (got %d,%d,%d)", D, h, w);
   const size_t need = casmvs_costreg_workspace_bytes(B, Cin, D, h, w);
@@ -171,22 +196,24 @@
   float* u9 = ws;            ws += 2 * n;
   float* u11 = ws;
   const float slope = 0.01f;
+  const int blk = blocked ? kLayoutXBlocked | kLayoutYBlocked : 0;
   int rc;
-#define LAYER(i, in, skip, out, d_, h_, w_, sl)                                                   \
-  rc = casmvs_conv3d_fwd(in, W[i], SC[i], SH[i], sl, skip, out, B, L[i].cin, L[i].cout, d_, h_,  \
-                         w_, L[i].kind, L[i].stride, precision, stream);                          \
+#define LAYER(i, in, skip, out, d_, h_, w_, sl, lay)                                              \
+  rc = conv_layer(in, W[i], SC[i], SH[i], sl, skip, out, B, L[i].cin, L[i].cout, d_, h_, w_,     \
+                  L[i].kind, L[i].stride, precision, lay, stream);                                \
   if (rc) return rc;
-  LAYER(0, x, nullptr, c0, D, h, w, slope)
-  LAYER(1, c0, nullptr, c1, D, h, w, slope)
-  LAYER(2, c1, nullptr, c2, D / 2, h / 2, w / 2, slope)
-  LAYER(3, c2, nullptr, c3, D / 2, h / 2, w / 2, slope)
-  LAYER(4, c3, nullptr, c4, D / 4, h / 4, w / 4, slope)
-  LAYER(5, c4, nullptr, c5, D / 4, h / 4, w / 4, slope)
-  LAYER(6, c5, nullptr, c6, D / 8, h / 8, w / 8, slope)
-  LAYER(7, c6, c4, u7, D / 8, h / 8, w / 8, slope)
-  LAYER(8, u7, c2, u9, D / 4, h / 4, w / 4, slope)
-  LAYER(9, u9, c0, u11, D / 2, h / 2, w / 2, slope)
-  LAYER(10, u11, nullptr, logits, D, h, w, 1.0f)
+  LAYER(0, x, nullptr, c0, D, h, w, slope,
+        (blk & kLayoutYBlocked) | (blocked_in ? kLayoutXBlocked : 0))
+  LAYER(1, c0, nullptr, c1, D, h, w, slope, blk)
+  LAYER(2, c1, nullptr, c2, D / 2, h / 2, w / 2, slope, blk)
+  LAYER(3, c2, nullptr, c3, D / 2, h / 2, w / 2, slope, blk)
+  LAYER(4, c3, nullptr, c4, D / 4, h / 4, w / 4, slope, blk)
+  LAYER(5, c4, nullptr, c5, D / 4, h / 4, w / 4, slope, blk)
+  LAYER(6, c5, nullptr, c6, D / 8, h / 8, w / 8, slope, blk)
+  LAYER(7, c6, c4, u7, D / 8, h / 8, w / 8, slope, blk)
+  LAYER(8, u7, c2, u9, D / 4, h / 4, w / 4, slope, blk)
+  LAYER(9, u9, c0, u11, D / 2, h / 2, w / 2, slope, blk)
+  LAYER(10, u11, nullptr, logits, D, h, w, 1.0f, blk & kLayoutXBlocked)
 #undef LAYER
   return 0;
 }
diff --git a/casmvsnet_pl_b200/csrc/common.cuh b/casmvsnet_pl_b200/csrc/common.cuh
--- a/casmvsnet_pl_b200/csrc/common.cuh
+++ b/casmvsnet_pl_b200/csrc/common.cuh
@@ -17,6 +17,8 @@
 extern std::atomic<uint64_t> g_fallbacks;
 
 inline cudaStream_t as_stream(void* s) { return reinterpret_cast<cudaStream_t>(s); }
+
+constexpr int kLayoutXBlocked = 1, kLayoutYBlocked = 2;
 
 inline int after_launch(const char* what) {
   g_launches.fetch_add(1, std::memory_order_relaxed);
diff --git a/casmvsnet_pl_b200/csrc/conv3d_tma.cu b/casmvsnet_pl_b200/csrc/conv3d_tma.cu
--- a/casmvsnet_pl_b200/csrc/conv3d_tma.cu
+++ b/casmvsnet_pl_b200/csrc/conv3d_tma.cu
@@ -25,6 +25,8 @@
   int tiles_w, tiles_h, nchunks, dchunk;
   int round_out;
   int planar;
+  int x_blocked;
+  int y_blocked;
 };
 
 template <int CIN, int GW, int SLOTS_>
@@ -42,7 +44,7 @@
   static constexpr int kTotal = kBarOff + 192 + 1024;
 };
 
-template <int GW, int OFF>
+template <int GW, int OFF, bool PLANAR>
 __device__ __forceinline__ void store_slice(const float* acc, const Params& p, const float* s_param,
                                             int b, int od, int h0, int w0, int row0, int wl,
                                             int lane, int co_base) {
@@ -50,7 +52,8 @@
     const int m = row0 + r;
     const int oh = h0 + (m >> 3), ow = w0 + (m & 7);
     if (oh >= p.H || ow >= p.W || c >= p.Cout) return;
-    const size_t o = ((((size_t)b * p.D + od) * p.H + oh) * p.W + ow) * p.cout_total + co_base + c;
+    const size_t o =
+        vol_offset(!PLANAR && p.y_blocked, b, od, oh, ow, co_base + c, p.D, p.H, p.W, p.cout_total);
     float v0 = fmaf(a0, s_param[c], s_param[GW + c]);
     float v1 = fmaf(a1, s_param[c + 1], s_param[GW + c + 1]);
     v0 = v0 >= 0.f ? v0 : v0 * p.slope;
@@ -138,9 +141,12 @@
           const uint32_t dst = s_ring + slot * S::kSlotBytes;
           mbar_expect_tx(bar_full + 8 * slot, S::CQ * S::kBrickData);
 #pragma unroll
-          for (int q = 0; q < S::CQ; ++q)
-            tma_load_5d(dst + q * S::kBrickBytes, &xmap, bar_full + 8 * slot, q * 4, w0 - 1,
-                        h0 - 1, d0 - halo + it, b);
+          for (int q = 0; q < S::CQ; ++q) {
+            const Coords5 k = brick_coords(!PLANAR && p.x_blocked, 1, S::CQ, q, w0 - 1, h0 - 1,
+                                           d0 - halo + it, b);
+            tma_load_5d(dst + q * S::kBrickBytes, &xmap, bar_full + 8 * slot, k.c[0], k.c[1],
+                        k.c[2], k.c[3], k.c[4]);
+          }
         }
       }
       __syncwarp();
@@ -170,8 +176,8 @@
         }
         wgmma_commit();
         if (pend_od >= 0)
-          store_slice<GW, 0>(done, p, s_param, pend_b, pend_od, pend_h0, pend_w0, row0, wl, lane,
-                             co_base);
+          store_slice<GW, 0, PLANAR>(done, p, s_param, pend_b, pend_od, pend_h0, pend_w0, row0, wl,
+                                     lane, co_base);
         wgmma_wait_all();
         mbar_arrive(bar_empty + 8 * (g % SLOTS));
 #pragma unroll
@@ -193,7 +199,8 @@
     gs += nslices;
   }
   if (pend_od >= 0)
-    store_slice<GW, 0>(done, p, s_param, pend_b, pend_od, pend_h0, pend_w0, row0, wl, lane, co_base);
+    store_slice<GW, 0, PLANAR>(done, p, s_param, pend_b, pend_od, pend_h0, pend_w0, row0, wl, lane,
+                               co_base);
 }
 
 
@@ -234,19 +241,20 @@
   return 0;
 }
 
-struct MapEntry { const void* x; int B, D, H, W, C, CB, bw, bh, sw; CUtensorMap map; };
+struct MapEntry { const void* x; int B, D, H, W, C, CB, bw, bh, sw, blk; CUtensorMap map; };
 static MapEntry g_maps[128];
 static int g_maps_n = 0, g_maps_next = 0;
 static std::mutex g_maps_mu;
 
 const CUtensorMap* input_map(const float* x, int B, int D, int H, int W, int C, int CB, int box_w,
-                             int box_h, int stride_w) {
+                             int box_h, int stride_w, bool blocked) {
   static thread_local CUtensorMap t_ret;
+  const int blk = blocked ? 1 : 0;
   std::lock_guard<std::mutex> lock(g_maps_mu);
   for (int i = 0; i < g_maps_n; ++i) {
     const MapEntry& e = g_maps[i];
     if (e.x == x && e.B == B && e.D == D && e.H == H && e.W == W && e.C == C && e.CB == CB &&
-        e.bw == box_w && e.bh == box_h && e.sw == stride_w) {
+        e.bw == box_w && e.bh == box_h && e.sw == stride_w && e.blk == blk) {
       t_ret = e.map;
       return &t_ret;
     }
@@ -256,12 +264,27 @@
   MapEntry& e = g_maps[g_maps_next];
   g_maps_next = (g_maps_next + 1) % 128;
   if (g_maps_n < 128) ++g_maps_n;
-  const cuuint64_t gdim[5] = {(cuuint64_t)C, (cuuint64_t)W, (cuuint64_t)H, (cuuint64_t)D,
+  const cuuint64_t vox = (cuuint64_t)D * H * W;
+  cuuint64_t gdim[5] = {(cuuint64_t)C, (cuuint64_t)W, (cuuint64_t)H, (cuuint64_t)D, (cuuint64_t)B};
+  cuuint64_t gstr[4] = {(cuuint64_t)C * 4, (cuuint64_t)W * C * 4, (cuuint64_t)H * W * C * 4,
+                        vox * C * 4};
+  cuuint32_t box[5] = {(cuuint32_t)CB, (cuuint32_t)box_w, (cuuint32_t)box_h, 1, 1};
+  cuuint32_t estr[5] = {1, (cuuint32_t)stride_w, 1, 1, 1};
+  if (blocked && stride_w == 1) {
+    const cuuint64_t d2[5] = {4 * (cuuint64_t)W, (cuuint64_t)H, (cuuint64_t)D, (cuuint64_t)C / 4,
                               (cuuint64_t)B};
-  const cuuint64_t gstr[4] = {(cuuint64_t)C * 4, (cuuint64_t)W * C * 4, (cuuint64_t)H * W * C * 4,
-                              (cuuint64_t)D * H * W * C * 4};
-  const cuuint32_t box[5] = {(cuuint32_t)CB, (cuuint32_t)box_w, (cuuint32_t)box_h, 1, 1};
-  const cuuint32_t estr[5] = {1, (cuuint32_t)stride_w, 1, 1, 1};
+    const cuuint64_t s2[4] = {(cuuint64_t)W * 16, (cuuint64_t)H * W * 16, vox * 16, vox * C * 4};
+    const cuuint32_t b2[5] = {4 * (cuuint32_t)box_w, (cuuint32_t)box_h, 1, 1, 1};
+    for (int i = 0; i < 5; ++i) { gdim[i] = d2[i]; box[i] = b2[i]; estr[i] = 1; }
+    for (int i = 0; i < 4; ++i) gstr[i] = s2[i];
+  } else if (blocked) {
+    const cuuint64_t d2[5] = {4, (cuuint64_t)W, (cuuint64_t)H, (cuuint64_t)D,
+                              (cuuint64_t)C / 4 * B};
+    const cuuint64_t s2[4] = {16, (cuuint64_t)W * 16, (cuuint64_t)H * W * 16, vox * 16};
+    for (int i = 0; i < 5; ++i) gdim[i] = d2[i];
+    for (int i = 0; i < 4; ++i) gstr[i] = s2[i];
+    box[0] = 4;
+  }
   const CUtensorMapSwizzle sw = CB * 4 == 128 ? CU_TENSOR_MAP_SWIZZLE_128B
                                 : CB * 4 == 64 ? CU_TENSOR_MAP_SWIZZLE_64B
                                 : CB * 4 == 32 ? CU_TENSOR_MAP_SWIZZLE_32B
@@ -275,7 +298,8 @@
               (int)r, C, W, H, D, B);
     return nullptr;
   }
-  e.x = x; e.B = B; e.D = D; e.H = H; e.W = W; e.C = C; e.CB = CB; e.bw = box_w; e.bh = box_h; e.sw = stride_w;
+  e.x = x; e.B = B; e.D = D; e.H = H; e.W = W; e.C = C; e.CB = CB; e.bw = box_w; e.bh = box_h;
+  e.sw = stride_w; e.blk = blk;
   t_ret = e.map;
   return &t_ret;
 }
@@ -288,7 +312,7 @@
   auto kfn = conv3d_tma_kernel<CIN, GW, SLOTS, PLANAR>;
   static std::atomic<bool> attr_set[kMaxDevices];
   if (int rc = opt_in_smem(kfn, S::kTotal, attr_set, "conv3d_tma")) return rc;
-  const CUtensorMap* map = input_map(x, p.B, p.D, p.H, p.W, CIN, 4, kHaloW, kHaloH);
+  const CUtensorMap* map = input_map(x, p.B, p.D, p.H, p.W, CIN, 4, kHaloW, kHaloH, 1, p.x_blocked);
   if (!map) return -2;
   static int dchunk_env = -1;
   if (dchunk_env < 0) {
@@ -320,18 +344,25 @@
 
 }
 
+bool conv3d_tma_enabled() {
+  static const int enabled = [] {
+    const char* e = getenv("CASMVS_TMA");
+    return e ? atoi(e) : 1;
+  }();
+  return enabled != 0;
+}
+
 int conv3d_tma(const float* x, const float* wpk, const float* scale, const float* shift,
                float slope, const float* skip, float* y, int B, int Cin, int Cout, int D, int h,
-               int w, int kind, int stride, int precision_flags, cudaStream_t st) {
+               int w, int kind, int stride, int precision_flags, int layout, cudaStream_t st) {
   const int precision = precision_flags & 0xff;
-  static int enabled = -1, round_out = 1;
-  if (enabled < 0) {
-    const char* e = getenv("CASMVS_TMA");
-    enabled = e ? atoi(e) : 1;
-    if (const char* s = getenv("CASMVS_TC_ROUND")) round_out = atoi(s);
-  }
-  if (!enabled || precision != CASMVS_TF32) return 1;
+  static const int round_out = [] {
+    const char* s = getenv("CASMVS_TC_ROUND");
+    return s ? atoi(s) : 1;
+  }();
+  if (!conv3d_tma_enabled() || precision != CASMVS_TF32) return 1;
   if ((kind != CASMVS_CONV && kind != CASMVS_CONV_PLANAR) || stride != 1) return 1;
+  if (kind == CASMVS_CONV_PLANAR && layout != 0) return 1;
   const bool deep = Cin == 64 && Cout == 64;
   if (!deep && (!(Cin == 8 || Cin == 16 || Cin == 32) || Cout > 32)) return 1;
   if ((reinterpret_cast<uintptr_t>(x) & 15) != 0) return 1;
@@ -343,6 +374,8 @@
   p.tiles_h = (h + tc::kTileH - 1) / tc::kTileH;
   const int npad = p.Cout <= 8 ? 8 : p.Cout <= 16 ? 16 : 32;
   p.planar = kind == CASMVS_CONV_PLANAR ? 1 : 0;
+  p.x_blocked = (layout & kLayoutXBlocked) ? 1 : 0;
+  p.y_blocked = (layout & kLayoutYBlocked) ? 1 : 0;
   p.round_out = (round_out && Cout > 1 && !(precision_flags & CASMVS_KEEP_FP32_OUT)) ? 1 : 0;
 #define TMA_CASE(CI, NP, SL)                                                    \
   if (Cin == CI && npad == NP)                                                  \
diff --git a/casmvsnet_pl_b200/csrc/conv3d_tma2.cu b/casmvsnet_pl_b200/csrc/conv3d_tma2.cu
--- a/casmvsnet_pl_b200/csrc/conv3d_tma2.cu
+++ b/casmvsnet_pl_b200/csrc/conv3d_tma2.cu
@@ -23,6 +23,8 @@
   int B, Di, Hi, Wi, Do, Ho, Wo, Cout;
   int tiles_w, tiles_h, nchunks, dchunk;
   int round_out;
+  int x_blocked;
+  int y_blocked;
 };
 
 template <int MODE, int CIN, int COUT>
@@ -113,8 +115,11 @@
             const int wc = MODE == MODE_S2 ? 2 * w0 - 1 + par
                            : MODE == MODE_T ? w0 : 2 * w0 - 2 + par;
             const int hc = MODE == MODE_S2 ? 2 * h0 - 1 : MODE == MODE_T ? h0 : 2 * h0 - 2;
-            tma_load_5d(dst + pl * C::kPlaneBytes, &xmap, bar_full + 8 * slot, 4 * q, wc,
-                        hc, s_first + it, b);
+            const tma::Coords5 k = tma::brick_coords(MODE != MODE_P5 && p.x_blocked,
+                                                     MODE == MODE_T ? 1 : 2, C::CQ,
+                                                     q, wc, hc, s_first + it, b);
+            tma_load_5d(dst + pl * C::kPlaneBytes, &xmap, bar_full + 8 * slot, k.c[0], k.c[1],
+                        k.c[2], k.c[3], k.c[4]);
           }
         }
       }
@@ -164,7 +169,9 @@
       };
 
       auto store2 = [&](int od, int oh, int ow, int c, float a0, float a1, bool has_skip) {
-        const size_t o = ((((size_t)b * p.Do + od) * p.Ho + oh) * p.Wo + ow) * p.Cout + co_base + c;
+        const size_t o =
+            tma::vol_offset(MODE != MODE_P5 && p.y_blocked, b, od, oh, ow, co_base + c, p.Do, p.Ho,
+                            p.Wo, p.Cout);
         float v0 = fmaf(a0, s_param[c], s_param[32 + c]);
         float v1 = fmaf(a1, s_param[c + 1], s_param[32 + c + 1]);
         v0 = v0 >= 0.f ? v0 : v0 * p.slope;
@@ -183,7 +190,52 @@
           if (c < COUT && mh < p.Ho && mw < p.Wo) store2(od, mh, mw, c, a0, a1, false);
         });
       };
+      auto store_t_blocked = [&](const float* src, int od) {
+        const bool odd = lane & 1;
+        const size_t qstr = (size_t)p.Do * p.Ho * p.Wo * 4;
+        const size_t yoff = ((size_t)b * (p.Cout / 4) + co_base / 4) * qstr +
+                            (size_t)od * p.Ho * p.Wo * 4;
+#pragma unroll
+        for (int ph = 0; ph < 2; ++ph) {
+#pragma unroll
+          for (int jj = 0; jj < COUT / 8; ++jj) {
+#pragma unroll
+            for (int h = 0; h < 2; ++h) {
+              const int i0 = 4 * (2 * ph * (COUT / 8) + jj) + 2 * h;
+              const int i1 = i0 + COUT / 2;
+              const int c = 8 * jj + 2 * (lane & 3);
+              float e[4] = {src[i0], src[i0 + 1], src[i1], src[i1 + 1]};
+#pragma unroll
+              for (int k = 0; k < 4; ++k) {
+                const float v = fmaf(e[k], s_param[c + (k & 1)], s_param[32 + c + (k & 1)]);
+                e[k] = v >= 0.f ? v : v * p.slope;
+              }
+              const float s0 = __shfl_xor_sync(0xffffffffu, odd ? e[0] : e[2], 1);
+              const float s1 = __shfl_xor_sync(0xffffffffu, odd ? e[1] : e[3], 1);
+              float4 v = odd ? make_float4(s0, s1, e[2], e[3]) : make_float4(e[0], e[1], s0, s1);
+              const int m = row0 + 16 * wl + (lane >> 2) + 8 * h;
+              const int mh = h0 + (m >> 3), mw = w0 + (m & 7);
+              if (mh >= p.Hi || mw >= p.Wi) continue;
+              const size_t o = yoff + (c >> 2) * qstr +
+                               (uint32_t)(((2 * mh + ph) * p.Wo + 2 * mw + (odd ? 1 : 0)) * 4);
+              if (p.skip) {
+                const float4 s4 = __ldg(reinterpret_cast<const float4*>(p.skip + o));
+                v.x += s4.x; v.y += s4.y; v.z += s4.z; v.w += s4.w;
+              }
+              if (p.round_out) {
+                v.x = to_tf32(v.x); v.y = to_tf32(v.y); v.z = to_tf32(v.z); v.w = to_tf32(v.w);
+              }
+              *reinterpret_cast<float4*>(p.y + o) = v;
+            }
+          }
+        }
+      };
       auto store_t = [&](const float* pd1, int jd) {
+        if (COUT >= 16 && p.y_blocked) {
+          store_t_blocked(prev0, 2 * jd);
+          store_t_blocked(pd1, 2 * jd + 1);
+          return;
+        }
         auto one = [&](int pd, int r, int col, float a0, float a1) {
           const int m = row0 + r;
           const int mh = h0 + (m >> 3), mw = w0 + (m & 7);
@@ -313,9 +365,11 @@
   static std::atomic<bool> attr_set[kMaxDevices];
   if (int rc = opt_in_smem(kfn, C::kTotal, attr_set, "conv3d_tma2")) return rc;
   const CUtensorMap* map =
-      MODE == MODE_S2   ? tma::input_map(x, p.B, p.Di, p.Hi, p.Wi, CIN, 4, 17, C::BR, 2)
+      MODE == MODE_S2   ? tma::input_map(x, p.B, p.Di, p.Hi, p.Wi, CIN, 4, 17, C::BR, 2,
+                                         p.x_blocked)
       : MODE == MODE_P5 ? tma::input_map(x, p.B, p.Di, p.Hi, p.Wi, CIN, 4, 19, C::BR, 2)
-                        : tma::input_map(x, p.B, p.Di, p.Hi, p.Wi, CIN, 4, C::BW, C::BR, 1);
+                        : tma::input_map(x, p.B, p.Di, p.Hi, p.Wi, CIN, 4, C::BW, C::BR, 1,
+                                         p.x_blocked);
   if (!map) return -2;
   const int per_sm = tma::resident_per_sm(kfn, kConvThreads, C::kTotal);
   const int Dm = MODE == MODE_T ? p.Di : p.Do;
@@ -353,19 +407,25 @@
 
 }
 
+int conv3d_tma2_modes() {
+  static const int modes = [] {
+    const char* e = getenv("CASMVS_TMA2");
+    return e ? atoi(e) : 3;
+  }();
+  return modes;
+}
+
 int conv3d_tma2(const float* x, const float* wpk, const float* scale, const float* shift,
                 float slope, const float* skip, float* y, int B, int Cin, int Cout, int D, int h,
-                int w, int kind, int stride, int precision, cudaStream_t st) {
-  static int enabled = -1;
-  if (enabled < 0) {
-    const char* e = getenv("CASMVS_TMA2");
-    enabled = e ? atoi(e) : 3;
-  }
+                int w, int kind, int stride, int precision, int layout, cudaStream_t st) {
+  const int enabled = conv3d_tma2_modes();
   if (!enabled || precision != CASMVS_TF32) return 1;
   if ((reinterpret_cast<uintptr_t>(x) & 15) != 0) return 1;
   tma2::Params p;
   p.scale = scale; p.shift = shift; p.skip = skip; p.y = y;
   p.slope = slope; p.B = B; p.Di = D; p.Hi = h; p.Wi = w; p.Cout = Cout; p.round_out = 1;
+  p.x_blocked = (layout & kLayoutXBlocked) ? 1 : 0;
+  p.y_blocked = (layout & kLayoutYBlocked) ? 1 : 0;
   if (kind == CASMVS_CONV && stride == 2 && (enabled & 1)) {
     if (skip) return 1;
     p.Do = (D - 1) / 2 + 1; p.Ho = (h - 1) / 2 + 1; p.Wo = (w - 1) / 2 + 1;
@@ -399,6 +459,7 @@
   p.scale = nullptr; p.shift = shift; p.skip = nullptr; p.y = y; p.slope = slope;
   p.B = 1; p.Di = N; p.Hi = H; p.Wi = W; p.Do = N; p.Ho = (H - 1) / 2 + 1; p.Wo = (W - 1) / 2 + 1;
   p.Cout = Cout; p.round_out = round_tf32 ? 1 : 0;
+  p.x_blocked = p.y_blocked = 0;
   cudaStream_t st = as_stream(stream);
   if (Cin == 8 && Cout == 16) return tma2::launch2<tma2::MODE_P5, 8, 16>(x, w, p, st);
   if (Cin == 16 && Cout == 32) return tma2::launch2<tma2::MODE_P5, 16, 32>(x, w, p, st);
diff --git a/casmvsnet_pl_b200/csrc/k1_common.cuh b/casmvsnet_pl_b200/csrc/k1_common.cuh
--- a/casmvsnet_pl_b200/csrc/k1_common.cuh
+++ b/casmvsnet_pl_b200/csrc/k1_common.cuh
@@ -37,6 +37,10 @@
 __device__ __forceinline__ void stg256(float* p, const u64 (&v)[4]) {
   asm volatile("st.global.v2.b64 [%0], {%1,%2};" ::"l"(p), "l"(v[0]), "l"(v[1]) : "memory");
   asm volatile("st.global.v2.b64 [%0], {%1,%2};" ::"l"(p + 4), "l"(v[2]), "l"(v[3]) : "memory");
+}
+__device__ __forceinline__ void stg256q(float* p, size_t qstride, const u64 (&v)[4]) {
+  asm volatile("st.global.v2.b64 [%0], {%1,%2};" ::"l"(p), "l"(v[0]), "l"(v[1]) : "memory");
+  asm volatile("st.global.v2.b64 [%0], {%1,%2};" ::"l"(p + qstride), "l"(v[2]), "l"(v[3]) : "memory");
 }
 
 __device__ __forceinline__ float round_tf32_f(float x) {
diff --git a/casmvsnet_pl_b200/csrc/tma_common.cuh b/casmvsnet_pl_b200/csrc/tma_common.cuh
--- a/casmvsnet_pl_b200/csrc/tma_common.cuh
+++ b/casmvsnet_pl_b200/csrc/tma_common.cuh
@@ -59,7 +59,21 @@
 }
 
 const CUtensorMap* input_map(const float* x, int B, int D, int H, int W, int C, int CB, int box_w,
-                             int box_h, int stride_w = 1);
+                             int box_h, int stride_w = 1, bool blocked = false);
+
+struct Coords5 { int c[5]; };
+__host__ __device__ __forceinline__ Coords5 brick_coords(bool blocked, int stride_w, int cq, int q,
+                                                         int w, int h, int d, int b) {
+  if (!blocked) return {{4 * q, w, h, d, b}};
+  if (stride_w == 1) return {{4 * w, h, d, q, b}};
+  return {{0, w, h, d, b * cq + q}};
+}
+
+__host__ __device__ __forceinline__ size_t vol_offset(bool blocked, int b, int d, int h, int w,
+                                                      int c, int D, int H, int W, int C) {
+  if (!blocked) return ((((size_t)b * D + d) * H + h) * W + w) * C + c;
+  return (((((size_t)b * (C >> 2) + (c >> 2)) * D + d) * H + h) * W + w) * 4 + (c & 3);
+}
 
 int encode_tiled(CUtensorMap* out, const void* base, int rank, const uint64_t* dims,
                  const uint64_t* strides_bytes, const uint32_t* box, int swizzle_bytes);
diff --git a/casmvsnet_pl_b200/csrc/warp_cost.cu b/casmvsnet_pl_b200/csrc/warp_cost.cu
--- a/casmvsnet_pl_b200/csrc/warp_cost.cu
+++ b/casmvsnet_pl_b200/csrc/warp_cost.cu
@@ -450,7 +450,8 @@
 int g_k1_dchunk = 0;
 
 int warp_var_smem(const float* feats, const float* proj, const Hyp& dv, float* cost, int B,
-                  int V, int C, int D, int h, int w, int num_groups, int rnd, cudaStream_t st);
+                  int V, int C, int D, int h, int w, int num_groups, int rnd, int blocked,
+                  cudaStream_t st);
 
 template <int NSRC, int CT>
 static void launch_k1(bool gwc, bool nhwc, dim3 grd, cudaStream_t st, const float* f,
@@ -539,7 +540,7 @@
   }
   if (nhwc) {
     const Hyp hyp{depth_values, nullptr, nullptr, nullptr, 0.f, 0.f};
-    const int rc = warp_var_smem(f, proj, hyp, cost, B, V, C, D, h, w, num_groups, rnd, st);
+    const int rc = warp_var_smem(f, proj, hyp, cost, B, V, C, D, h, w, num_groups, rnd, 0, st);
     if (rc <= 0) return rc;
   }
   if (!gwc && nhwc && (V == 3 || V == 2) && (C == 8 || C == 16 || C == 32)) {
@@ -608,9 +609,11 @@
                  "warp_cost_ladder: bad dims (h,w >= 2)");
   CASMVS_REQUIRE((size_t)h * w * C < (1u << 31), "warp_cost_ladder: view too large");
   if (B == 0) return 0;
+  const int blocked = (round_tf32 & CASMVS_BLOCKED) ? 1 : 0;
+  const int rnd = (round_tf32 & ~CASMVS_BLOCKED) ? 1 : 0;
   const Hyp hyp{nullptr, first_map, first_b, step_b, first, step};
-  const int rc = warp_var_smem(feats, proj, hyp, cost, B, V, C, D, h, w, num_groups,
-                               round_tf32 ? 1 : 0, as_stream(stream));
+  const int rc = warp_var_smem(feats, proj, hyp, cost, B, V, C, D, h, w, num_groups, rnd, blocked,
+                               as_stream(stream));
   if (rc == 1) {
     set_error("warp_cost_ladder: shape not covered by the staged kernel (V-1 in {1,2}, C in "
               "{8,16,32}, groups 1 or 8, channels-last features): materialise the hypotheses and "
diff --git a/casmvsnet_pl_b200/csrc/warp_cost_smem.cu b/casmvsnet_pl_b200/csrc/warp_cost_smem.cu
--- a/casmvsnet_pl_b200/csrc/warp_cost_smem.cu
+++ b/casmvsnet_pl_b200/csrc/warp_cost_smem.cu
@@ -57,7 +57,8 @@
   return t;
 }
 
-template <int NSRC, int C, int TW, int TH, int MINB, bool GWC = false, int CP = 8>
+template <int NSRC, int C, int TW, int TH, int MINB, bool GWC = false, int CP = 8,
+          bool BLOCKED = false>
 __global__ void __launch_bounds__(TW* TH*(C / CP), MINB)
 warp_var_smem_kernel(const __grid_constant__ CUtensorMap fmap, const float* __restrict__ feats,
                      const float* __restrict__ proj, const Hyp hyp,
@@ -108,7 +109,12 @@
   const int d_begin = blockIdx.z * dchunk;
   const int d_end = min(D, d_begin + dchunk);
   const HypPix hp(hyp, b, D, (size_t)hw, pix);
-  float* optr = cost + ((size_t)(b * D + d_begin) * hw + pix) * COUT + (GWC ? sub * NG : c0);
+  const int co = GWC ? sub * NG : c0;
+  const size_t pstr = BLOCKED ? (size_t)hw * 4 : (size_t)hw * COUT;
+  const size_t qstr = BLOCKED ? (size_t)D * hw * 4 : 4;
+  float* optr = cost + (BLOCKED ? (((size_t)b * (COUT / 4) + co / 4) * D + d_begin) * hw * 4 +
+                                      (size_t)pix * 4 + (co & 3)
+                                : ((size_t)(b * D + d_begin) * hw + pix) * COUT + co);
   const int row_b = BW * TEXB;
 
   uint32_t phase = 0;
@@ -255,14 +261,14 @@
         if (active) {
           if constexpr (NG == 8) {
             u64 ov[4] = {pk2(o[0], o[1]), pk2(o[2], o[3]), pk2(o[4], o[5]), pk2(o[6], o[7])};
-            stg256(optr, ov);
+            stg256q(optr, qstr, ov);
           } else if constexpr (NG == 4) {
             st4(optr, make_float4(o[0], o[1], o[2], o[3]));
           } else {
             *reinterpret_cast<float2*>(optr) = make_float2(o[0], o[1]);
           }
         }
-        optr += (size_t)hw * COUT;
+        optr += pstr;
         continue;
       }
       u64 o[NP];
@@ -283,16 +289,16 @@
 #pragma unroll
         for (int hh = 0; hh < CP / 8; ++hh) {
           const u64 oo[4] = {o[4 * hh], o[4 * hh + 1], o[4 * hh + 2], o[4 * hh + 3]};
-          stg256(optr + 8 * hh, oo);
-        }
-      }
-      optr += (size_t)hw * C;
+          stg256q(optr + 2 * hh * qstr, qstr, oo);
+        }
+      }
+      optr += pstr;
     }
     d0 += n;
   }
 }
 
-template <int C, int TW, int TH, int PG, int MINB>
+template <int C, int TW, int TH, int PG, int MINB, bool BLOCKED>
 __global__ void __launch_bounds__(TW* TH*(C / kCPT), MINB)
 warp_var_smem_pg_kernel(const __grid_constant__ CUtensorMap fmap, const float* __restrict__ feats,
                         const float* __restrict__ proj, const Hyp hyp, float* __restrict__ cost,
@@ -338,7 +344,11 @@
   const int d_begin = blockIdx.z * dchunk;
   const int d_end = min(D, d_begin + dchunk);
   const HypPix hp(hyp, b, D, (size_t)hw, pix);
-  float* optr = cost + ((size_t)(b * D + d_begin) * hw + pix) * C + c0;
+  const size_t pstr = BLOCKED ? (size_t)hw * 4 : (size_t)hw * C;
+  const size_t qstr = BLOCKED ? (size_t)D * hw * 4 : 4;
+  float* optr = cost + (BLOCKED ? (((size_t)b * (C / 4) + c0 / 4) * D + d_begin) * hw * 4 +
+                                      (size_t)pix * 4
+                                : ((size_t)(b * D + d_begin) * hw + pix) * C + c0);
   const int row_b = BW * TEXB;
   const bool rowal = (row_b & 1023) == 0;
   u64 refsq[4];
@@ -489,13 +499,13 @@
                 o[k] = pk2(round_tf32_f(lo), round_tf32_f(hi));
               }
             }
-            if (active) stg256(optr + (size_t)p * hw * C, o);
+            if (active) stg256q(optr + p * pstr, qstr, o);
           }
         }
       }
-      optr += (size_t)PG * hw * C;
-    }
-    optr -= (size_t)(((n + PG - 1) / PG) * PG - n) * hw * C;
+      optr += PG * pstr;
+    }
+    optr -= (((n + PG - 1) / PG) * PG - n) * pstr;
     d0 += n;
   }
 }
@@ -534,7 +544,7 @@
 
 template <int NSRC, int C, int TW, int TH, int MINB, bool GWC = false, int CP = 8>
 static int launch(const float* feats, const float* proj, const Hyp& dv, float* cost, int B, int D,
-                  int h, int w, int rnd, cudaStream_t st) {
+                  int h, int w, int rnd, int blocked, cudaStream_t st) {
   constexpr int NT = TW * TH * (C / CP);
   static const int mx = env_int("CASMVS_K1_MARGIN_X", NSRC <= 2 ? 16 : 8);
   static const int my = env_int("CASMVS_K1_MARGIN_Y", NSRC <= 2 ? 4 : 3);
@@ -542,9 +552,10 @@
   const int BW = TW + mx, BH = TH + my;
   const int box_stride = (BW * BH * C * 4 + 1023) & ~1023;
   const size_t smem = (size_t)NSRC * box_stride + sizeof(Small) + 1024;
-  auto kfn = warp_var_smem_kernel<NSRC, C, TW, TH, MINB, GWC, CP>;
-  static std::atomic<bool> attr_set[kMaxDevices];
-  if (int rc = opt_in_smem(kfn, 200 * 1024, attr_set, "warp_cost")) return rc;
+  auto kfn = blocked ? warp_var_smem_kernel<NSRC, C, TW, TH, MINB, GWC, CP, true>
+                     : warp_var_smem_kernel<NSRC, C, TW, TH, MINB, GWC, CP, false>;
+  static std::atomic<bool> attr_set[2][kMaxDevices];
+  if (int rc = opt_in_smem(kfn, 200 * 1024, attr_set[blocked ? 1 : 0], "warp_cost")) return rc;
   if (smem > 200 * 1024) return 1;
   CUtensorMap map;
   if (!feature_map(&map, feats, B * (NSRC + 1), h, w, C, BW, BH)) return -2;
@@ -561,7 +572,7 @@
 
 template <int C, int TW, int TH, int PG, int MINB>
 static int launch_pg(const float* feats, const float* proj, const Hyp& dv, float* cost, int B, int D,
-                     int h, int w, int rnd, cudaStream_t st) {
+                     int h, int w, int rnd, int blocked, cudaStream_t st) {
   constexpr int NSRC = 2, NT = TW * TH * (C / kCPT);
   static const int mx = env_int("CASMVS_K1_MARGIN_X", 16);
   static const int my = env_int("CASMVS_K1_MARGIN_Y", 4);
@@ -570,9 +581,10 @@
   const int BW = (TW + mx + wq - 1) / wq * wq, BH = TH + my;
   const int box_stride = (BW * BH * C * 4 + 1023) & ~1023;
   const size_t smem = (size_t)NSRC * box_stride + sizeof(Small) + 1024;
-  auto kfn = warp_var_smem_pg_kernel<C, TW, TH, PG, MINB>;
-  static std::atomic<bool> attr_set[kMaxDevices];
-  if (int rc = opt_in_smem(kfn, 200 * 1024, attr_set, "warp_cost")) return rc;
+  auto kfn = blocked ? warp_var_smem_pg_kernel<C, TW, TH, PG, MINB, true>
+                     : warp_var_smem_pg_kernel<C, TW, TH, PG, MINB, false>;
+  static std::atomic<bool> attr_set[2][kMaxDevices];
+  if (int rc = opt_in_smem(kfn, 200 * 1024, attr_set[blocked ? 1 : 0], "warp_cost")) return rc;
   if (smem > 200 * 1024) return 1;
   CUtensorMap map;
   if (!feature_map(&map, feats, B * (NSRC + 1), h, w, C, BW, BH)) return -2;
@@ -590,7 +602,8 @@
 }
 
 int warp_var_smem(const float* feats, const float* proj, const Hyp& dv, float* cost, int B,
-                  int V, int C, int D, int h, int w, int num_groups, int rnd, cudaStream_t st) {
+                  int V, int C, int D, int h, int w, int num_groups, int rnd, int blocked,
+                  cudaStream_t st) {
   static const int enabled = k1s::env_int("CASMVS_K1_SMEM", 1);
   if (!enabled) return 1;
   if ((reinterpret_cast<uintptr_t>(feats) & 15) != 0 || B > 65535) return 1;
@@ -600,7 +613,7 @@
   if (num_groups != 1) {
     if (num_groups != 8) return 1;
 #define K1G(NS, CC, TW_, TH_, MB) \
-  if (V - 1 == NS && C == CC) return launch<NS, CC, TW_, TH_, MB, true>(feats, proj, dv, cost, B, D, h, w, rnd, st);
+  if (V - 1 == NS && C == CC) return launch<NS, CC, TW_, TH_, MB, true>(feats, proj, dv, cost, B, D, h, w, rnd, blocked, st);
     K1G(1, 8, 32, 4, 5) K1G(1, 16, 32, 2, 5) K1G(1, 32, 16, 2, 5)
     K1G(2, 8, 32, 4, 5) K1G(2, 16, 32, 2, 5) K1G(2, 32, 16, 2, 5)
     K1G(4, 8, 32, 4, 4) K1G(4, 16, 32, 4, 2) K1G(4, 32, 16, 4, 2)
@@ -609,9 +622,9 @@
   }
   static const int variant = env_int("CASMVS_K1S_VARIANT", 16);
 #define K1S(VAR, NS, CC, TW_, TH_, MB) \
-  if (variant == VAR && V - 1 == NS && C == CC) return launch<NS, CC, TW_, TH_, MB>(feats, proj, dv, cost, B, D, h, w, rnd, st);
+  if (variant == VAR && V - 1 == NS && C == CC) return launch<NS, CC, TW_, TH_, MB>(feats, proj, dv, cost, B, D, h, w, rnd, blocked, st);
 #define K1P(VAR, CC, TW_, TH_, PG_, MB) \
-  if (variant == VAR && V - 1 == 2 && C == CC) return launch_pg<CC, TW_, TH_, PG_, MB>(feats, proj, dv, cost, B, D, h, w, rnd, st);
+  if (variant == VAR && V - 1 == 2 && C == CC) return launch_pg<CC, TW_, TH_, PG_, MB>(feats, proj, dv, cost, B, D, h, w, rnd, blocked, st);
   K1P(16, 8, 32, 4, 2, 4) K1P(16, 16, 32, 2, 2, 4) K1P(16, 32, 16, 2, 2, 4)
   K1P(11, 8, 32, 4, 4, 4) K1P(11, 16, 32, 2, 4, 4) K1P(11, 32, 16, 2, 4, 4)
   K1S(4, 2, 8, 32, 4, 5) K1S(4, 2, 16, 32, 2, 5) K1S(4, 2, 32, 16, 2, 5)
diff --git a/casmvsnet_pl_b200/models/mvsnet.py b/casmvsnet_pl_b200/models/mvsnet.py
--- a/casmvsnet_pl_b200/models/mvsnet.py
+++ b/casmvsnet_pl_b200/models/mvsnet.py
@@ -285,19 +285,32 @@
         x = conv0 + up(self.conv11, x)
         return AG.conv3d(x, self.prob.weight, ops.CONV, 1, prec) + self.prob.bias.view(1, -1, 1, 1, 1)
 
-    def forward(self, x):
-        if torch.is_grad_enabled() and (x.requires_grad or
-                                        any(p.requires_grad for p in self.parameters())):
-            return self._forward_autograd(x)
+    def _check_inference(self):
         for bn in self._norm_modules():
             if bn.training:
                 raise ops._lib.CasMVSError("CostRegNet inference path needs .eval() (training "
                                            "runs through the autograd path: enable grad)")
             if abs(activation_slope(bn) - 0.01) > 1e-12:
                 raise ops._lib.CasMVSError("casmvs_costreg_fwd assumes LeakyReLU(0.01) norm_act")
+
+    def forward(self, x):
+        if torch.is_grad_enabled() and (x.requires_grad or
+                                        any(p.requires_grad for p in self.parameters())):
+            return self._forward_autograd(x)
+        self._check_inference()
         logits = ops.costreg(x, self.packed_params(), self.in_channels,
                              ops.PRECISIONS[self.precision])
         return logits.unsqueeze(1)
+
+    def blocked_supported(self):
+        return self.precision == "tf32" and ops.costreg_blocked_supported(self.in_channels)
+
+    def forward_blocked(self, x):
+        self._check_inference()
+        if not self.blocked_supported():
+            raise ops._lib.CasMVSError("CostRegNet.forward_blocked needs the tf32 precision and "
+                                       "tensor-core kernels for every layer (in_channels 8, 16, 32)")
+        return ops.costreg(x, self.packed_params(), self.in_channels, ops.TF32, blocked=True)
 
 
 class CascadeMVSNet(nn.Module):
@@ -390,9 +403,10 @@
                 ops.is_channels_last_feats(feats_l):
             first = init_depth_min if depth_prev is None else ops.depth_first(depth_prev, D, depth_interval_l)
             lad = ops.Ladder(first, depth_interval_l, D, B, h, w, feats_l.device)
+            blocked = cost_reg.blocked_supported()
             cost = ops.warp_cost_ladder(feats_l, proj_mats_l, lad, self.G,
-                                        round_tf32=(cost_reg.precision == "tf32"))
-            logits = cost_reg(cost).squeeze(1)
+                                        round_tf32=(cost_reg.precision == "tf32"), blocked=blocked)
+            logits = cost_reg.forward_blocked(cost) if blocked else cost_reg(cost).squeeze(1)
             del cost
             depth, confidence, self._last_index = ops.regress_ladder(logits, lad,
                                                                      want_index=self.return_index)
diff --git a/casmvsnet_pl_b200/ops.py b/casmvsnet_pl_b200/ops.py
--- a/casmvsnet_pl_b200/ops.py
+++ b/casmvsnet_pl_b200/ops.py
@@ -7,7 +7,7 @@
 import torch
 
 from . import _lib
-from ._lib import (CONV, CONV_PLANAR, CONV_TRANSPOSE, FP32, KEEP_FP32_OUT, NCHW, NHWC, PRECISIONS, TF32,
+from ._lib import (BLOCKED, CONV, CONV_PLANAR, CONV_TRANSPOSE, FP32, KEEP_FP32_OUT, NCHW, NHWC, PRECISIONS, TF32,
                    check)
 
 _checked_devices = set()
@@ -195,13 +195,25 @@
                 w_off=wo.value, scale_off=so.value, shift_off=ho.value)
 
 
-@_on_tensor_device
-def costreg(x, params, cin, precision=FP32):
+def costreg_blocked_supported(cin, precision=TF32):
+    return bool(_lib.load().casmvs_costreg_blocked_supported(cin, precision))
+
+
+@_on_tensor_device
+def costreg(x, params, cin, precision=FP32, blocked=False):
     _require_cuda(x, params)
     _no_grad_only(x)
-    xs = volume_storage(x)
-    B, D, h, w, c = xs.shape
-    assert c == cin
+    if blocked:
+        if x.dim() != 6 or x.shape[-1] != 4 or x.shape[1] * 4 != cin or not x.is_contiguous():
+            raise ValueError(f"costreg: blocked input must be a contiguous (B,{cin // 4},D,h,w,4) "
+                             f"tensor, got {tuple(x.shape)}")
+        xs = x
+        B, _, D, h, w, _ = xs.shape
+        precision |= BLOCKED
+    else:
+        xs = volume_storage(x)
+        B, D, h, w, c = xs.shape
+        assert c == cin
     lib = _lib.load()
     ws_bytes = lib.casmvs_costreg_workspace_bytes(B, cin, D, h, w)
     ws = torch.empty(ws_bytes // 4, device=x.device, dtype=torch.float32)
@@ -309,19 +321,21 @@
 
 
 @_on_tensor_device
-def warp_cost_ladder(feats, proj_mats, ladder, num_groups=1, round_tf32=False):
+def warp_cost_ladder(feats, proj_mats, ladder, num_groups=1, round_tf32=False, blocked=False):
     _require_cuda(feats, proj_mats)
     _no_grad_only(feats)
     B, V, C, h, w = feats.shape
     assert is_channels_last_feats(feats) and (ladder.B, ladder.h, ladder.w) == (B, h, w)
     cout = C if num_groups == 1 else num_groups
-    out = torch.empty(B, ladder.D, h, w, cout, device=feats.device, dtype=torch.float32)
+    shape = (B, cout // 4, ladder.D, h, w, 4) if blocked else (B, ladder.D, h, w, cout)
+    out = torch.empty(shape, device=feats.device, dtype=torch.float32)
     fm, fb, f, sb, s = ladder._args()
     check(_lib.load().casmvs_warp_cost_ladder_fwd(_ptr(feats), _ptr(proj_mats.contiguous()), _ptr(fm),
                                                   _ptr(fb), f, _ptr(sb), s, _ptr(out),
-                                                  1 if round_tf32 else 0, B, V, C, ladder.D, h, w,
-                                                  num_groups, _stream()), "warp_cost_ladder")
-    return as_volume_view(out)
+                                                  (1 if round_tf32 else 0) | (BLOCKED if blocked else 0),
+                                                  B, V, C, ladder.D, h, w, num_groups, _stream()),
+          "warp_cost_ladder")
+    return out if blocked else as_volume_view(out)
 
 
 @_on_tensor_device
diff --git a/include/casmvs.h b/include/casmvs.h
--- a/include/casmvs.h
+++ b/include/casmvs.h
@@ -19,6 +19,8 @@
 };
 
 #define CASMVS_KEEP_FP32_OUT 256
+
+#define CASMVS_BLOCKED 512
 
 enum casmvs_conv_kind {
   CASMVS_CONV = 0,
@@ -59,6 +61,7 @@
 int casmvs_costreg_layer_info(int Cin, int layer, int* cin, int* cout, int* kind, int* stride,
                               size_t* w_off, size_t* scale_off, size_t* shift_off);
 size_t casmvs_costreg_workspace_bytes(int B, int Cin, int D, int h, int w);
+int casmvs_costreg_blocked_supported(int Cin, int precision);
 int casmvs_costreg_fwd(const float* x, const float* params, float* logits,
                        int B, int Cin, int D, int h, int w, int precision,
                        void* workspace, size_t workspace_bytes, void* stream);
```

Result: faster. 562.7, median of 6 (+6.8%).
